# danielSanchezQ/dkg

Measured on AMD Instinct MI355X. Metric: verified shares/sec (whole node) at n=1024,t=511; full-ceremony wall time, higher is better.
Workload: dtype u32 (GF(2^255-19), Z_l); 1 GPU; one DKG ceremony n=1024, t=511 (share gen + round-2/4 checks + finalise); n=1024, t=511, parallelism=single GPU, verify_streams=2, rounds_2_4_fused=True, degree_split=4, recombination=short lattice multipliers, recombination_addends=affine Niels, stepping_additions=dedicated (complete redo where exceptional)

## Files before the change

### dkg_amd/_lib.py

```python
import ctypes
import os
import sys

HERE = os.path.dirname(os.path.abspath(__file__))
LIB_PATH = os.environ.get("DKG_AMD_LIB", os.path.join(HERE, "libdkg_amd.so"))

DKG_OK = 0
DKG_E_ARG = -1
DKG_E_DECODE = -2
DKG_E_DEVICE = -3
DKG_E_NOMEM = -4
REJECT, ACCEPT, SELF, SKIPPED, MISSING = 0, 1, 2, 3, 4
FIN_OK, FIN_R2_ERROR, FIN_R4_ERROR, FIN_PHASE4_ERROR, FIN_INSUFFICIENT, FIN_PANIC = 0, 1, 2, 3, 4, 5
COMPLAINT_IGNORED, COMPLAINT_NO_PHASE3 = 4, 5
COMPLAINT_NOT_OWNED = -2
DKG_PS_OK, DKG_PS_NO_COMMITMENT, DKG_PS_NO_DISCLOSURE = 0, 1, 2

_lib = None


class DkgError(RuntimeError):
    def __init__(self, code, msg=""):
        self.code = code
        names = {DKG_E_ARG: "DKG_E_ARG", DKG_E_DECODE: "DKG_E_DECODE", DKG_E_DEVICE: "DKG_E_DEVICE",
                 DKG_E_NOMEM: "DKG_E_NOMEM"}
        super().__init__(f"{names.get(code, code)}: {msg}")


class CeremonyOut(ctypes.Structure):
    _fields_ = [
        ("E", ctypes.c_void_p), ("A", ctypes.c_void_p),
        ("s", ctypes.c_void_p), ("s_prime", ctypes.c_void_p),
        ("dec2", ctypes.c_void_p), ("dec4", ctypes.c_void_p),
        ("qualified", ctypes.c_void_p), ("r2_error", ctypes.c_void_p), ("r4_error", ctypes.c_void_p),
        ("complaints2", ctypes.c_void_p), ("reconstruct", ctypes.c_void_p),
        ("final_share", ctypes.c_void_p), ("public_share", ctypes.c_void_p),
        ("mpk", ctypes.c_uint8 * 32),
        ("n_qualified", ctypes.c_int32), ("phase4_error", ctypes.c_int32),
        ("ms_round1", ctypes.c_double), ("ms_round2", ctypes.c_double), ("ms_round3", ctypes.c_double),
        ("ms_round4", ctypes.c_double), ("ms_finalise", ctypes.c_double), ("ms_total", ctypes.c_double),
    ]


class ReceiverPlan(ctypes.Structure):
    _fields_ = [("chunk", ctypes.c_uint32), ("stages", ctypes.c_uint32), ("arity", ctypes.c_uint32 * 16),
                ("mult", (ctypes.c_uint8 * 32) * 16)]


class ShardOutcome(ctypes.Structure):
    _fields_ = [
        ("qualified", ctypes.c_void_p), ("complaints2", ctypes.c_void_p), ("r2_error", ctypes.c_void_p),
        ("reconstruct", ctypes.c_void_p), ("r4_error", ctypes.c_void_p),
        ("n_qualified", ctypes.c_int32), ("phase4_error", ctypes.c_int32),
    ]


class BatchOut(ctypes.Structure):
    _fields_ = [
        ("mpk", ctypes.c_void_p), ("n_qualified", ctypes.c_void_p), ("phase4_error", ctypes.c_void_p),
        ("qualified", ctypes.c_void_p),
        ("r2_error", ctypes.c_void_p), ("r4_error", ctypes.c_void_p), ("complaints2", ctypes.c_void_p),
        ("reconstruct", ctypes.c_void_p), ("final_share", ctypes.c_void_p), ("public_share", ctypes.c_void_p),
        ("dec2", ctypes.c_void_p), ("dec4", ctypes.c_void_p),
        ("ms_round1", ctypes.c_double), ("ms_checks", ctypes.c_double), ("ms_round3", ctypes.c_double),
        ("ms_finalise", ctypes.c_double), ("ms_total", ctypes.c_double),
    ]


def lib():
    global _lib
    if _lib is not None:
        return _lib
    if not os.path.exists(LIB_PATH):
        raise RuntimeError(f"{LIB_PATH} is missing: build it with `make -C dkg_amd` or __graft_entry__.build()")
    if "torch" not in sys.modules and not os.environ.get("DKG_NO_TORCH_PREIMPORT"):
        try:
            import torch
        except Exception:
            pass
    L = ctypes.CDLL(LIB_PATH)
    sz, p, u8p = ctypes.c_size_t, ctypes.c_void_p, ctypes.c_char_p
    L.dkg_ctx_create.argtypes = [ctypes.c_int, ctypes.POINTER(p)]
    L.dkg_ctx_destroy.argtypes = [p]
    L.dkg_ctx_destroy.restype = None
    L.dkg_ctx_last_error.argtypes = [p]
    L.dkg_ctx_last_error.restype = ctypes.c_char_p
    L.dkg_device_count.argtypes = []
    L.dkg_ctx_set_streams.argtypes = [p, ctypes.c_int]
    L.dkg_ctx_set_overlap.argtypes = [p, ctypes.c_int]
    L.dkg_ctx_set_verify_mode.argtypes = [p, ctypes.c_int]
    L.dkg_ctx_fallback_rows.argtypes = [p]
    L.dkg_ctx_fallback_rows.restype = sz
    L.dkg_ctx_set_split.argtypes = [p, ctypes.c_int]
    L.dkg_ctx_set_stepping.argtypes = [p, ctypes.c_int]
    L.dkg_ctx_set_field_mode.argtypes = [p, ctypes.c_int]
    L.dkg_ctx_set_binomial.argtypes = [p, ctypes.c_int]
    L.dkg_ctx_set_check.argtypes = [p, ctypes.c_int]
    L.dkg_ctx_last_split.argtypes = [p]
    L.dkg_ctx_last_split_len.argtypes = [p]
    L.dkg_ctx_last_split_len.restype = sz
    L.dkg_split_model_ms.argtypes = [sz, sz, sz, ctypes.c_int]
    L.dkg_split_model_ms.restype = ctypes.c_double
    L.dkg_split_len.argtypes = [sz, sz, sz, ctypes.c_int]
    L.dkg_split_len.restype = sz
    L.dkg_ctx_set_combine.argtypes = [p, ctypes.c_int]
    L.dkg_ctx_last_combine.argtypes = [p]
    L.dkg_ctx_last_binomial.argtypes = [p]
    L.dkg_ctx_set_addends.argtypes = [p, ctypes.c_int]
    L.dkg_ctx_set_stepping_formula.argtypes = [p, ctypes.c_int]
    L.dkg_ctx_stepping_redos.argtypes = [p]
    L.dkg_ctx_stepping_redos.restype = ctypes.c_longlong
    L.dkg_ctx_binomial_reruns.argtypes = [p]
    L.dkg_ctx_binomial_wave_redos.argtypes = [p]
    L.dkg_ctx_binomial_wave_redos.restype = ctypes.c_longlong
    L.dkg_ctx_clock_probe.argtypes = [p, ctypes.c_uint, ctypes.POINTER(ctypes.c_double), ctypes.POINTER(ctypes.c_double)]
    L.dkg_device_pci_bus_id.argtypes = [ctypes.c_int, ctypes.c_char_p, ctypes.c_int]
    L.dkg_split_multipliers.argtypes = [sz, sz, ctypes.c_int, p, p]
    if hasattr(L, "dkg_zero_tests"):
        L.dkg_zero_tests.argtypes = [p, sz, p, p]
    if hasattr(L, "dkg_fe_ops"):
        L.dkg_fe_ops.argtypes = [p, ctypes.c_int, ctypes.c_int, sz, p, p]
    if hasattr(L, "dkg_sc_ops"):
        L.dkg_sc_ops.argtypes = [p, ctypes.c_int, sz, p, p]
    L.dkg_jsf_digits.argtypes = [p, p, p, p, p]
    L.dkg_split_digits.argtypes = [sz, sz, ctypes.c_int, ctypes.c_int, p, p]
    L.dkg_ctx_phase_ms.argtypes = [p, ctypes.c_char_p]
    L.dkg_ctx_phase_ms.restype = ctypes.c_double
    L.dkg_env_check.argtypes = [sz, sz]
    L.dkg_env_init.argtypes = [p, sz, sz, u8p, sz, p]
    L.dkg_msm_batch.argtypes = [p, sz, sz, u8p, u8p, p]
    L.dkg_fixed_base_batch.argtypes = [p, p, sz, u8p, p]
    L.dkg_poly_eval_batch.argtypes = [p, sz, sz, u8p, sz, p, p]
    L.dkg_points_valid_batch.argtypes = [p, sz, u8p, p]
    L.dkg_share_gen.argtypes = [p, sz, sz, sz, u8p, u8p, p, p, p, p]
    L.dkg_verify_pairs.argtypes = [p, sz, sz, ctypes.c_int, sz, sz, u8p, u8p, p, p]
    L.dkg_verify_receiver.argtypes = [p, sz, sz, ctypes.c_int, sz, u8p, u8p, p, p]
    L.dkg_receiver_plan_for.argtypes = [sz, sz, ctypes.c_uint32, ctypes.c_int, ctypes.POINTER(ReceiverPlan)]
    L.dkg_receiver_plan_cost_us.argtypes = [sz, sz, ctypes.c_uint32, ctypes.POINTER(ReceiverPlan)]
    L.dkg_receiver_plan_cost_us.restype = ctypes.c_double
    L.dkg_receiver_plan_constants.argtypes = [ctypes.POINTER(ctypes.c_double)]
    L.dkg_receiver_plan_constants.restype = None
    L.dkg_ctx_set_receiver_chunk.argtypes = [p, ctypes.c_int]
    L.dkg_ctx_last_receiver_chunk.argtypes = [p]
    L.dkg_commitment_eval.argtypes = [p, sz, sz, sz, p, u8p, p, p]
    if hasattr(L, "dkg_pair_eval_shape"):
        L.dkg_pair_eval_shape.argtypes = [sz, ctypes.c_int] + [ctypes.POINTER(ctypes.c_uint32)] * 3
        L.dkg_commitment_eval_pairs.argtypes = [p, sz, sz, sz, p, p, u8p, p, p]
    L.dkg_verify_receivers.argtypes = [p, sz, sz, ctypes.c_int, sz, p, u8p, u8p, p, p, p]
    L.dkg_party_round2.argtypes = [p, sz, sz, sz, u8p, u8p, u8p, u8p, p, p, p, p, p, p, p]
    if hasattr(L, "dkg_seat_pack"):
        L.dkg_seat_pack.argtypes = [sz, sz, p] + [ctypes.POINTER(ctypes.c_uint32)] * 3 + [p, p, ctypes.POINTER(ctypes.c_uint32)]
        L.dkg_commitment_eval_seats.argtypes = [p, sz, sz, sz, sz, p, p, u8p, p, p]
        L.dkg_verify_seats.argtypes = [p, sz, sz, sz, ctypes.c_int, sz, p, p, u8p, u8p, p, p, p]
        L.dkg_party_round2_seats.argtypes = [p, sz, sz, sz, sz, p, p, u8p, u8p, u8p, u8p, p, p, p, p, p, p, p]
    if hasattr(L, "dkg_finalise_seats"):
        L.dkg_complaints_verify_ceremonies.argtypes = [p, sz, sz, sz, sz, p, p, p, u8p, u8p, u8p, u8p, u8p, p, p]
        L.dkg_complaints3_verify_ceremonies.argtypes = [p, sz, sz, sz, sz, p, p, p, u8p, u8p, u8p, u8p, u8p, u8p, p, p]
        L.dkg_party_round3_seats.argtypes = [p, sz, sz, sz, sz, p, p, u8p, u8p, p, p]
        L.dkg_finalise_seats.argtypes = [p, sz, sz, sz, sz, p, p, u8p, u8p, u8p, u8p, u8p, u8p, u8p, sz, p, p, p, u8p,
                                         p, p, p]
        L.dkg_seat_finalise_status.argtypes = [sz, sz, sz, u8p, u8p, u8p, p, ctypes.c_int, ctypes.c_int, p]
    if hasattr(L, "dkg_party_round1_seats"):
        L.dkg_party_round1_seats.argtypes = [p, sz, sz, sz, sz, p, p, u8p, u8p, u8p, u8p, p, p, p, p, p, p, p]
        L.dkg_ctx_set_seat_deal.argtypes = [p, ctypes.c_int]
        L.dkg_ctx_last_seat_deal.argtypes = [p]
        L.dkg_seat_enc_digits.argtypes = [p, p, ctypes.POINTER(ctypes.c_int)]
    if hasattr(L, "dkg_seat_eval_shape"):
        L.dkg_seat_eval_shape.argtypes = [sz, sz, sz, ctypes.c_uint32, ctypes.c_int] + [ctypes.POINTER(ctypes.c_uint32)] * 3 + [
            ctypes.POINTER(ctypes.c_uint64)]
        L.dkg_seat_eval_constants.argtypes = [ctypes.POINTER(ctypes.c_double)]
        L.dkg_seat_eval_constants.restype = None
        L.dkg_ctx_set_seat_eval.argtypes = [p, ctypes.c_int, ctypes.c_int]
        L.dkg_ctx_last_seat_eval.argtypes = [p, ctypes.POINTER(ctypes.c_int)]
    if hasattr(L, "dkg_public_shares"):
        L.dkg_commitment_sum.argtypes = [p, sz, sz, sz, u8p, u8p, p, p]
        L.dkg_public_shares.argtypes = [p, sz, sz, sz, u8p, u8p, u8p, u8p, sz, p, sz, p, p, p, u8p, p, p, p, p]
        L.dkg_public_share_status.argtypes = [sz, u8p, u8p, u8p, ctypes.c_uint32, sz, p, p, p]
        L.dkg_ctx_set_public_share_slab.argtypes = [p, sz]
    L.dkg_ceremony_run.argtypes = [p, sz, sz, u8p, u8p, ctypes.POINTER(CeremonyOut)]
    L.dkg_ceremony_verify.argtypes = [p, sz, sz, u8p, u8p, u8p, u8p, ctypes.POINTER(CeremonyOut)]
    L.dkg_ceremony_verify_fetched.argtypes = [p, sz, sz, u8p, u8p, u8p, u8p, u8p, u8p, ctypes.POINTER(CeremonyOut)]
    L.dkg_ceremony_run_device.argtypes = [p, sz, sz, p, p, ctypes.POINTER(CeremonyOut)]
    L.dkg_ceremony_shard_device.argtypes = [p, sz, sz, sz, sz, p, p, p, p, p, p, ctypes.POINTER(ctypes.c_double)]
    L.dkg_ceremony_shard_verify_device.argtypes = [p, sz, sz, sz, sz, p, p, p, p, p, p, p, p,
                                                    ctypes.POINTER(ctypes.c_double)]
    L.dkg_ceremony_shard_full_device.argtypes = [p, sz, sz, sz, sz, p, p, p, u8p, u8p, p, p, p, p, p, p,
                                                  ctypes.POINTER(ctypes.c_double)]
    L.dkg_ceremony_shard_verify_full_device.argtypes = [p, sz, sz, sz, sz, p, p, p, p, u8p, p, p, p, p,
                                                         ctypes.POINTER(ctypes.c_double)]
    L.dkg_ctx_set_key_comb.argtypes = [p, ctypes.c_int]
    L.dkg_ctx_last_key_comb.argtypes = [p]
    L.dkg_key_comb_choice.argtypes = [sz, sz, ctypes.c_int, ctypes.c_int]
    L.dkg_key_comb_constants.argtypes = [ctypes.POINTER(ctypes.c_double)]
    L.dkg_key_comb_constants.restype = None
    L.dkg_ceremony_batch_device.argtypes = [p, sz, sz, sz, p, p, ctypes.POINTER(BatchOut)]
    L.dkg_ceremony_batch_verify.argtypes = [p, sz, sz, sz, u8p, u8p, u8p, u8p, ctypes.POINTER(BatchOut)]
    L.dkg_dealer_coeffs_device.argtypes = [p, u8p, ctypes.c_uint32, sz, sz, sz, sz, p, p]
    L.dkg_member_keys.argtypes = [p, u8p, ctypes.c_uint32, sz, p, p]
    L.dkg_enc_randomness.argtypes = [u8p, ctypes.c_uint32, sz, sz, sz, sz, p]
    L.dkg_enc_randomness_device.argtypes = [p, u8p, ctypes.c_uint32, sz, sz, sz, sz, sz, p]
    L.dkg_encrypt_shares.argtypes = [p, sz, sz, u8p, u8p, u8p, u8p, p, p]
    L.dkg_decrypt_shares.argtypes = [p, sz, sz, u8p, u8p, u8p, p, p, p]
    L.dkg_ceremony_run_full_device.argtypes = [p, sz, sz, p, p, p, u8p, u8p, ctypes.POINTER(CeremonyOut)]
    L.dkg_ceremony_verify_full.argtypes = [p, sz, sz, u8p, u8p, u8p, u8p, u8p, ctypes.POINTER(CeremonyOut)]
    L.dkg_member_keys_batch.argtypes = [p, u8p, ctypes.c_uint32, sz, sz, p, p]
    L.dkg_encrypt_shares_batch.argtypes = [p, sz, sz, u8p, u8p, u8p, u8p, p, p]
    L.dkg_decrypt_shares_batch.argtypes = [p, sz, sz, u8p, u8p, u8p, p, p, p]
    L.dkg_ceremony_batch_full_device.argtypes = [p, sz, sz, sz, p, p, p, u8p, u8p, ctypes.POINTER(BatchOut)]
    L.dkg_ceremony_batch_verify_full.argtypes = [p, sz, sz, sz, u8p, u8p, u8p, u8p, u8p, ctypes.POINTER(BatchOut),
                                                 p, p]
    L.dkg_ctx_set_batch_full_chunk.argtypes = [p, sz]
    L.dkg_misbehaviour_prove.argtypes = [p, sz, u8p, u8p, u8p, p]
    L.dkg_complaint1_verify.argtypes = [p, sz, sz, p, u8p, u8p, u8p, u8p, p]
    L.dkg_complaint3_verify.argtypes = [p, sz, sz, p, u8p, u8p, u8p, u8p, p]
    L.dkg_complaints_prove.argtypes = [p, sz, u8p, u8p, u8p, p]
    L.dkg_complaints_verify.argtypes = [p, sz, sz, sz, p, p, u8p, u8p, u8p, u8p, u8p, p, p]
    L.dkg_ctx_set_complaint_eval.argtypes = [p, ctypes.c_int]
    L.dkg_ceremony_verify_full_complaints.argtypes = [p, sz, sz, u8p, u8p, u8p, u8p, u8p, u8p, sz, p, p, u8p,
                                                      ctypes.POINTER(CeremonyOut), p, p]
    L.dkg_complaints3_verify.argtypes = [p, sz, sz, sz, p, p, u8p, u8p, u8p, u8p, u8p, u8p, p, p]
    L.dkg_ceremony_verify_fetched_proven.argtypes = [p, sz, sz, u8p, u8p, u8p, u8p, u8p, u8p, sz, p, p, u8p, u8p,
                                                     ctypes.POINTER(CeremonyOut), p, p, p]
    L.dkg_ceremony_verify_full_proven.argtypes = [p, sz, sz, u8p, u8p, u8p, u8p, u8p, u8p, sz, p, p, u8p, u8p, sz, p, p,
                                                  u8p, u8p, ctypes.POINTER(CeremonyOut), p, p, p, p, p]
    L.dkg_ceremony_batch_verify_proven.argtypes = [p, sz, sz, sz, u8p, u8p, u8p, u8p, u8p, u8p, sz, p, p, p, u8p, u8p,
                                                   ctypes.POINTER(BatchOut), p, p, p]
    L.dkg_ceremony_batch_verify_full_proven.argtypes = [p, sz, sz, sz, u8p, u8p, u8p, u8p, u8p, u8p, sz, p, p, p, u8p,
                                                        u8p, sz, p, p, p, u8p, u8p, ctypes.POINTER(BatchOut), p, p, p, p,
                                                        p, p, p]
    L.dkg_ceremony_shard_verify_proven_device.argtypes = [p, sz, sz, sz, sz, p, p, p, p, u8p, u8p, sz, p, p, u8p, u8p,
                                                           p, p, p, p, sz, p, p, ctypes.POINTER(ctypes.c_double)]
    L.dkg_ceremony_shard_verify_full_proven_device.argtypes = [p, sz, sz, sz, sz, p, p, p, p, u8p, u8p, u8p, u8p, sz, p,
                                                                p, u8p, sz, p, p, u8p, u8p, p, p, p, p, sz, p, p, p, p,
                                                                ctypes.POINTER(ctypes.c_double)]
    L.dkg_ctx_last_complaint_eval.argtypes = [p]
    L.dkg_shard_combine_proven_device.argtypes = [p, sz, sz, sz, p, p, p, p, ctypes.c_int, p, p,
                                                  ctypes.POINTER(ShardOutcome), p, p, p]
    L.dkg_multi_ceremony_verify_proven.argtypes = [p, sz, sz, u8p, u8p, u8p, u8p, u8p, u8p, sz, p, p, u8p, u8p,
                                                   ctypes.POINTER(CeremonyOut), p, p, p]
    L.dkg_multi_ceremony_verify_full_proven.argtypes = [p, sz, sz, u8p, u8p, u8p, u8p, u8p, u8p, sz, p, p, u8p, u8p, sz,
                                                        p, p, u8p, u8p, ctypes.POINTER(CeremonyOut), p, p, p, p, p]
    L.dkg_dealer_coeffs.argtypes = [u8p, ctypes.c_uint32, sz, sz, sz, p, p]
    L.dkg_scalar_sum_device.argtypes = [p, sz, sz, p, p, p]
    L.dkg_point_sum_device.argtypes = [p, sz, p, p, p]
    L.dkg_share_gen_device.argtypes = [p, sz, sz, sz, p, p, p, p, p, p]
    L.dkg_ceremony_shard_recon_device.argtypes = [p, sz, sz, sz, sz, u8p, u8p, u8p, u8p, p, p,
                                                  ctypes.POINTER(ctypes.c_int32)]
    L.dkg_finalise_parties.argtypes = [p, sz, sz, u8p, u8p, u8p, u8p, u8p, u8p, u8p, p, p, p]
    L.dkg_shard_range.argtypes = [sz, sz, sz, ctypes.POINTER(sz), ctypes.POINTER(sz)]
    L.dkg_shard_range.restype = None
    L.dkg_shard_rows.argtypes = [sz, sz]
    L.dkg_shard_rows.restype = sz
    L.dkg_shard_combine_device.argtypes = [p, sz, sz, sz, p, p, p, p, ctypes.POINTER(ShardOutcome)]
    L.dkg_shard_combine_packed_device.argtypes = [p, sz, sz, sz, p, p, p, p, ctypes.POINTER(ShardOutcome)]
    L.dkg_fixed_base_windows.argtypes = []
    L.dkg_key_comb_windows.argtypes = []
    if hasattr(L, "dkg_comb_geometry"):
        L.dkg_ctx_set_comb_build.argtypes = [p, ctypes.c_int]
        L.dkg_ctx_last_comb_build.argtypes = [p]
        L.dkg_ctx_last_comb_build_ms.argtypes = [p]
        L.dkg_ctx_last_comb_build_ms.restype = ctypes.c_double
        L.dkg_comb_geometry.argtypes = [ctypes.c_int, ctypes.POINTER(ctypes.c_int), ctypes.POINTER(ctypes.c_int),
                                        ctypes.POINTER(ctypes.c_uint32), ctypes.POINTER(ctypes.c_uint32)]
        L.dkg_comb_entries.argtypes = [p, ctypes.c_int, u8p, ctypes.c_int, ctypes.c_uint32, ctypes.c_uint32, p]
    L.dkg_packed_row_words.argtypes = [sz]
    L.dkg_packed_row_words.restype = sz
    L.dkg_decisions_pack_device.argtypes = [p, sz, sz, sz, sz, p, p]
    L.dkg_shard_finalise_device.argtypes = [p, sz, sz, sz, p, p, u8p, ctypes.c_int, p, p, p]
    L.dkg_multi_create.argtypes = [ctypes.POINTER(ctypes.c_int), ctypes.c_int, ctypes.POINTER(p)]
    L.dkg_multi_destroy.argtypes = [p]
    L.dkg_multi_destroy.restype = None
    L.dkg_multi_size.argtypes = [p]
    L.dkg_multi_ctx.argtypes = [p, ctypes.c_int]
    L.dkg_multi_ctx.restype = p
    L.dkg_multi_last_error.argtypes = [p]
    L.dkg_multi_last_error.restype = ctypes.c_char_p
    L.dkg_multi_phase_ms.argtypes = [p, ctypes.c_char_p]
    L.dkg_multi_phase_ms.restype = ctypes.c_double
    L.dkg_multi_env_init.argtypes = [p, sz, sz, u8p, sz, p]
    L.dkg_multi_ceremony_run.argtypes = [p, sz, sz, u8p, u8p, ctypes.POINTER(CeremonyOut)]
    L.dkg_multi_ceremony_run_device.argtypes = [p, sz, sz, ctypes.POINTER(p), ctypes.POINTER(p),
                                                ctypes.POINTER(CeremonyOut)]
    L.dkg_multi_ceremony_verify.argtypes = [p, sz, sz, u8p, u8p, u8p, u8p, ctypes.POINTER(CeremonyOut)]
    L.dkg_multi_ceremony_run_full.argtypes = [p, sz, sz, u8p, u8p, u8p, u8p, u8p, ctypes.POINTER(CeremonyOut)]
    L.dkg_multi_ceremony_run_full_device.argtypes = [p, sz, sz, ctypes.POINTER(p), ctypes.POINTER(p), ctypes.POINTER(p),
                                                     u8p, u8p, ctypes.POINTER(CeremonyOut)]
    L.dkg_multi_ceremony_verify_full.argtypes = [p, sz, sz, u8p, u8p, u8p, u8p, u8p, ctypes.POINTER(CeremonyOut)]
    _lib = L
    return L


EXPORTED = [
    "dkg_ctx_create", "dkg_ctx_destroy", "dkg_ctx_last_error", "dkg_ctx_phase_ms", "dkg_ctx_set_streams", "dkg_ctx_set_overlap",
    "dkg_device_count", "dkg_env_init",
    "dkg_env_check", "dkg_msm_batch", "dkg_fixed_base_batch", "dkg_poly_eval_batch",
    "dkg_points_valid_batch", "dkg_share_gen", "dkg_verify_pairs", "dkg_verify_receiver",
    "dkg_ctx_set_split", "dkg_ctx_set_stepping", "dkg_ctx_set_field_mode", "dkg_ctx_set_binomial", "dkg_ctx_set_check", "dkg_ctx_last_split", "dkg_ctx_last_split_len", "dkg_ctx_set_verify_mode", "dkg_ctx_fallback_rows", "dkg_split_model_ms", "dkg_split_len",
    "dkg_ctx_set_combine", "dkg_ctx_last_combine", "dkg_ctx_last_binomial", "dkg_ctx_set_addends", "dkg_ctx_set_stepping_formula", "dkg_ctx_stepping_redos", "dkg_zero_tests", "dkg_fe_ops", "dkg_sc_ops", "dkg_stepping_lane_map", "dkg_ctx_binomial_reruns", "dkg_ctx_binomial_wave_redos", "dkg_split_multipliers", "dkg_jsf_digits", "dkg_split_digits",
    "dkg_ctx_clock_probe", "dkg_device_pci_bus_id",
    "dkg_ceremony_run", "dkg_ceremony_verify", "dkg_ceremony_verify_fetched", "dkg_ceremony_run_device", "dkg_ceremony_shard_device",
    "dkg_ceremony_shard_verify_device",
    "dkg_ceremony_batch_device", "dkg_ceremony_batch_verify", "dkg_member_keys", "dkg_enc_randomness",
    "dkg_enc_randomness_device", "dkg_encrypt_shares", "dkg_decrypt_shares", "dkg_ceremony_run_full_device",
    "dkg_ceremony_verify_full", "dkg_misbehaviour_prove", "dkg_complaint1_verify", "dkg_complaint3_verify", "dkg_dealer_coeffs", "dkg_dealer_coeffs_device",
    "dkg_scalar_sum_device", "dkg_point_sum_device", "dkg_ceremony_shard_recon_device", "dkg_finalise_parties",
    "dkg_share_gen_device", "dkg_shard_range", "dkg_shard_rows", "dkg_shard_combine_device",
    "dkg_shard_combine_packed_device", "dkg_packed_row_words", "dkg_fixed_base_windows", "dkg_key_comb_windows", "dkg_decisions_pack_device",
    "dkg_shard_finalise_device", "dkg_multi_create", "dkg_multi_destroy", "dkg_multi_size", "dkg_multi_ctx",
    "dkg_multi_last_error", "dkg_multi_phase_ms", "dkg_multi_env_init", "dkg_multi_ceremony_run",
    "dkg_multi_ceremony_run_device", "dkg_multi_ceremony_verify",
    "dkg_member_keys_batch", "dkg_encrypt_shares_batch", "dkg_decrypt_shares_batch", "dkg_ceremony_batch_full_device",
    "dkg_ceremony_batch_verify_full", "dkg_ctx_set_batch_full_chunk",
    "dkg_complaints_prove", "dkg_complaints_verify", "dkg_ctx_set_complaint_eval", "dkg_ceremony_verify_full_complaints",
    "dkg_complaints3_verify", "dkg_ceremony_verify_fetched_proven", "dkg_ceremony_verify_full_proven",
    "dkg_ceremony_batch_verify_proven", "dkg_ceremony_batch_verify_full_proven",
    "dkg_ceremony_shard_full_device", "dkg_ceremony_shard_verify_full_device", "dkg_ctx_set_key_comb",
    "dkg_ctx_last_key_comb", "dkg_key_comb_choice", "dkg_key_comb_constants", "dkg_multi_ceremony_run_full",
    "dkg_multi_ceremony_run_full_device", "dkg_multi_ceremony_verify_full",
    "dkg_ceremony_shard_verify_proven_device", "dkg_ceremony_shard_verify_full_proven_device",
    "dkg_ctx_last_complaint_eval", "dkg_shard_combine_proven_device",
    "dkg_multi_ceremony_verify_proven", "dkg_multi_ceremony_verify_full_proven",
    "dkg_receiver_plan_for", "dkg_receiver_plan_cost_us", "dkg_receiver_plan_constants", "dkg_ctx_set_receiver_chunk",
    "dkg_ctx_set_comb_build", "dkg_ctx_last_comb_build", "dkg_ctx_last_comb_build_ms", "dkg_comb_geometry", "dkg_comb_entries",
    "dkg_ctx_last_receiver_chunk", "dkg_pair_eval_shape", "dkg_commitment_eval_pairs", "dkg_commitment_eval", "dkg_verify_receivers", "dkg_party_round2",
    "dkg_seat_pack", "dkg_commitment_eval_seats", "dkg_verify_seats", "dkg_party_round2_seats",
    "dkg_complaints_verify_ceremonies", "dkg_complaints3_verify_ceremonies", "dkg_party_round3_seats", "dkg_finalise_seats",
    "dkg_seat_finalise_status",
    "dkg_party_round1_seats", "dkg_ctx_set_seat_deal", "dkg_ctx_last_seat_deal", "dkg_seat_enc_digits",
    "dkg_seat_eval_shape", "dkg_seat_eval_constants", "dkg_ctx_set_seat_eval", "dkg_ctx_last_seat_eval",
    "dkg_commitment_sum", "dkg_public_shares", "dkg_public_share_status", "dkg_ctx_set_public_share_slab",
]
```

### dkg_amd/api.py

```python
import ctypes
from collections.abc import Sequence
from dataclasses import dataclass
from typing import List, Optional

from . import _lib
from ._lib import BatchOut, CeremonyOut, DkgError

CK_DEFAULT = b"Example of a shared string."


def _check(ctx, rc):
    if rc != _lib.DKG_OK:
        msg = _lib.lib().dkg_ctx_last_error(ctx).decode() if ctx else ""
        raise DkgError(rc, msg)


def env_check(threshold: int, nr_members: int) -> None:
    rc = _lib.lib().dkg_env_check(threshold, nr_members)
    if rc != _lib.DKG_OK:
        raise DkgError(rc, f"threshold {threshold} must be < (nr_members + 1) / 2 = {(nr_members + 1) // 2}")


def dealer_coefficients(master: bytes, ceremony: int, d0: int, D: int, t: int):
    N = t + 1
    a = ctypes.create_string_buffer(32 * D * N)
    b = ctypes.create_string_buffer(32 * D * N)
    rc = _lib.lib().dkg_dealer_coeffs(master, ceremony, d0, D, t, a, b)
    if rc != _lib.DKG_OK:
        raise DkgError(rc, "dealer_coeffs")
    return a.raw, b.raw


def enc_randomness(master: bytes, ceremony: int, d0: int, D: int, n: int, t: int) -> bytes:
    r = ctypes.create_string_buffer(max(64 * D * n, 1))
    rc = _lib.lib().dkg_enc_randomness(master, ceremony, d0, D, n, t, r)
    if rc != _lib.DKG_OK:
        raise DkgError(rc, "enc_randomness")
    return r.raw[:64 * D * n]


def split_multipliers(n: int, L: int, pieces: int):
    mag = ctypes.create_string_buffer(32 * n * pieces)
    sign = ctypes.create_string_buffer(n * pieces)
    rc = _lib.lib().dkg_split_multipliers(n, L, pieces, mag, sign)
    if rc != _lib.DKG_OK:
        raise DkgError(rc, "split_multipliers")
    sg = [1 if b < 128 else -1 for b in sign.raw]
    m = mag.raw
    return [[sg[j * pieces + u] * int.from_bytes(m[(j * pieces + u) * 32:(j * pieces + u + 1) * 32], "little")
             for u in range(pieces)] for j in range(n)]


def _carray(ctype, count: int, values=()):
    return (ctype * max(count, 1))(*values)


@dataclass
class CeremonyResult:
    n: int
    t: int
    mpk: bytes
    qualified: List[int]
    r2_error: List[int]
    r4_error: List[int]
    complaints2: List[int]
    reconstruct: List[int]
    n_qualified: int
    phase4_error: int
    ms: dict
    E: Optional[bytes] = None
    A: Optional[bytes] = None
    s: Optional[bytes] = None
    s_prime: Optional[bytes] = None
    dec2: Optional[bytes] = None
    dec4: Optional[bytes] = None
    final_share: Optional[bytes] = None
    public_share: Optional[bytes] = None


@dataclass
class ProvenResult:
    result: CeremonyResult
    verdict4: List[int]
    finalise_status: int
    recovery_index: int
    verdict: Optional[List[int]] = None
    dissent: Optional[List[int]] = None


@dataclass
class PartyFinalise:
    mpk: List[bytes]
    status: List[int]
    recovery_index: List[int]


@dataclass
class PublicShares:
    V: bytes
    status: List[int]
    which: List[int]
    S: Optional[bytes]


class Backend:

    def __init__(self, device: int = 0):
        L = _lib.lib()
        h = ctypes.c_void_p()
        rc = L.dkg_ctx_create(device, ctypes.byref(h))
        if rc != _lib.DKG_OK:
            raise DkgError(rc, f"dkg_ctx_create(device={device}) failed (is a gfx950 GPU visible?)")
        self._ctx = h
        self.device = device
        self.h: Optional[bytes] = None

    def close(self):
        if self._ctx:
            _lib.lib().dkg_ctx_destroy(self._ctx)
            self._ctx = None

    def __del__(self):
        try:
            self.close()
        except Exception:
            pass

    @property
    def ctx(self):
        return self._ctx

    def set_streams(self, nsub: int):
        _check(self._ctx, _lib.lib().dkg_ctx_set_streams(self._ctx, nsub))

    def set_verify_mode(self, mode):
        m = {"group": 0, "interp": 1}.get(mode, mode)
        _check(self._ctx, _lib.lib().dkg_ctx_set_verify_mode(self._ctx, int(m)))

    def fallback_rows(self) -> int:
        return _lib.lib().dkg_ctx_fallback_rows(self._ctx)

    def set_split(self, pieces: int):
        _check(self._ctx, _lib.lib().dkg_ctx_set_split(self._ctx, pieces))

    def set_field_mode(self, mode: int):
        _check(self._ctx, _lib.lib().dkg_ctx_set_field_mode(self._ctx, mode))

    def set_binomial(self, mode: int):
        _check(self._ctx, _lib.lib().dkg_ctx_set_binomial(self._ctx, mode))

    def set_check(self, mode: int):
        _check(self._ctx, _lib.lib().dkg_ctx_set_check(self._ctx, mode))

    def set_stepping(self, mode: int):
        _check(self._ctx, _lib.lib().dkg_ctx_set_stepping(self._ctx, mode))

    def set_combine(self, mode: int):
        _check(self._ctx, _lib.lib().dkg_ctx_set_combine(self._ctx, mode))

    def set_stepping_formula(self, mode: int):
        _check(self._ctx, _lib.lib().dkg_ctx_set_stepping_formula(self._ctx, mode))

    def stepping_redos(self) -> int:
        r = _lib.lib().dkg_ctx_stepping_redos(self._ctx)
        if r < 0:
            raise DkgError(_lib.DKG_E_DEVICE, "dkg_ctx_stepping_redos failed")
        return r

    def zero_tests(self, limbs) -> list:
        count = len(limbs)
        arr = (ctypes.c_uint32 * (10 * max(count, 1)))(*[v for el in limbs for v in el])
        out = ctypes.create_string_buffer(3 * max(count, 1))
        _check(self._ctx, _lib.lib().dkg_zero_tests(self._ctx, count, arr, out))
        return [tuple(out.raw[3 * i:3 * i + 3]) for i in range(count)]

    FE_OPS = {"mul": (0, 20, 10), "sq": (1, 10, 10), "mul2": (2, 40, 20), "sq2": (3, 20, 20),
              "mul_small": (4, 11, 10), "carry": (5, 10, 10), "add": (6, 20, 10), "sub": (7, 20, 10),
              "neg": (8, 10, 10), "dbl": (9, 10, 10), "invert": (10, 10, 10), "pow22523": (11, 10, 10),
              "tobytes": (12, 10, 10), "frombytes": (13, 8, 10), "abs": (14, 10, 10)}
    SC_OPS = {"reduce9": (0, 9, 8), "reduce256": (1, 8, 8), "reduce512": (2, 16, 8), "add": (3, 16, 8),
              "sub": (4, 16, 8), "neg": (5, 8, 8), "mul_small_add": (6, 17, 8), "horner2": (7, 25, 8),
              "lazy": (8, 20, 18), "mont_mul": (9, 16, 8), "mul": (10, 16, 8), "mont_inv": (11, 8, 8),
              "radix16": (12, 8, 16)}

    @staticmethod
    def _word_ops(table, op, tuples):
        code, win, wout = table[op]
        count = len(tuples)
        flat = [w for tup in tuples for w in tup]
        if len(flat) != win * count:
            raise ValueError(f"{op}: every operand tuple takes {win} words")
        arr = (ctypes.c_uint32 * max(len(flat), 1))(*flat)
        out = (ctypes.c_uint32 * max(wout * count, 1))()
        return code, count, wout, arr, out

    def fe_ops(self, flavour: int, op: str, tuples) -> list:
        code, count, wout, arr, out = self._word_ops(self.FE_OPS, op, tuples)
        _check(self._ctx, _lib.lib().dkg_fe_ops(self._ctx, flavour, code, count, arr, out))
        return [list(out[wout * i:wout * (i + 1)]) for i in range(count)]

    def sc_ops(self, op: str, tuples) -> list:
        code, count, wout, arr, out = self._word_ops(self.SC_OPS, op, tuples)
        _check(self._ctx, _lib.lib().dkg_sc_ops(self._ctx, code, count, arr, out))
        return [list(out[wout * i:wout * (i + 1)]) for i in range(count)]

    def binomial_reruns(self) -> int:
        return _lib.lib().dkg_ctx_binomial_reruns(self._ctx)

    def binomial_wave_redos(self) -> int:
        r = _lib.lib().dkg_ctx_binomial_wave_redos(self._ctx)
        if r < 0:
            raise DkgError(_lib.DKG_E_DEVICE, "dkg_ctx_binomial_wave_redos failed")
        return r

    def clock_probe(self, iters: int = 200_000) -> dict:
        mhz, ms = ctypes.c_double(), ctypes.c_double()
        _check(self._ctx, _lib.lib().dkg_ctx_clock_probe(self._ctx, iters, ctypes.byref(mhz), ctypes.byref(ms)))
        return {"sclk_mhz": mhz.value, "busy_ms": ms.value}

    def pci_bus_id(self) -> str:
        return device_pci_bus_id(self.device)

    def set_addends(self, mode: int):
        _check(self._ctx, _lib.lib().dkg_ctx_set_addends(self._ctx, mode))

    def last_combine(self) -> int:
        return _lib.lib().dkg_ctx_last_combine(self._ctx)

    def last_binomial(self) -> int:
        return _lib.lib().dkg_ctx_last_binomial(self._ctx)

    def last_split(self) -> int:
        return _lib.lib().dkg_ctx_last_split(self._ctx)

    def last_split_len(self) -> int:
        return _lib.lib().dkg_ctx_last_split_len(self._ctx)

    def set_overlap(self, on: bool):
        _check(self._ctx, _lib.lib().dkg_ctx_set_overlap(self._ctx, 1 if on else 0))

    def phase_times(self, tag="r24") -> dict:
        L = _lib.lib()
        if isinstance(tag, int):
            tag = f"r{tag}"
        names = (("interpolate", "coef_check", "decide", "fallback") if tag == "interp"
                 else ("decrypt", "decode", "chunks", "fold", "check", "prove") if tag == "recv"
                 else ("decode", "eval") if tag == "pairs"
                 else ("decode", "sum", "eval", "disclosed") if tag == "pubshares"
                 else ("decrypt", "decode", "eval", "fold", "check", "prove", "lagrange", "mpk", "commit", "deal_e1", "deal_mul",
                       "deal_encode", "deal_sym") if tag == "seats"
                 else ("enc_mul", "enc_encode", "enc_sym", "dec_decode", "dec_mul", "dec_encode", "dec_sym")
                 if tag == "full" else ("binomial", "stepping", "combine", "check"))
        return {k: L.dkg_ctx_phase_ms(self._ctx, f"{tag}.{k}".encode()) for k in names}

    def env_init(self, threshold: int, nr_members: int, ck_gen_bytes: bytes = CK_DEFAULT) -> bytes:
        out = ctypes.create_string_buffer(32)
        _check(self._ctx, _lib.lib().dkg_env_init(self._ctx, threshold, nr_members, ck_gen_bytes,
                                                   len(ck_gen_bytes), out))
        self.h = out.raw
        return out.raw

    def msm_batch(self, scalars: bytes, points: bytes, B: int, N: int) -> bytes:
        out = ctypes.create_string_buffer(32 * max(B, 1))
        _check(self._ctx, _lib.lib().dkg_msm_batch(self._ctx, B, N, scalars, points, out))
        return out.raw[: 32 * B]

    def fixed_base_batch(self, scalars: bytes, base: Optional[bytes] = None) -> bytes:
        count = len(scalars) // 32
        out = ctypes.create_string_buffer(32 * max(count, 1))
        _check(self._ctx, _lib.lib().dkg_fixed_base_batch(self._ctx, base, count, scalars, out))
        return out.raw[: 32 * count]

    def poly_eval_batch(self, coeffs: bytes, D: int, N: int, xs: List[int]) -> bytes:
        M = len(xs)
        arr = _carray(ctypes.c_uint32, M, xs)
        out = ctypes.create_string_buffer(32 * max(D * M, 1))
        _check(self._ctx, _lib.lib().dkg_poly_eval_batch(self._ctx, D, N, coeffs, M, arr, out))
        return out.raw[: 32 * D * M]

    def points_valid(self, points: bytes) -> bytes:
        count = len(points) // 32
        out = ctypes.create_string_buffer(max(count, 1))
        _check(self._ctx, _lib.lib().dkg_points_valid_batch(self._ctx, count, points, out))
        return out.raw[:count]

    def share_gen(self, a: bytes, b: bytes, D: int, n: int, t: int):
        N = t + 1
        E, A = ctypes.create_string_buffer(32 * D * N), ctypes.create_string_buffer(32 * D * N)
        s, sp = ctypes.create_string_buffer(32 * D * n), ctypes.create_string_buffer(32 * D * n)
        _check(self._ctx, _lib.lib().dkg_share_gen(self._ctx, D, n, t, a, b, E, A, s, sp))
        return E.raw, A.raw, s.raw, sp.raw

    def share_gen_device(self, D: int, n: int, t: int, d_a: int, d_b: int, d_E: Optional[int], d_A: Optional[int],
                         d_s: int, d_sp: int):
        vp = ctypes.c_void_p
        _check(self._ctx, _lib.lib().dkg_share_gen_device(self._ctx, D, n, t, vp(d_a), vp(d_b), vp(d_E), vp(d_A),
                                                           vp(d_s), vp(d_sp)))

    def verify_pairs(self, n: int, t: int, rnd: int, d0: int, d1: int, C: bytes, s: bytes,
                     s_prime: Optional[bytes] = None) -> bytes:
        dec = ctypes.create_string_buffer(max((d1 - d0) * n, 1))
        _check(self._ctx, _lib.lib().dkg_verify_pairs(self._ctx, n, t, rnd, d0, d1, C, s, s_prime, dec))
        return dec.raw[: (d1 - d0) * n]

    def verify_receiver(self, n: int, t: int, rnd: int, j: int, C: bytes, s_col: bytes,
                        sp_col: Optional[bytes] = None) -> bytes:
        dec = ctypes.create_string_buffer(max(n, 1))
        _check(self._ctx, _lib.lib().dkg_verify_receiver(self._ctx, n, t, rnd, j, C, s_col, sp_col, dec))
        return dec.raw[:n]

    def set_receiver_chunk(self, chunk: int = 0):
        _check(self._ctx, _lib.lib().dkg_ctx_set_receiver_chunk(self._ctx, chunk))

    def last_receiver_chunk(self) -> int:
        return _lib.lib().dkg_ctx_last_receiver_chunk(self._ctx)

    def commitment_eval(self, D: int, t: int, js: Sequence[int], C: bytes):
        M = len(js)
        arr = (ctypes.c_uint32 * max(M, 1))(*js)
        P = ctypes.create_string_buffer(max(32 * M * D, 1))
# ... 1090 lines not shown
```

### dkg_amd/csrc/kernels.hip

```cpp
#ifdef DKG_FE_ILP
#define dkgk dkgk_ilp
#endif
#include "kernels.h"
#include "split.h"

#include <algorithm>
#include <cmath>
#include <type_traits>
#include "points.h"

namespace dkgk {

constexpr int COMB_WORDS = AFF_WORDS * COMB_ENTRIES;

#ifndef DKG_DECODE_WAVES
#define DKG_DECODE_WAVES 2
#endif
__global__ __launch_bounds__(256, DKG_DECODE_WAVES) void k_decode(const uint32_t* __restrict__ comp, size_t count,
                                                uint32_t* __restrict__ ext, size_t stride,
                                                uint8_t* __restrict__ ok, size_t pm_N, size_t pm_npad,
                                                uint32_t nseg, uint32_t seg, size_t pm_L, size_t pm_pstride) {
  size_t e = (size_t)blockIdx.x * blockDim.x + threadIdx.x;
  if (e >= count) return;
  uint32_t w[8];
  ld_words8(w, comp + 8 * e);
  ge_p3 p;
  bool v = ristretto_decode(p, w);
  if (!v) ge_identity(p);
  size_t idx = e, oidx = e;
  if (pm_N) {
    const size_t i = e / pm_N, k = e % pm_N;
    const size_t col = (i / 64) * 64 * nseg + seg * 64 + i % 64;
    idx = (k % pm_L) * pm_npad + (k / pm_L) * pm_pstride + col;
    oidx = col * pm_N + k;
  }
  pt_store(ext, stride, idx, p);
  ok[oidx] = v ? 1 : 0;
}

__global__ __launch_bounds__(256) void k_place_pm(const uint32_t* __restrict__ src, size_t sstride, size_t D,
                                                  size_t N, uint32_t* __restrict__ out, size_t npad, uint32_t nseg,
                                                  uint32_t seg, size_t L, size_t pstride) {
  __shared__ uint32_t tile[64][65];
  const size_t w = blockIdx.z, k0 = (size_t)blockIdx.x * 64, i0 = (size_t)blockIdx.y * 64;
  const int tx = threadIdx.x & 63, ty = threadIdx.x >> 6;
#pragma unroll
  for (int r = 0; r < 16; r++) {
    const size_t i = i0 + ty + 4 * r, k = k0 + tx;
    if (i < D && k < N) tile[ty + 4 * r][tx] = src[w * sstride + i * N + k];
  }
  __syncthreads();
  const size_t i = i0 + tx;
  const size_t col = (i / 64) * 64 * nseg + seg * 64 + i % 64;
  uint32_t* o = out + w * L * npad + col;
#pragma unroll
  for (int r = 0; r < 16; r++) {
    const size_t k = k0 + ty + 4 * r;
    if (i < D && k < N) o[(k % L) * npad + (k / L) * pstride] = tile[tx][ty + 4 * r];
  }
}

void place_position_major(const uint32_t* src, size_t sstride, size_t D, size_t N, size_t npad, uint32_t* out,
                          hipStream_t stream, int nseg, int seg, size_t L, size_t pstride) {
  if (!D || !N) return;
  if (!L) L = N;
  hipLaunchKernelGGL(k_place_pm, dim3((unsigned)((N + 63) / 64), (unsigned)((D + 63) / 64), (unsigned)PT_WORDS),
                     dim3(256), 0, stream, src, sstride, D, N, out, npad, (uint32_t)nseg, (uint32_t)seg, L, pstride);
}

__global__ void k_gather_pts(const uint32_t* __restrict__ src, size_t sstride, size_t step, size_t k0, size_t count,
                             uint32_t* __restrict__ dst, size_t dstride) {
  const size_t i = (size_t)blockIdx.x * blockDim.x + threadIdx.x;
  if (i >= count) return;
#pragma unroll 8
  for (int w = 0; w < PT_WORDS; w++) dst[w * dstride + i] = src[w * sstride + i * step + k0];
}

void gather_points(const uint32_t* src, size_t sstride, size_t step, size_t k0, size_t count, uint32_t* dst,
                   size_t dstride, hipStream_t stream) {
  if (!count) return;
  hipLaunchKernelGGL(k_gather_pts, dim3((unsigned)((count + 255) / 256)), dim3(256), 0, stream, src, sstride, step, k0,
                     count, dst, dstride);
}

#ifndef DKG_ENCODE_WAVES
#define DKG_ENCODE_WAVES 3
#endif
#ifndef DKG_ENCODE_RECOMP
#define DKG_ENCODE_RECOMP 0
#endif
#ifndef DKG_ENCODE_PAIR
#define DKG_ENCODE_PAIR 0
#endif
#if DKG_ENCODE_PAIR
__global__ __launch_bounds__(256, DKG_ENCODE_WAVES) void k_encode(const uint32_t* __restrict__ ext, size_t stride,
                                                size_t count, uint32_t* __restrict__ comp) {
  const size_t half = (count + 1) / 2;
  const size_t e0 = (size_t)blockIdx.x * blockDim.x + threadIdx.x;
  if (e0 >= half) return;
  const size_t e1 = e0 + half;
  const bool two = e1 < count;
  fe t[2], inv[2];
#pragma unroll
  for (int k = 0; k < 2; k++) {
    ge_p3 p;
    fe u1, u2;
    pt_load(p, ext, stride, (k && two) ? e1 : e0);
    ristretto_encode_pre(u1, u2, t[k], p);
  }
  fe_invsqrt_x2(inv, t);
  const uint32_t* ext2 = ext;
  asm volatile("" : "+s"(ext2));
#pragma unroll
  for (int k = 0; k < 2; k++) {
    if (k && !two) break;
    const size_t e = k ? e1 : e0;
    ge_p3 p;
    pt_load(p, ext2, stride, e);
    fe u1, u2;
    ristretto_encode_u(u1, u2, p);
    uint32_t w[8];
    ristretto_encode_post(w, p, u1, u2, inv[k]);
    st_words8(comp + 8 * e, w);
  }
}
#else
__global__ __launch_bounds__(256, DKG_ENCODE_WAVES) void k_encode(const uint32_t* __restrict__ ext, size_t stride,
                                                size_t count, uint32_t* __restrict__ comp) {
  size_t e = (size_t)blockIdx.x * blockDim.x + threadIdx.x;
  if (e >= count) return;
  fe u1, u2, t, inv, one;
  {
    ge_p3 p;
    pt_load(p, ext, stride, e);
    ristretto_encode_pre(u1, u2, t, p);
  }
  fe_one(one);
  fe_sqrt_ratio_m1(inv, one, t);
  const uint32_t* ext2 = ext;
  asm volatile("" : "+s"(ext2));
  ge_p3 p;
  pt_load(p, ext2, stride, e);
  if (DKG_ENCODE_RECOMP) ristretto_encode_u(u1, u2, p);
  uint32_t w[8];
  ristretto_encode_post(w, p, u1, u2, inv);
  st_words8(comp + 8 * e, w);
}
#endif

void decode_points(const uint32_t* comp, size_t count, uint32_t* ext, size_t stride, uint8_t* ok,
                   hipStream_t stream) {
  if (!count) return;
  hipLaunchKernelGGL(k_decode, dim3((unsigned)((count + 255) / 256)), dim3(256), 0, stream, comp, count,
                     ext, stride, ok, (size_t)0, (size_t)0, 1u, 0u, (size_t)1, (size_t)0);
}

void decode_position_major(const uint32_t* comp, size_t D, size_t N, size_t npad, uint32_t* out, uint8_t* ok,
                           hipStream_t stream, int nseg, int seg, size_t L, size_t pstride) {
  const size_t count = D * N;
  if (!count) return;
  if (!L) L = N;
  hipLaunchKernelGGL(k_decode, dim3((unsigned)((count + 255) / 256)), dim3(256), 0, stream, comp, count, out,
                     L * npad, ok, N, npad, (uint32_t)nseg, (uint32_t)seg, L, pstride);
}

void encode_points(const uint32_t* ext, size_t stride, size_t count, uint32_t* comp, hipStream_t stream) {
  if (!count) return;
  const size_t lanes = DKG_ENCODE_PAIR ? (count + 1) / 2 : count;
  hipLaunchKernelGGL(k_encode, dim3((unsigned)((lanes + 255) / 256)), dim3(256), 0, stream, ext, stride,
                     count, comp);
}

__global__ __launch_bounds__(64) void k_build_comb(const uint32_t* __restrict__ ext, size_t stride, size_t e0,
                                                   uint32_t* __restrict__ tab) {
  const int w = threadIdx.x;
  tab += (size_t)blockIdx.x * COMB_WORDS;
  ge_p3 b;
  pt_load(b, ext, stride, e0 + blockIdx.x);
  for (int i = 0; i < 4 * w; i++) ge_dbl<true>(b, b);
  ge_cached bc;
  ge_to_cached(bc, b);
  ge_p3 m = b;
  fe d2;
  fe_ld(d2, ge_const::D2);
  for (int d = 1; d <= 8; d++) {
    if (d > 1) ge_add(m, m, bc);
    fe zi, x, y, t;
    fe_invert(zi, m.Z);
    fe_mul(x, m.X, zi);
    fe_mul(y, m.Y, zi);
    const int e = w * 8 + d - 1;
    fe_add(t, y, x);
    fe_carry(t, t);
#pragma unroll
    for (int i = 0; i < 10; i++) tab[i * COMB_ENTRIES + e] = t.v[i];
    fe_sub(t, y, x);
    fe_carry(t, t);
#pragma unroll
    for (int i = 0; i < 10; i++) tab[(10 + i) * COMB_ENTRIES + e] = t.v[i];
    fe_mul(t, x, y);
    fe_mul(t, t, d2);
#pragma unroll
    for (int i = 0; i < 10; i++) tab[(20 + i) * COMB_ENTRIES + e] = t.v[i];
  }
}

void build_comb(const uint32_t* ext, size_t stride, size_t e0, uint32_t* tab, hipStream_t stream, size_t count) {
  if (!count) return;
  hipLaunchKernelGGL(k_build_comb, dim3((unsigned)count), dim3(64), 0, stream, ext, stride, e0, tab);
}

__device__ __forceinline__ void lds_fill(uint32_t* lds, const uint32_t* __restrict__ g, int words) {
  const uint4* src = reinterpret_cast<const uint4*>(g);
  uint4* dst = reinterpret_cast<uint4*>(lds);
  for (int i = threadIdx.x; i < words / 4; i += blockDim.x) dst[i] = src[i];
}


__global__ __launch_bounds__(256, DKG_COMB_WAVES) void k_commit(size_t count, const uint32_t* __restrict__ a,
                                                const uint32_t* __restrict__ b,
                                                const uint32_t* __restrict__ tab_g,
                                                const uint32_t* __restrict__ tab_h,
                                                uint32_t* __restrict__ A_ext, uint32_t* __restrict__ E_ext,
                                                size_t stride) {
  const size_t e = (size_t)blockIdx.x * blockDim.x + threadIdx.x;
  if (e >= count) return;
  sc x;
  sc_load(x, a + 8 * e);
  ge_p3 acc;
  ge_identity(acc);
  combw_mul_add(acc, x, tab_g);
  pt_store(A_ext, stride, e, acc);
  sc_load(x, b + 8 * e);
  combw_mul_add(acc, x, tab_h);
  pt_store(E_ext, stride, e, acc);
}

void commit(size_t count, const uint32_t* a, const uint32_t* b, const uint32_t* tab_g, const uint32_t* tab_h,
            uint32_t* A_ext, uint32_t* E_ext, hipStream_t stream, size_t stride) {
  if (!count) return;
  hipLaunchKernelGGL(k_commit, dim3((unsigned)((count + 255) / 256)), dim3(256), 0, stream, count, a, b, tab_g, tab_h,
                     A_ext, E_ext, stride ? stride : count);
}

__global__ __launch_bounds__(64, 3) void k_commit_pm(size_t D, size_t N, const uint32_t* __restrict__ a,
                                                   const uint32_t* __restrict__ b,
                                                   const uint32_t* __restrict__ tab_g,
                                                   const uint32_t* __restrict__ tab_h, uint32_t* __restrict__ out,
                                                   size_t W, size_t L, size_t pstride,
                                                   uint32_t* __restrict__ A0, size_t A0stride) {
  const size_t g = blockIdx.x, i = g * 64 + threadIdx.x;
  const uint32_t k = blockIdx.y, Lu = (uint32_t)L;
  if (i >= D) return;
  sc x;
  sc_load(x, a + 8 * (i * N + k));
  ge_p3 acc;
  ge_identity(acc);
  combw_mul_add(acc, x, tab_g);
  uint32_t* o = out + (size_t)(k % Lu) * W + (size_t)(k / Lu) * pstride + g * 128;
  asm volatile("" : "+s"(o));
  pt_store(o + 64, L * W, threadIdx.x, acc);
  if (k == 0) pt_store(A0, A0stride, i, acc);
  sc_load(x, b + 8 * (i * N + k));
  combw_mul_add(acc, x, tab_h);
  asm volatile("" : "+s"(o));
  pt_store(o, L * W, threadIdx.x, acc);
}

void commit_position_major(size_t D, size_t N, const uint32_t* a, const uint32_t* b, const uint32_t* tab_g,
                           const uint32_t* tab_h, uint32_t* out, size_t W, size_t L, size_t pstride, uint32_t* A0,
                           size_t A0stride, hipStream_t stream) {
  if (!D || !N) return;
  hipLaunchKernelGGL(k_commit_pm, dim3((unsigned)((D + 63) / 64), (unsigned)N), dim3(64), 0, stream, D, N, a, b, tab_g,
                     tab_h, out, W, L, pstride, A0, A0stride);
}

__global__ __launch_bounds__(256) void k_share_eval(size_t D, size_t n, size_t N, const uint32_t* __restrict__ a,
                                                    const uint32_t* __restrict__ b, uint32_t* __restrict__ s,
                                                    uint32_t* __restrict__ sp) {
  const size_t e = (size_t)blockIdx.x * blockDim.x + threadIdx.x;
  if (e >= D * n) return;
  size_t i = e / n;
  const size_t j = e % n;
  if (n % 64 == 0) i = (size_t)(uint32_t)__builtin_amdgcn_readfirstlane((uint32_t)i);
  const uint32_t x = (uint32_t)(j + 1);
  const uint32_t* ai = a + 8 * i * N;
  const uint32_t* bi = b + 8 * i * N;
  sc fa, fb, c;
  sc_load(fa, ai + 8 * (N - 1));
  sc_load(fb, bi + 8 * (N - 1));
  size_t k = N - 1;
  if (x < 8192) {
    uint32_t va[10], vb[10];
#pragma unroll
    for (int i = 0; i < 10; i++) {
      va[i] = i < 8 ? fa.v[i] : 0u;
      vb[i] = i < 8 ? fb.v[i] : 0u;
    }
    while (k > 0) {
      const int steps = k < (size_t)SC_LAZY_STEPS ? (int)k : SC_LAZY_STEPS;
#pragma unroll 1
      for (int u = 0; u < steps; u++) {
        k--;
        sc_load(c, ai + 8 * k);
        sc_lazy_step(va, x, c);
        sc_load(c, bi + 8 * k);
        sc_lazy_step(vb, x, c);
      }
      sc_lazy_fold(va);
      sc_lazy_fold(vb);
    }
    sc_lazy_final(fa, va);
    sc_lazy_final(fb, vb);
  }
  while (k-- > 0) {
    sc_load(c, ai + 8 * k);
    sc_mul_small_add(fa, fa, x, c);
    sc_load(c, bi + 8 * k);
    sc_mul_small_add(fb, fb, x, c);
  }
  st_words8(s + 8 * e, fa.v);
  st_words8(sp + 8 * e, fb.v);
}
// ... 1697 lines not shown
  if (!width || !jn || (pieces != 2 && pieces != 4)) return;
  const dim3 grid((unsigned)((width + 63) / 64), (unsigned)jn);
  if (pieces == 2)
    hipLaunchKernelGGL((k_combine_jsf<2, 1>), grid, dim3(64), 0, stream, width, pstride, nrecv, digits, top, ev, A, R, j0);
  else
    hipLaunchKernelGGL((k_combine_jsf<4, 2>), grid, dim3(64), 0, stream, width, pstride, nrecv, digits, top, ev, A, R, j0);
}

void combine(size_t width, size_t pstride, size_t pieces, size_t nrecv, const int8_t* digits, const int16_t* top,
             uint32_t* R, hipStream_t stream) {
  if (!width || !nrecv || pieces < 2) return;
  const dim3 grid((unsigned)((width + 63) / 64), (unsigned)nrecv);
  if (pieces == 2)
    hipLaunchKernelGGL(k_combine<1>, grid, dim3(64), 0, stream, width, pstride, (int)pieces, nrecv, digits, top, R);
  else
    hipLaunchKernelGGL(k_combine<2>, grid, dim3(64), 0, stream, width, pstride, (int)pieces, nrecv, digits, top, R);
}

__global__ __launch_bounds__(256, DKG_COMB_WAVES) void k_check(size_t ndealers, size_t nrecv, size_t dealer_base, size_t recv_base,
                                               uint32_t nmod, int round,
                                               const uint32_t* __restrict__ s, const uint32_t* __restrict__ sp,
                                               const uint32_t* __restrict__ R,
                                               const uint32_t* __restrict__ tab_g,
                                               const uint32_t* __restrict__ tab_h,
                                               const uint8_t* __restrict__ dok, uint8_t* __restrict__ dec,
                                               const uint32_t* __restrict__ scale) {
  const size_t p = (size_t)blockIdx.x * blockDim.x + threadIdx.x;
  if (p >= ndealers * nrecv) return;
  const size_t i = p / nrecv, j = p % nrecv;
  ge_p3 acc, r;
  ge_identity(acc);
  sc x, f;
  if (scale) sc_load(f, scale + 8 * j);
  sc_load(x, s + 8 * p);
  if (scale) sc_mont_mul(x, x, f);
  combw_mul_add(acc, x, tab_g);
  if (round == 2) {
    sc_load(x, sp + 8 * p);
    if (scale) sc_mont_mul(x, x, f);
    combw_mul_add(acc, x, tab_h);
  }
  pt_load_aos(r, R, p);
  const bool eq = ristretto_eq(acc, r);
  uint8_t v = dok[i] ? (eq ? 1 : 0) : (round == 2 ? 4 : 0);
  if ((uint32_t)((i + dealer_base) % nmod) == (uint32_t)(j + recv_base)) v = 2;
  dec[p] = v;
}

void check(size_t ndealers, size_t nrecv, size_t dealer_base, size_t recv_base, size_t nmod, int round,
           const uint32_t* s, const uint32_t* sp, const uint32_t* R, const uint32_t* tab_g,
           const uint32_t* tab_h, const uint8_t* dok, uint8_t* dec, hipStream_t stream, const uint32_t* scale) {
  const size_t total = ndealers * nrecv;
  if (!total) return;
  hipLaunchKernelGGL(k_check, dim3((unsigned)((total + 255) / 256)), dim3(256), 0, stream, ndealers, nrecv,
                     dealer_base, recv_base, (uint32_t)nmod, round, s, sp, R, tab_g, tab_h, dok, dec, scale);
}

template <int PASS>
__global__ __launch_bounds__(256, DKG_COMB_WAVES) void k_check_both(size_t ndealers, size_t nrecv, size_t dealer0, size_t dealer_base,
                                                    uint32_t nmod, const uint32_t* __restrict__ s,
                                                    const uint32_t* __restrict__ sp, const uint32_t* __restrict__ R,
                                                    const uint32_t* __restrict__ tab_g,
                                                    const uint32_t* __restrict__ tab_h,
                                                    const uint8_t* __restrict__ dok, uint8_t* __restrict__ dec2,
                                                    uint8_t* __restrict__ dec4, const uint32_t* __restrict__ scale,
                                                    size_t j0, size_t jn, uint32_t* __restrict__ accb) {
  const size_t p = (size_t)blockIdx.x * blockDim.x + threadIdx.x;
  if (p >= ndealers * jn) return;
  const size_t i = dealer0 + p / jn, j = j0 + p % jn;
  const size_t cE = (i / 64) * 128 + i % 64, cA = cE + 64;
  const size_t q = i * nrecv + j;
  const bool self = (uint32_t)((i + dealer_base) % nmod) == (uint32_t)j;
  ge_p3 acc, r;
  sc x, f;
  if (scale) sc_load(f, scale + 8 * j);
  if constexpr (PASS != 2) {
    ge_identity(acc);
    sc_load(x, s + 8 * q);
    if (scale) sc_mont_mul(x, x, f);
    combw_mul_add<DKG_CHECK_IL != 0>(acc, x, tab_g);
    pt_load_aos(r, R, cA * nrecv + j);
    const bool eq = ristretto_eq(acc, r);
    dec4[q] = self ? 2 : ((dok[cA] && eq) ? 1 : 0);
    if constexpr (PASS == 1) {
      pt_store_aos(accb, p, acc);
      return;
    }
  } else {
    pt_load_aos(acc, accb, p);
  }
  sc_load(x, sp + 8 * q);
  if (scale) sc_mont_mul(x, x, f);
  combw_mul_add<DKG_CHECK_IL != 0>(acc, x, tab_h);
  pt_load_aos(r, R, cE * nrecv + j);
  const bool eq = ristretto_eq(acc, r);
  dec2[q] = self ? 2 : (dok[cE] ? (eq ? 1 : 0) : 4);
}

void check_both(size_t ndealers, size_t nrecv, size_t dealer0, size_t dealer_base, size_t nmod, const uint32_t* s,
                const uint32_t* sp, const uint32_t* R, const uint32_t* tab_g, const uint32_t* tab_h,
                const uint8_t* dok, uint8_t* dec2, uint8_t* dec4, hipStream_t stream, const uint32_t* scale, size_t j0,
                size_t jn, uint32_t* acc) {
  if (!jn) jn = nrecv - j0;
  const size_t total = ndealers * jn;
  if (!total) return;
  const dim3 grid((unsigned)((total + 255) / 256));
  if (!acc) {
    hipLaunchKernelGGL(k_check_both<0>, grid, dim3(256), 0, stream, ndealers, nrecv, dealer0, dealer_base,
                       (uint32_t)nmod, s, sp, R, tab_g, tab_h, dok, dec2, dec4, scale, j0, jn, acc);
    return;
  }
  hipLaunchKernelGGL(k_check_both<1>, grid, dim3(256), 0, stream, ndealers, nrecv, dealer0, dealer_base,
                     (uint32_t)nmod, s, sp, R, tab_g, tab_h, dok, dec2, dec4, scale, j0, jn, acc);
  hipLaunchKernelGGL(k_check_both<2>, grid, dim3(256), 0, stream, ndealers, nrecv, dealer0, dealer_base,
                     (uint32_t)nmod, s, sp, R, tab_g, tab_h, dok, dec2, dec4, scale, j0, jn, acc);
}

__global__ void k_fill_all_identity(size_t S, uint32_t* __restrict__ out) {
  const size_t e = (size_t)blockIdx.x * blockDim.x + threadIdx.x;
  if (e >= S) return;
  ge_p3 id;
  ge_identity(id);
  pt_store(out, S, e, id);
}

void fill_identity(size_t S, uint32_t* out, hipStream_t stream) {
  if (!S) return;
  hipLaunchKernelGGL(k_fill_all_identity, dim3((unsigned)((S + 255) / 256)), dim3(256), 0, stream, S, out);
}

__global__ void k_dealer_ok(size_t ndealers, size_t N, const uint8_t* __restrict__ pok, uint8_t* __restrict__ ok) {
  const size_t i = (size_t)blockIdx.x * blockDim.x + threadIdx.x;
  if (i >= ndealers) return;
  uint8_t v = 1;
  for (size_t k = 0; k < N; k++) v &= pok[i * N + k];
  ok[i] = v;
}

__global__ void k_and_dealer_mask(size_t D, uint32_t nseg, uint32_t seg, const uint8_t* __restrict__ extra,
                                  uint8_t* __restrict__ dok) {
  const size_t i = (size_t)blockIdx.x * blockDim.x + threadIdx.x;
  if (i >= D) return;
  const size_t col = (i / 64) * 64 * nseg + seg * 64 + i % 64;
  dok[col] &= extra[i];
}

void and_dealer_mask(size_t D, int nseg, int seg, const uint8_t* extra, uint8_t* dok, hipStream_t stream) {
  if (!D) return;
  hipLaunchKernelGGL(k_and_dealer_mask, dim3((unsigned)((D + 255) / 256)), dim3(256), 0, stream, D, (uint32_t)nseg,
                     (uint32_t)seg, extra, dok);
}

__global__ __launch_bounds__(256) void k_mask_not_and(size_t V, const uint8_t* __restrict__ a,
                                                      const uint8_t* __restrict__ b, uint8_t* __restrict__ out) {
  const size_t i = (size_t)blockIdx.x * 256 + threadIdx.x;
  if (i < V) out[i] = !a[i] && (!b || b[i]);
}

void mask_not_and(size_t V, const uint8_t* a, const uint8_t* b, uint8_t* out, hipStream_t stream) {
  if (!V) return;
  hipLaunchKernelGGL(k_mask_not_and, dim3((unsigned)((V + 255) / 256)), dim3(256), 0, stream, V, a, b, out);
}

void dealer_ok(size_t ndealers, size_t N, const uint8_t* point_ok, uint8_t* ok, hipStream_t stream) {
  if (!ndealers) return;
  hipLaunchKernelGGL(k_dealer_ok, dim3((unsigned)((ndealers + 255) / 256)), dim3(256), 0, stream, ndealers, N,
                     point_ok, ok);
}

__global__ __launch_bounds__(64, 3) void k_horner(size_t ndealers, size_t npad, size_t N, const uint32_t* __restrict__ C,
                                                uint32_t x0, size_t nrecv, uint32_t* __restrict__ R) {
  const size_t d = (size_t)blockIdx.x * blockDim.x + threadIdx.x;
  const uint32_t x = x0 + blockIdx.y;
  if (d >= npad) return;
  const size_t S = N * npad;
  ge_p3 acc, c;
  pt_load(acc, C, S, (N - 1) * npad + d);
  for (size_t k = N - 1; k-- > 0;) {
    mul_small_uniform(acc, acc, x);
    pt_load(c, C, S, k * npad + d);
    ge_cached cc;
    ge_to_cached(cc, c);
    ge_add(acc, acc, cc);
  }
  if (d < ndealers) pt_store_aos(R, d * nrecv + blockIdx.y, acc);
}

void horner(size_t ndealers, size_t npad, size_t N, const uint32_t* C, uint32_t x0, size_t nrecv, uint32_t* R,
            hipStream_t stream) {
  if (!ndealers || !nrecv) return;
  hipLaunchKernelGGL(k_horner, dim3((unsigned)(npad / 64), (unsigned)nrecv), dim3(64), 0, stream, ndealers, npad, N,
                     C, x0, nrecv, R);
}

__global__ __launch_bounds__(256) void k_sum_points(size_t count, const uint32_t* __restrict__ pts, size_t stride,
                                                    const uint8_t* __restrict__ mask, uint32_t* __restrict__ out,
                                                    size_t ostride, size_t col) {
  __shared__ uint32_t red[256][PT_WORDS];
  ge_p3 acc;
  ge_identity(acc);
  const size_t g = blockIdx.x;
  for (size_t e = g * count + threadIdx.x; e < (g + 1) * count; e += blockDim.x) {
    if (mask && !mask[e]) continue;
    ge_p3 p;
    pt_load(p, pts, stride, e);
    ge_cached pc;
    ge_to_cached(pc, p);
    ge_add(acc, acc, pc);
  }
  uint32_t* aw = reinterpret_cast<uint32_t*>(&acc);
  for (int w = 0; w < PT_WORDS; w++) red[threadIdx.x][w] = aw[w];
  __syncthreads();
  for (int h = 128; h > 0; h >>= 1) {
    if ((int)threadIdx.x < h) {
      ge_p3 x, y;
      uint32_t* xw = reinterpret_cast<uint32_t*>(&x);
      uint32_t* yw = reinterpret_cast<uint32_t*>(&y);
      for (int w = 0; w < PT_WORDS; w++) {
        xw[w] = red[threadIdx.x][w];
        yw[w] = red[threadIdx.x + h][w];
      }
      ge_cached yc;
      ge_to_cached(yc, y);
      ge_add(x, x, yc);
      for (int w = 0; w < PT_WORDS; w++) red[threadIdx.x][w] = xw[w];
    }
    __syncthreads();
  }
  if (threadIdx.x == 0)
    for (int w = 0; w < PT_WORDS; w++) out[w * ostride + col + g] = red[0][w];
}

void sum_points(size_t count, const uint32_t* pts, size_t stride, const uint8_t* mask, uint32_t* out,
                size_t ostride, size_t col, hipStream_t stream, size_t groups) {
  if (!groups) return;
  hipLaunchKernelGGL(k_sum_points, dim3((unsigned)groups), dim3(256), 0, stream, count, pts, stride, mask, out,
                     ostride, col);
}

__global__ __launch_bounds__(256) void k_add_points(size_t count, const uint32_t* __restrict__ a,
                                                    const uint32_t* __restrict__ b, size_t stride,
                                                    uint32_t* __restrict__ out) {
  const size_t e = (size_t)blockIdx.x * blockDim.x + threadIdx.x;
  if (e >= count) return;
  ge_p3 x, y;
  pt_load(x, a, stride, e);
  pt_load(y, b, stride, e);
  ge_cached yc;
  ge_to_cached(yc, y);
  ge_add(x, x, yc);
  pt_store(out, stride, e, x);
}

void add_points(size_t count, const uint32_t* a, const uint32_t* b, size_t stride, uint32_t* out,
                hipStream_t stream) {
  if (!count) return;
  hipLaunchKernelGGL(k_add_points, dim3((unsigned)((count + 255) / 256)), dim3(256), 0, stream, count, a, b, stride,
                     out);
}

__global__ void k_from_uniform(const uint32_t* __restrict__ in16, uint32_t* __restrict__ out) {
  uint32_t a[8], b[8];
  for (int i = 0; i < 8; i++) {
    a[i] = in16[i];
    b[i] = in16[8 + i];
  }
  ge_p3 p, q;
  ristretto_elligator(p, a);
  ristretto_elligator(q, b);
  ge_cached qc;
  ge_to_cached(qc, q);
  ge_add(p, p, qc);
  pt_store(out, 1, 0, p);
}

void from_uniform(const uint32_t* in16, uint32_t* out, hipStream_t stream) {
  hipLaunchKernelGGL(k_from_uniform, dim3(1), dim3(1), 0, stream, in16, out);
}

__global__ __launch_bounds__(256) void k_msm_tables(size_t count, const uint32_t* __restrict__ pts, size_t stride,
                                                  uint32_t* __restrict__ tab) {
  const size_t e = (size_t)blockIdx.x * blockDim.x + threadIdx.x;
  if (e >= count) return;
  ge_p3 p, acc;
  pt_load(p, pts, stride, e);
  ge_cached pc;
  ge_to_cached(pc, p);
  acc = p;
  uint4* out = reinterpret_cast<uint4*>(tab + e * 15 * PT_WORDS);
#pragma unroll 1
  for (int d = 1; d <= 15; d++) {
    if (d > 1) ge_add(acc, acc, pc);
    ge_cached c;
    ge_to_cached(c, acc);
    const uint4* c4 = reinterpret_cast<const uint4*>(&c);
#pragma unroll
    for (int w = 0; w < PT_WORDS / 4; w++) out[(d - 1) * (PT_WORDS / 4) + w] = c4[w];
  }
}

__global__ __launch_bounds__(256) void k_msm(size_t N, const uint32_t* __restrict__ scalars,
                                             const uint32_t* __restrict__ tab, uint32_t* __restrict__ out,
                                             size_t ostride) {
  __shared__ uint32_t red[256][PT_WORDS];
  const size_t b = blockIdx.x;
  const int T = blockDim.x, q = threadIdx.x;
  ge_p3 acc;
  ge_identity(acc);
  if ((size_t)q < N) {
#pragma unroll 1
    for (int w = 63; w >= 0; w--) {
      if (w != 63) {
#pragma unroll 1
        for (int i = 0; i < 4; i++) ge_dbl_lean(acc, acc, i == 3);
      }
#pragma unroll 1
      for (size_t k = q; k < N; k += T) {
        const uint32_t word = scalars[8 * (b * N + k) + (w >> 3)];
        const uint32_t nib = (word >> (4 * (w & 7))) & 15u;
        if (nib) {
          ge_cached c;
          const uint4* src = reinterpret_cast<const uint4*>(tab + ((b * N + k) * 15 + nib - 1) * PT_WORDS);
          uint4* c4 = reinterpret_cast<uint4*>(&c);
#pragma unroll
          for (int x = 0; x < PT_WORDS / 4; x++) c4[x] = src[x];
          ge_add(acc, acc, c);
        }
      }
    }
  }
  uint32_t* aw = reinterpret_cast<uint32_t*>(&acc);
  for (int w = 0; w < PT_WORDS; w++) red[q][w] = aw[w];
  __syncthreads();
  for (int h = T / 2; h > 0; h >>= 1) {
    if (q < h) {
      ge_p3 x, y;
      uint32_t* xw = reinterpret_cast<uint32_t*>(&x);
      uint32_t* yw = reinterpret_cast<uint32_t*>(&y);
      for (int w = 0; w < PT_WORDS; w++) {
        xw[w] = red[q][w];
        yw[w] = red[q + h][w];
      }
      ge_cached yc;
      ge_to_cached(yc, y);
      ge_add(x, x, yc);
      for (int w = 0; w < PT_WORDS; w++) red[q][w] = xw[w];
    }
    __syncthreads();
  }
  if (q == 0) {
    ge_p3 r;
    uint32_t* rw = reinterpret_cast<uint32_t*>(&r);
    for (int w = 0; w < PT_WORDS; w++) rw[w] = red[0][w];
    pt_store(out, ostride, b, r);
  }
}

void msm_batch(size_t B, size_t N, const uint32_t* scalars, const uint32_t* pts, size_t stride, uint32_t* tab,
               uint32_t* out_ext, hipStream_t stream) {
  if (!B) return;
  const size_t count = B * N;
  if (count)
    hipLaunchKernelGGL(k_msm_tables, dim3((unsigned)((count + 255) / 256)), dim3(256), 0, stream, count, pts, stride,
                       tab);
  size_t T = 64;
  while (T < N && T < 256) T <<= 1;
  hipLaunchKernelGGL(k_msm, dim3((unsigned)B), dim3((unsigned)T), 0, stream, N, scalars, tab, out_ext, B);
}

__global__ __launch_bounds__(256, 4) void k_fixed_base(size_t count, const uint32_t* __restrict__ scalars,
                                                    const uint32_t* __restrict__ tab, uint32_t* __restrict__ out) {
  const size_t e = (size_t)blockIdx.x * blockDim.x + threadIdx.x;
  if (e >= count) return;
  sc x;
  sc_load(x, scalars + 8 * e);
  ge_p3 acc;
  ge_identity(acc);
  combw_mul_add(acc, x, tab);
  pt_store(out, count, e, acc);
}

void fixed_base(size_t count, const uint32_t* scalars, const uint32_t* tab, uint32_t* out_ext, hipStream_t stream) {
  if (!count) return;
  hipLaunchKernelGGL(k_fixed_base, dim3((unsigned)((count + 255) / 256)), dim3(256), 0, stream, count, scalars, tab,
                     out_ext);
}

__global__ void k_to_pos_major(size_t D, size_t N, size_t npad, const uint32_t* __restrict__ in,
                               uint32_t* __restrict__ out) {
  const size_t e = (size_t)blockIdx.x * blockDim.x + threadIdx.x;
  if (e >= N * npad) return;
  const size_t k = e / npad, i = e % npad;
  const size_t S = N * npad, Sin = D * N;
  for (int w = 0; w < PT_WORDS; w++) {
    uint32_t v;
    if (i < D) v = in[w * Sin + i * N + k];
    else v = (w == 10 || w == 20) ? 1u : 0u;
    out[w * S + e] = v;
  }
}

void to_position_major(size_t D, size_t N, size_t npad, const uint32_t* in, uint32_t* out, hipStream_t stream) {
  const size_t tot = N * npad;
  if (!tot) return;
  hipLaunchKernelGGL(k_to_pos_major, dim3((unsigned)((tot + 255) / 256)), dim3(256), 0, stream, D, N, npad, in, out);
}

__global__ void k_reduce_scalars(size_t count, const uint32_t* __restrict__ in, uint32_t* __restrict__ out) {
  const size_t e = (size_t)blockIdx.x * blockDim.x + threadIdx.x;
  if (e >= count) return;
  uint32_t w[8];
  ld_words8(w, in + 8 * e);
  w[7] &= 0x7fffffffu;
  sc r;
  sc_reduce256(r, w);
  st_words8(out + 8 * e, r.v);
}

void reduce_scalars(size_t count, const uint32_t* in, uint32_t* out, hipStream_t stream) {
  if (!count) return;
  hipLaunchKernelGGL(k_reduce_scalars, dim3((unsigned)((count + 255) / 256)), dim3(256), 0, stream, count, in, out);
}

template <int SLICES>
__global__ __launch_bounds__(64 * SLICES) void k_sum_shares(size_t D, size_t n, const uint32_t* __restrict__ s,
                                                          const uint8_t* __restrict__ mask,
                                                          uint32_t* __restrict__ out) {
  __shared__ uint32_t part[SLICES > 1 ? SLICES * 8 * 64 : 1];
  const int lane = threadIdx.x & 63, slice = threadIdx.x >> 6;
  const size_t j = (size_t)blockIdx.x * 64 + lane;
  const size_t g = blockIdx.y;
  s += g * D * n * 8;
  mask += g * D;
  out += g * n * 8;
  sc acc, x;
  sc_zero(acc);
  if (j < n)
    for (size_t i = slice; i < D; i += SLICES) {
      if (!mask[i]) continue;
      sc_load(x, s + 8 * (i * n + j));
      sc_add(acc, acc, x);
    }
  if (SLICES > 1) {
#pragma unroll
    for (int w = 0; w < 8; w++) part[(slice * 8 + w) * 64 + lane] = acc.v[w];
    __syncthreads();
    if (slice != 0) return;
    for (int q = 1; q < SLICES; q++) {
#pragma unroll
      for (int w = 0; w < 8; w++) x.v[w] = part[(q * 8 + w) * 64 + lane];
      sc_add(acc, acc, x);
    }
  }
  if (j < n) st_words8(out + 8 * j, acc.v);
}

void sum_shares(size_t D, size_t n, const uint32_t* s, const uint8_t* mask, uint32_t* out, hipStream_t stream,
                size_t groups) {
  if (!n) return;
  for (size_t g0 = 0; g0 < groups; g0 += 65535) {
    const size_t gc = groups - g0 < 65535 ? groups - g0 : 65535;
    const dim3 grid((unsigned)((n + 63) / 64), (unsigned)gc);
    if (gc * ((n + 63) / 64) >= 1024)
      hipLaunchKernelGGL(k_sum_shares<1>, grid, dim3(64), 0, stream, D, n, s + g0 * D * n * 8, mask + g0 * D,
                         out + g0 * n * 8);
    else
      hipLaunchKernelGGL(k_sum_shares<16>, grid, dim3(1024), 0, stream, D, n, s + g0 * D * n * 8, mask + g0 * D,
                         out + g0 * n * 8);
  }
}

__global__ __launch_bounds__(256) void k_row_reject(size_t rows, size_t n, const uint8_t* __restrict__ dec,
                                                    uint8_t* __restrict__ out) {
  const size_t i = (size_t)blockIdx.x * 4 + (threadIdx.x >> 6);
  if (i >= rows) return;
  bool r = false;
  for (size_t j = threadIdx.x & 63; j < n; j += 64) r |= dec[i * n + j] == 0 || dec[i * n + j] == 4;
  const bool any = __ballot(r) != 0;
  if ((threadIdx.x & 63) == 0) out[i] = any;
}

constexpr int COL_SLICES = 16;
template <typename Pred>
__device__ __forceinline__ int32_t column_count(size_t groups, size_t n, const uint8_t* __restrict__ dec, Pred pred,
                                                size_t& e_out) {
  __shared__ int32_t part[COL_SLICES][64];
  const int lane = threadIdx.x & 63, slice = threadIdx.x >> 6;
  const size_t e = (size_t)blockIdx.x * 64 + lane;
  const bool live = e < groups * n;
  const size_t g = live ? e / n : 0, j = live ? e % n : 0;
  int32_t c = 0;
  if (live)
    for (size_t i = slice; i < n; i += COL_SLICES) c += pred(g * n + i, dec[(g * n + i) * n + j]);
  part[slice][lane] = c;
  __syncthreads();
  int32_t s = 0;
  if (slice == 0)
    for (int k = 0; k < COL_SLICES; k++) s += part[k][lane];
  e_out = live && slice == 0 ? e : SIZE_MAX;
  return s;
}

__global__ __launch_bounds__(64 * COL_SLICES) void k_col_complaints(size_t groups, size_t n,
                                                                   const uint8_t* __restrict__ dec,
                                                                   int32_t* __restrict__ out) {
  size_t e;
  const int32_t c = column_count(groups, n, dec, [](size_t, uint8_t d) { return (int32_t)(d == 0); }, e);
  if (e != SIZE_MAX) out[e] = c;
}

__global__ __launch_bounds__(64 * COL_SLICES) void k_r4_error(size_t groups, size_t n, size_t t,
                                                             const uint8_t* __restrict__ dec,
                                                             const uint8_t* __restrict__ qmask,
                                                             uint8_t* __restrict__ out) {
  size_t e;
  const int32_t c = column_count(
      groups, n, dec, [qmask](size_t row, uint8_t d) { return (int32_t)(qmask[row] && d == 1); }, e);
  if (e != SIZE_MAX) out[e] = (size_t)(1 + c) < t + 1;
}

void r4_error(size_t groups, size_t n, size_t t, const uint8_t* dec, const uint8_t* qmask, uint8_t* out,
              hipStream_t stream) {
  const size_t rows = groups * n;
  if (!rows) return;
  hipLaunchKernelGGL(k_r4_error, dim3((unsigned)((rows + 63) / 64)), dim3(64 * COL_SLICES), 0, stream, groups, n, t,
                     dec, qmask, out);
}

__global__ __launch_bounds__(256) void k_apply_skipped(size_t rows, size_t n, uint8_t* __restrict__ dec,
                                                       const uint8_t* __restrict__ qmask) {
  const size_t i = (size_t)blockIdx.x * 4 + (threadIdx.x >> 6);
  if (i >= rows || qmask[i]) return;
  const size_t self = i % n;
  for (size_t j = threadIdx.x & 63; j < n; j += 64)
    if (j != self) dec[i * n + j] = 3;
}

void apply_skipped(size_t groups, size_t n, uint8_t* dec, const uint8_t* qmask, hipStream_t stream) {
  const size_t rows = groups * n;
  if (!rows) return;
  hipLaunchKernelGGL(k_apply_skipped, dim3((unsigned)((rows + 3) / 4)), dim3(256), 0, stream, rows, n, dec, qmask);
}

template <typename T>
__global__ __launch_bounds__(256) void k_compact_ranks(size_t n, size_t ws, size_t R, size_t q,
                                                       const T* __restrict__ in, T* __restrict__ out) {
  const size_t e = (size_t)blockIdx.x * 256 + threadIdx.x;
  if (e >= n * q) return;
  const size_t i = e / q, w = e % q;
  size_t r = (i * ws) / n;
  while (r + 1 < ws && ((r + 1) * n) / ws <= i) r++;
  while (r > 0 && (r * n) / ws > i) r--;
  out[e] = in[(r * R + (i - (r * n) / ws)) * q + w];
}

void compact_ranks(size_t n, size_t ws, size_t R, size_t width, const void* in, void* out, hipStream_t stream) {
  if (!n || !width) return;
  const uintptr_t al = (uintptr_t)in | (uintptr_t)out | width;
  if (al % 16 == 0) {
    const size_t q = width / 16, total = n * q;
    hipLaunchKernelGGL(k_compact_ranks<uint4>, dim3((unsigned)((total + 255) / 256)), dim3(256), 0, stream, n, ws, R,
                       q, (const uint4*)in, (uint4*)out);
  } else if (al % 4 == 0) {
    const size_t q = width / 4, total = n * q;
    hipLaunchKernelGGL(k_compact_ranks<uint32_t>, dim3((unsigned)((total + 255) / 256)), dim3(256), 0, stream, n, ws,
                       R, q, (const uint32_t*)in, (uint32_t*)out);
  } else {
    const size_t total = n * width;
    hipLaunchKernelGGL(k_compact_ranks<uint8_t>, dim3((unsigned)((total + 255) / 256)), dim3(256), 0, stream, n, ws,
                       R, width, (const uint8_t*)in, (uint8_t*)out);
  }
}

__global__ __launch_bounds__(64) void k_pack_rows(size_t nvalid, size_t n, size_t d0, const uint8_t* __restrict__ dec,
                                                  uint32_t* __restrict__ out, uint32_t* __restrict__ err) {
  const size_t r = blockIdx.y, W = (n + 31) / 32, w = (size_t)blockIdx.x * 64 + threadIdx.x;
  if (w > W) return;
  uint32_t* o = out + r * (W + 1);
  if (r >= nvalid) {
    o[w] = 0;
    return;
  }
  const uint8_t* row = dec + r * n;
  const size_t self = d0 + r;
  const uint8_t ref = n > 1 ? row[self == 0 ? 1 : 0] : 1;
  const uint32_t kind = ref == 4 ? 1u : ref == 3 ? 2u : 0u;
  if (w == W) {
    o[w] = kind;
    return;
  }
  uint32_t bits = 0, bad = 0;
  for (int b = 0; b < 32; b++) {
    const size_t j = w * 32 + b;
    if (j >= n) break;
    const uint32_t v = row[j];
    if (j == self) bad |= v != 2;
    else if (kind == 0) {
      bad |= v > 1;
      bits |= (v & 1u) << b;
    } else {
      bad |= v != (kind == 1 ? 4u : 3u);
    }
  }
  o[w] = bits;
  if (bad) err[0] = 1u;
}

void pack_rows(size_t rows, size_t nvalid, size_t n, size_t d0, const uint8_t* dec, uint32_t* out, uint32_t* err,
               hipStream_t stream) {
  if (!rows || !n) return;
  const size_t W1 = (n + 31) / 32 + 1;
  hipLaunchKernelGGL(k_pack_rows, dim3((unsigned)((W1 + 63) / 64), (unsigned)rows), dim3(64), 0, stream, nvalid, n,
                     d0, dec, out, err);
}

__global__ __launch_bounds__(256) void k_unpack_ranks(size_t n, size_t ws, size_t R, const uint32_t* __restrict__ in,
                                                      uint8_t* __restrict__ out) {
  const size_t W = (n + 31) / 32, e = (size_t)blockIdx.x * 256 + threadIdx.x;
  if (e >= n * W) return;
  const size_t i = e / W, w = e % W;
  size_t r = (i * ws) / n;
// ... 47 lines not shown
```

### dkg_amd/csrc/kernels_decl.inc

```
namespace dkgk {

void decode_points(const uint32_t* comp, size_t count, uint32_t* ext, size_t stride, uint8_t* ok,
                   hipStream_t stream);
void place_position_major(const uint32_t* src, size_t sstride, size_t D, size_t N, size_t npad, uint32_t* out,
                          hipStream_t stream, int nseg = 1, int seg = 0, size_t L = 0, size_t pstride = 0);
void gather_points(const uint32_t* src, size_t sstride, size_t step, size_t k0, size_t count, uint32_t* dst,
                   size_t dstride, hipStream_t stream);
void decode_position_major(const uint32_t* comp, size_t D, size_t N, size_t npad, uint32_t* out, uint8_t* ok,
                           hipStream_t stream, int nseg = 1, int seg = 0, size_t L = 0, size_t pstride = 0);
void fill_identity(size_t S, uint32_t* out, hipStream_t stream);
void check_both(size_t ndealers, size_t nrecv, size_t dealer0, size_t dealer_base, size_t nmod, const uint32_t* s,
                const uint32_t* sp, const uint32_t* R, const uint32_t* tab_g, const uint32_t* tab_h,
                const uint8_t* dok, uint8_t* dec2, uint8_t* dec4, hipStream_t stream, const uint32_t* scale = nullptr,
                size_t j0 = 0, size_t jn = 0, uint32_t* acc = nullptr);
void encode_points(const uint32_t* ext, size_t stride, size_t count, uint32_t* comp, hipStream_t stream);
void build_comb(const uint32_t* ext, size_t stride, size_t e0, uint32_t* tab, hipStream_t stream, size_t count = 1);
void build_combw(const uint32_t* ext, size_t stride, size_t e0, uint32_t* tab, hipStream_t stream, size_t count = 1);

void commit_position_major(size_t D, size_t N, const uint32_t* a, const uint32_t* b, const uint32_t* tab_g,
                           const uint32_t* tab_h, uint32_t* out, size_t W, size_t L, size_t pstride, uint32_t* A0,
                           size_t A0stride, hipStream_t stream);
void commit(size_t count, const uint32_t* a, const uint32_t* b, const uint32_t* tab_g,
            const uint32_t* tab_h, uint32_t* A_ext, uint32_t* E_ext, hipStream_t stream, size_t stride = 0);
void share_eval(size_t D, size_t n, size_t N, const uint32_t* a, const uint32_t* b, uint32_t* s,
                uint32_t* sp, hipStream_t stream);
void poly_eval(size_t D, size_t N, const uint32_t* coeffs, size_t M, const uint32_t* xs, uint32_t* out,
               hipStream_t stream);

uint32_t* binomial(size_t width, size_t npad, size_t N, const uint32_t* C, uint32_t* e0, uint32_t* e1,
                   hipStream_t stream, size_t pieces = 1, size_t pstride = 0, size_t last_len = 0);
void binom_init(size_t width, size_t npad, size_t N, const uint32_t* C, uint32_t* e0, hipStream_t stream,
                size_t pieces = 1, size_t pstride = 0);
void binom_step(size_t r, size_t width, size_t npad, size_t N, const uint32_t* C, const uint32_t* in, uint32_t* out,
                hipStream_t stream, size_t pieces = 1, size_t pstride = 0, size_t last_len = 0,
                uint32_t* flags = nullptr, size_t col_base = 0, size_t dreal = 0, unsigned gw = 64,
                bool flag_any = false,
                bool nt = false,
                bool il = false);
void binomial_wave_redo(size_t width, size_t npad, size_t N, const uint32_t* C, uint32_t* e, hipStream_t stream,
                        size_t pieces, size_t pstride, size_t last_len, uint32_t* flags, size_t col_base,
                        size_t dreal, unsigned gw);
uint32_t* binomial_wave(size_t width, size_t npad, size_t N, const uint32_t* C, uint32_t* e, hipStream_t stream,
                        size_t pieces = 1, size_t pstride = 0, size_t last_len = 0, uint32_t* eT = nullptr,
                        bool prefetch = false, uint32_t* flags = nullptr, size_t col_base = 0, size_t dreal = 0,
                        unsigned gw = 64);
void binom_step_pair(size_t r, size_t width, size_t npad, size_t N, const uint32_t* C, const uint32_t* in,
                     uint32_t* out, hipStream_t stream, size_t pieces = 1, size_t pstride = 0, size_t last_len = 0);
void to_column_major(size_t width, size_t npad, size_t N, const uint32_t* e, uint32_t* eT, size_t pieces,
                     size_t pstride, hipStream_t stream);
struct StepShape {
  size_t nblk, P, per, bs, maxbs;
};
StepShape stepping_shape(size_t N);
double step_occupancy(size_t bs, size_t maxbs);
bool stepping_whole_columns(size_t L, size_t pieces, size_t last_len);
double stepping_cycles(size_t cols, size_t N, size_t pieces, size_t last_len, bool whole, size_t nrecv = 0);
double stepping_waves_per_simd(size_t cols, size_t N, size_t pieces, size_t last_len, bool whole);
size_t stepping_flag_words(size_t ndealers, size_t pieces);
void zero_tests(size_t count, const uint32_t* limbs, uint8_t* out, hipStream_t stream);
enum {
  FE_OP_MUL, FE_OP_SQ, FE_OP_MUL2, FE_OP_SQ2, FE_OP_MUL_SMALL, FE_OP_CARRY, FE_OP_ADD, FE_OP_SUB, FE_OP_NEG,
  FE_OP_DBL, FE_OP_INVERT, FE_OP_POW22523, FE_OP_TOBYTES, FE_OP_FROMBYTES, FE_OP_ABS, FE_OP_COUNT
};
bool fe_ops_shape(int op, size_t* win, size_t* wout);
void fe_ops(int op, size_t count, const uint32_t* in, uint32_t* out, hipStream_t stream);
enum {
  SC_OP_REDUCE9, SC_OP_REDUCE256, SC_OP_REDUCE512, SC_OP_ADD, SC_OP_SUB, SC_OP_NEG, SC_OP_MUL_SMALL_ADD,
  SC_OP_HORNER2, SC_OP_LAZY, SC_OP_MONT_MUL, SC_OP_MUL, SC_OP_MONT_INV, SC_OP_RADIX16, SC_OP_COUNT
};
bool sc_ops_shape(int op, size_t* win, size_t* wout);
uint32_t sc_ops_lazy_steps();
void sc_ops(int op, size_t count, const uint32_t* in, uint32_t* out, hipStream_t stream);
bool stepping(size_t ndealers, size_t npad, size_t N, const uint32_t* e, size_t nrecv, uint32_t* R,
              uint32_t* stream_a, uint32_t* stream_b, hipStream_t stream, size_t pieces = 1, size_t pstride = 0,
              size_t last_len = 0, bool whole = true, uint32_t* flags = nullptr, size_t col0 = 0,
              size_t dreal = (size_t)-1, unsigned gw = 64, uint32_t* Rz = nullptr, uint32_t* tail_a = nullptr,
              uint32_t* tail_b = nullptr, bool r_scaled = false);
int stepping_tail_phases(size_t N, size_t nrecv, size_t pieces);
size_t stepping_tail_words(size_t ndealers, size_t N);
void combine(size_t width, size_t pstride, size_t pieces, size_t nrecv, const int8_t* digits, const int16_t* top,
             uint32_t* R, hipStream_t stream);
void combine_short(size_t width, size_t pstride, size_t pieces, size_t nrecv, const uint32_t* digits,
                   const int16_t* top, uint32_t* R, hipStream_t stream);
void affine_pieces(size_t width, size_t pstride, size_t pieces, size_t nrecv, const uint32_t* R, uint32_t* A,
                   hipStream_t stream, const uint32_t* Rz = nullptr, size_t j0 = 0, size_t jn = 0,
                   bool scaled = false);
void combine_short_aff(size_t width, size_t pstride, size_t pieces, size_t nrecv, const uint32_t* digits,
                       const int16_t* top, const uint32_t* A, uint32_t* R, hipStream_t stream, size_t j0 = 0,
                       size_t jn = 0);
void affine_pairs(size_t width, size_t pstride, size_t pieces, size_t nrecv, const uint32_t* R, uint32_t* A,
                  hipStream_t stream, size_t j0 = 0, size_t jn = 0, bool scaled = false);
constexpr uint32_t JSF_EV_NONE = 0xffu;
constexpr size_t JSF_EV_WORDS = 384;
void combine_short_jsf(size_t width, size_t pstride, size_t pieces, size_t nrecv, const uint32_t* digits,
                       const int16_t* top, const uint32_t* ev, const uint32_t* A, uint32_t* R, hipStream_t stream,
                       size_t j0 = 0, size_t jn = 0);
void check(size_t ndealers, size_t nrecv, size_t dealer_base, size_t recv_base, size_t nmod, int round,
           const uint32_t* s, const uint32_t* sp, const uint32_t* R, const uint32_t* tab_g,
           const uint32_t* tab_h, const uint8_t* dealer_ok, uint8_t* decision, hipStream_t stream,
           const uint32_t* scale = nullptr);
void and_dealer_mask(size_t D, int nseg, int seg, const uint8_t* extra, uint8_t* dok, hipStream_t stream);
void dealer_ok(size_t ndealers, size_t N, const uint8_t* point_ok, uint8_t* ok, hipStream_t stream);
void horner(size_t ndealers, size_t npad, size_t N, const uint32_t* C, uint32_t x0, size_t nrecv, uint32_t* R,
            hipStream_t stream);
void sum_points(size_t count, const uint32_t* pts, size_t stride, const uint8_t* mask, uint32_t* out, size_t ostride,
                size_t col, hipStream_t stream, size_t groups = 1);
void add_points(size_t count, const uint32_t* a, const uint32_t* b, size_t stride, uint32_t* out, hipStream_t stream);
void r4_error(size_t groups, size_t n, size_t t, const uint8_t* dec, const uint8_t* qmask, uint8_t* out,
              hipStream_t stream);
void decision_summary(size_t groups, size_t n, const uint8_t* dec, uint8_t* row_reject, int32_t* complaints,
                      hipStream_t stream);
void apply_skipped(size_t groups, size_t n, uint8_t* dec, const uint8_t* qmask, hipStream_t stream);
void compact_ranks(size_t n, size_t ws, size_t R, size_t width, const void* in, void* out, hipStream_t stream);
void mask_not_and(size_t V, const uint8_t* a, const uint8_t* b, uint8_t* out, hipStream_t stream);
void row_reject(size_t rows, size_t n, const uint8_t* dec, uint8_t* out, hipStream_t stream);
size_t key_comb_words();
int key_comb_windows();
void build_key_combs(const uint32_t* ext, size_t stride, size_t e0, uint32_t* tab, hipStream_t stream,
                     size_t count);
int fixed_base_windows();
void pack_rows(size_t rows, size_t nvalid, size_t n, size_t d0, const uint8_t* dec, uint32_t* out, uint32_t* err,
               hipStream_t stream);
void unpack_ranks(size_t n, size_t ws, size_t R, const uint32_t* in, uint8_t* out, hipStream_t stream);
void from_uniform(const uint32_t* in16, uint32_t* out, hipStream_t stream);

void msm_batch(size_t B, size_t N, const uint32_t* scalars, const uint32_t* pts, size_t stride, uint32_t* tab,
               uint32_t* out_ext, hipStream_t stream);
void fixed_base(size_t count, const uint32_t* scalars, const uint32_t* tab, uint32_t* out_ext,
                hipStream_t stream);
void to_position_major(size_t D, size_t N, size_t npad, const uint32_t* in, uint32_t* out,
                       hipStream_t stream);
void reduce_scalars(size_t count, const uint32_t* in, uint32_t* out, hipStream_t stream);
void sum_shares(size_t D, size_t n, const uint32_t* s, const uint8_t* mask, uint32_t* out, hipStream_t stream,
                size_t groups = 1);
void dealer_coeffs(size_t rows, size_t D, size_t d0, uint32_t c0, const uint32_t* master, size_t N, uint32_t* seeds,
                   uint32_t* a, uint32_t* b, hipStream_t stream);

void enc_mul(size_t D, size_t n, const uint32_t* r, const uint32_t* tab_gw, const uint32_t* tabs_pk, uint32_t* R_ext,
             uint32_t* K_ext, hipStream_t stream);
void dec_mul(size_t D, size_t n, const uint32_t* sk, const uint32_t* R_ext, uint32_t* K_ext, hipStream_t stream,
             uint32_t* table = nullptr);
size_t dec_mul_table_words(size_t D, size_t n);
void sym_xor(size_t D, size_t n, const uint32_t* Kc, bool decrypt, uint32_t* ct, uint32_t* s, uint32_t* sp,
             hipStream_t stream);
void dealer_seeds(size_t rows, size_t D, size_t d0, uint32_t c0, const uint32_t* master, uint32_t* seeds,
                  hipStream_t stream);
void enc_randomness(size_t rows, size_t n, size_t N, const uint32_t* seeds, uint32_t* r, hipStream_t stream);

size_t benc_tab_words();
void benc_tab(size_t keys, const uint32_t* pk_ext, size_t stride, uint32_t* tab, hipStream_t stream);
void benc_mul(size_t keys, size_t n, size_t rows, const uint32_t* r, const uint32_t* tab, uint32_t* K_ext,
              size_t count, hipStream_t stream);
size_t bdec_mul_table_words(size_t keys, size_t n);
size_t bdec_launch_waves();
void bdec_mul(size_t keys, size_t n, const uint32_t* sk, const uint32_t* R_ext, uint32_t* K_ext, size_t count,
              uint32_t* table, hipStream_t stream);
void seat_dec_mul(size_t seats, size_t n, const uint32_t* sk, const uint32_t* R_ext, uint32_t* K_ext, size_t count,
                  uint32_t* table, hipStream_t stream);

size_t cmp_ladder_table_words(size_t cnt);
void cmp_ladder(size_t cnt, bool joint, const uint32_t* bp, const uint32_t* bq, const uint32_t* sa, const uint32_t* sb,
                const uint32_t* Pext, size_t pstride, uint32_t* T, uint32_t* out, hipStream_t stream);
void cmp_horner(size_t cnt, const uint32_t* list, const uint32_t* xs, const uint32_t* crow, const uint32_t* Eext,
                size_t stride, size_t N, int nb, uint32_t* R, hipStream_t stream);
void cv_prep(size_t C, const uint32_t* party, const uint32_t* pk, const uint32_t* enc, const uint32_t* proofs,
             uint32_t* Pc, uint32_t* rs, uint32_t* nc, uint32_t* p12, uint32_t* bp1, uint32_t* bp2, uint32_t* bq2,
             hipStream_t stream);
void cv_check(size_t C, const uint32_t* accuser, const uint32_t* p12, const uint32_t* ridx, const uint32_t* Rh,
              const uint32_t* Rt, const uint32_t* scale, const uint32_t* tab_g, const uint32_t* tab_h, uint8_t* eq,
              hipStream_t stream);
void cv_final(size_t C, const uint32_t* party, const uint32_t* crow, const uint32_t* pk, const uint32_t* enc,
              const uint32_t* proofs, const uint32_t* a1c, const uint32_t* a2c, const uint8_t* pok, const uint8_t* rowok,
              const uint8_t* fetched, const uint8_t* eq, int32_t* verdict, hipStream_t stream);
void cp_prep(size_t C, const uint32_t* sk, const uint32_t* enc, const uint32_t* w, uint32_t* Pc, uint32_t* ls,
             uint32_t* lb, uint32_t* gs, hipStream_t stream);
void cp_finish(size_t C, const uint32_t* enc, const uint32_t* lc, const uint32_t* gc, const uint32_t* gs,
               uint32_t* proofs, hipStream_t stream);
void qualified_complaints(size_t rows, size_t n, const uint8_t* dec, const uint8_t* cmask, uint8_t* rej, uint8_t* qmask,
                          hipStream_t stream);
void c3_prep(size_t C, size_t arows, const uint32_t* accuser, const uint32_t* crow, const uint32_t* share,
             const uint32_t* randomness, uint32_t* sr, uint32_t* acc2, uint32_t* acd2, hipStream_t stream);
void c3_check(size_t C, const uint32_t* accuser, const uint32_t* sr, const uint32_t* ridx, const uint32_t* Rh,
              const uint32_t* Rt, const uint32_t* scale, const uint32_t* tab_g, const uint32_t* tab_h, uint8_t* eq,
              hipStream_t stream);
void c3_final(size_t C, size_t arows, const uint32_t* crow, const uint32_t* drow, const uint8_t* rowok,
              const uint8_t* qualified, const uint8_t* fetched3, const uint8_t* eq, int32_t* verdict,
              hipStream_t stream);
void gather_rows(size_t R, size_t N, const uint32_t* rows, const uint32_t* srcE, const uint32_t* srcA, uint32_t* out,
                 hipStream_t stream);
void gather_enc(size_t C, size_t n, const uint32_t* drow, const uint32_t* accuser, const uint32_t* e1,
                const uint32_t* ct, uint32_t* enc, hipStream_t stream);
void proven_masks(size_t C2, size_t n, const uint32_t* drow2, const uint32_t* accuser2, const int32_t* verdict2,
                  size_t C4, const uint32_t* drow4, const int32_t* verdict4, uint8_t* cmask, uint8_t* pair,
                  uint8_t* proven4, hipStream_t stream);
void dissent_rows(size_t V, size_t n, const uint8_t* dec2, const uint8_t* pair, int32_t* dissent, hipStream_t stream);
void segment_mask(size_t D, int nseg, int seg, const uint8_t* dok, uint8_t* out, hipStream_t stream);
void shard_ridx(size_t C, int items, size_t D, size_t n, const uint32_t* lrow, const uint32_t* accuser,
                const uint8_t* rowok, uint32_t* ridx, hipStream_t stream);
void shard_flags(size_t D, size_t rows, const uint8_t* cmask, const uint8_t* proven4, const uint8_t* a_dec,
                 const uint8_t* fetched3, uint32_t* flags, hipStream_t stream);
void shard_dissent(size_t D, size_t n, const uint8_t* dec2, const uint8_t* pair, int32_t* dissent, hipStream_t stream);
void flag_masks(size_t n, const uint32_t* flags, uint8_t* cmask, uint8_t* proven4, uint8_t* a_ok, hipStream_t stream);
void sum_partials_i32(size_t ws, size_t n, const int32_t* in, int32_t* out, hipStream_t stream);

void interp(size_t D, size_t N, size_t nrecv, const uint32_t* WT, const uint32_t* s, const uint32_t* sp, uint32_t* F,
            uint32_t* Fp, hipStream_t stream);
void coef_check(size_t D, size_t N, const uint32_t* F, const uint32_t* Fp, const uint32_t* Eext, const uint32_t* Aext,
                size_t cstride, const uint32_t* tab_g, const uint32_t* tab_h, uint8_t* okE, uint8_t* okA,
                hipStream_t stream);
void interp_decide(size_t D, size_t nrecv, size_t N, size_t dealer_base, size_t nmod, const uint32_t* s,
                   const uint32_t* sp, const uint32_t* F, const uint32_t* Fp, const uint8_t* dokE, const uint8_t* dokA,
                   const uint8_t* cE, const uint8_t* cA, const uint32_t* tab_g, const uint32_t* tab_h, uint8_t* dec2,
                   uint8_t* dec4, hipStream_t stream);
void and_mask(size_t D, const uint8_t* extra, uint8_t* ok, hipStream_t stream);

void recv_chunks(size_t ndealers, size_t npad, size_t N, size_t L, const uint32_t* C, const uint32_t* xs, size_t m0,
                 size_t Ms, uint32_t* Q, uint32_t* R, hipStream_t stream);
void recv_fold(size_t ndealers, size_t npad, size_t Gin, size_t r, const uint32_t* in, const uint32_t* digits,
               size_t dstride, size_t m0, size_t Ms, uint32_t* out, uint32_t* R, hipStream_t stream);
void recv_decide(size_t M, size_t n, int round, const uint32_t* xs, const uint8_t* dok, const uint8_t* qualified,
                 uint8_t* dec, hipStream_t stream);
void recv_encode(size_t M, size_t D, const uint32_t* R, const uint8_t* dok, uint32_t* P, hipStream_t stream);
void pair_eval(size_t cnt, const uint32_t* list, const uint32_t* xs, const uint32_t* crow, const uint32_t* slot,
               const uint32_t* Eext, size_t stride, size_t N, uint32_t L, uint32_t G, uint32_t S,
               const uint32_t* digits, uint32_t* R, hipStream_t stream);
void seat_horner(size_t waves, size_t n, size_t N, size_t cols, uint32_t width, const uint32_t* wdesc,
                 const uint32_t* wseat, const uint32_t* scol, const uint32_t* C, uint32_t* R, hipStream_t stream);
void seat_chunks(size_t waves, size_t n, size_t N, size_t cols, uint32_t width, size_t L, const uint32_t* wdesc,
                 const uint32_t* wseat, const uint32_t* scol, const uint32_t* C, uint32_t* Q, hipStream_t stream);
void seat_fold(size_t waves, size_t n, uint32_t width, size_t Gin, const uint32_t* wdesc, const uint32_t* wseat,
               const uint32_t* xslot, const uint32_t* digits, size_t dstride, const uint32_t* in, uint32_t* out,
               uint32_t* R, hipStream_t stream);
void seat_ok(size_t S, size_t n, const uint32_t* scol, const uint8_t* dok, const uint8_t* extra, uint8_t* sok,
             hipStream_t stream);
void seat_decide(size_t S, size_t n, int round, const uint32_t* sx, const uint32_t* scer, const uint8_t* sok,
                 const uint8_t* qualified, uint8_t* dec, hipStream_t stream);
void pair_ok(size_t cnt, const uint32_t* crow, const uint8_t* rowok, uint8_t* ok, hipStream_t stream);

void commit_colsum(size_t n, size_t N, size_t r0, size_t rows, size_t spad, const uint32_t* C, const uint8_t* rowok,
                   const uint8_t* use, size_t bpad, uint32_t* Sacc, uint8_t* ok, hipStream_t stream);
void pubshare_out(size_t B, size_t M, const uint32_t* R, const uint32_t* G, uint32_t* V, hipStream_t stream);

}
```

### dkg_amd/csrc/runtime.hip

```cpp
#include <hip/hip_runtime.h>

#include <cstdio>
#include <cstdlib>
#include <cstring>
#include <algorithm>
#include <array>
#include <iterator>
#include <map>
#include <memory>
#include <optional>
#include <string>
#include <thread>
#include <unordered_map>
#include <unordered_set>
#include <vector>

#include "../../include/dkg_amd.h"
#include "host_crypto.h"
#include "kernels.h"
#include "kernels_ilp.h"
#include "comb_build.h"
#include "seat_finalise.h"
#include "seat_deal.h"

struct dkg_ctx {
  int device = 0;
  hipStream_t stream = nullptr;
  std::string err;
  std::map<std::string, std::pair<void*, size_t>> bufs;
  std::map<std::string, std::pair<void*, size_t>> hbufs;
  uint32_t* tab_g = nullptr;
  uint32_t* tab_h = nullptr;
  uint32_t* tab_gw = nullptr;
  uint32_t* tab_hw = nullptr;
  uint8_t h[32] = {0};
  bool have_h = false;
  size_t threshold = 0, nr_members = 0;
  hipEvent_t ev[8] = {};
  struct PhaseMark {
    const char* tag;
    int phase;
  };
  std::vector<hipEvent_t> phase_pool;
  std::vector<PhaseMark> phase_marks;
  int receiver_chunk = 0;
  int last_receiver_chunk = 0;
  size_t ps_slab = 0;
  std::map<std::array<size_t, 4>, dkg_receiver_plan> recv_plans;
  std::map<std::array<size_t, 3>, std::vector<uint32_t>> pair_digits;
  static constexpr int MAX_SUB = 8;
  int nsub = 2;
  hipStream_t sub[MAX_SUB] = {};
  hipEvent_t fork = nullptr, join[MAX_SUB] = {};
  hipStream_t side = nullptr;
  hipEvent_t side_fork = nullptr, shares_done = nullptr, pub_done = nullptr;
  hipEvent_t terms_done = nullptr;
  bool shares_pending = false;
  bool overlap = true;
  int split = 0;
  std::vector<uint8_t> key_tabs_pk;
  std::vector<uint8_t> key_tabs16_pk;
  int key_comb = 0;
  int last_key_comb = 0;
  int seat_deal = 0;
  int last_seat_deal = 0;
  int seat_eval = 0, seat_eval_chunk = 0;
  int last_seat_eval = 0, last_seat_eval_chunk = 0;
  uint8_t fb_base[32] = {0};
  bool fb_valid = false;
  int comb_build = 0;
  int last_comb_build = 0;
  hipEvent_t cb_ev[2] = {};
  int binom_mode = 0;
  int step_mode = 0;
  int check_mode = 0;
  int fe_mode = 0;
  int verify_mode = 0;
  size_t vinv_N = 0;
  size_t fallback_rows = 0;
  int last_split = 1;
  size_t last_split_len = 0;
  size_t ydig_n = 0, ydig_L = 0;
  int combine_mode = 0;
  int last_combine = 0;
  int last_binomial = 0;
  int step_formula = 0;
  uint32_t* last_step_flags = nullptr;
  size_t last_step_flag_words = 0;
  uint32_t* last_bflags = nullptr;
  size_t last_bflag_words = 0;
  bool binom_step_ded = false;
  uint32_t* binom_any = nullptr;
  const uint32_t* binom_any_host = nullptr;
  int last_binom_rerun = 0;
  int addend_mode = 0;
  size_t sdig_n = 0, sdig_L = 0, sdig_K = 0;
  int sdig_jsf = -1;
  const uint32_t* last_R = nullptr;
  const uint32_t* last_scale = nullptr;
  const uint8_t* last_dok = nullptr;
  int last_dok_nseg = 1;
  const uint8_t* last_pok = nullptr;
  size_t last_npad = 0;
  int complaint_eval = 0;
  int last_complaint_eval = 0;
  const uint32_t* ext_E = nullptr;
  const uint32_t* ext_A = nullptr;
  const uint32_t* r1_a = nullptr;
  const uint32_t* r1_b = nullptr;
  size_t r1_D = 0;
  uint32_t* r1_A0 = nullptr;
  size_t ext_stride = 0;
  const uint32_t* shard_s = nullptr;
  size_t shard_n = 0, shard_d0 = 0, shard_D = 0;
  size_t bfull_chunk = 0;
  std::map<std::string, double> phase_ms;
};

namespace {

constexpr size_t PTB = 160;
constexpr size_t PT_WORDS_H = 40;
constexpr size_t AFFP_WORDS_H = 32;
constexpr size_t COMB_BYTES = 30 * 512 * 4;
#ifndef DKG_COMBW_BITS
#define DKG_COMBW_BITS 19
#endif
constexpr size_t COMBW_BYTES =
    (size_t)(256 / DKG_COMBW_BITS + 1) * (1u << (DKG_COMBW_BITS - 1)) * 32 * 4;
const uint8_t BASEPOINT[32] = {0xe2, 0xf2, 0xae, 0x0a, 0x6a, 0xbc, 0x4e, 0x71, 0xa8, 0x84, 0xa9,
                               0x61, 0xc5, 0x00, 0x51, 0x5f, 0x58, 0xe3, 0x0b, 0x6a, 0xa5, 0x82,
                               0xdd, 0x8d, 0xb6, 0xa6, 0x59, 0x45, 0xe0, 0x8d, 0x2d, 0x76};

struct Fail {
  int code;
};

#define HCK(call)                                                                      \
  do {                                                                                 \
    hipError_t e_ = (call);                                                            \
    if (e_ != hipSuccess) {                                                            \
      ctx->err = std::string(#call) + ": " + hipGetErrorString(e_);                    \
      throw Fail{DKG_E_DEVICE};                                                        \
    }                                                                                  \
  } while (0)

template <typename T = void>
T* buf(dkg_ctx* ctx, const char* name, size_t bytes) {
  if (bytes == 0) bytes = 16;
  auto it = ctx->bufs.find(name);
  if (it != ctx->bufs.end() && it->second.second >= bytes) return reinterpret_cast<T*>(it->second.first);
  if (it != ctx->bufs.end()) {
    HCK(hipDeviceSynchronize());
    HCK(hipFree(it->second.first));
    ctx->bufs.erase(it);
  }
  void* p = nullptr;
  hipError_t e = hipMalloc(&p, bytes);
  if (e != hipSuccess) {
    ctx->err = std::string("hipMalloc(") + name + ", " + std::to_string(bytes) + "): " + hipGetErrorString(e);
    throw Fail{DKG_E_NOMEM};
  }
  ctx->bufs[name] = {p, bytes};
  return reinterpret_cast<T*>(p);
}

template <typename T = void>
T* hbuf(dkg_ctx* ctx, const char* name, size_t bytes) {
  if (bytes == 0) bytes = 16;
  auto it = ctx->hbufs.find(name);
  if (it != ctx->hbufs.end() && it->second.second >= bytes) return reinterpret_cast<T*>(it->second.first);
  if (it != ctx->hbufs.end()) {
    HCK(hipDeviceSynchronize());
    HCK(hipHostFree(it->second.first));
    ctx->hbufs.erase(it);
  }
  void* p = nullptr;
  hipError_t e = hipHostMalloc(&p, bytes, hipHostMallocDefault);
  if (e != hipSuccess) {
    ctx->err = std::string("hipHostMalloc(") + name + ", " + std::to_string(bytes) + "): " + hipGetErrorString(e);
    throw Fail{DKG_E_NOMEM};
  }
  ctx->hbufs[name] = {p, bytes};
  return reinterpret_cast<T*>(p);
}

void h2d(dkg_ctx* ctx, void* d, const void* h, size_t n) {
  if (n) HCK(hipMemcpyAsync(d, h, n, hipMemcpyHostToDevice, ctx->stream));
}
void d2h(dkg_ctx* ctx, void* h, const void* d, size_t n) {
  if (n) HCK(hipMemcpyAsync(h, d, n, hipMemcpyDeviceToHost, ctx->stream));
}
void sync(dkg_ctx* ctx) {
  HCK(hipStreamSynchronize(ctx->stream));
}
void check_launch(dkg_ctx* ctx) { HCK(hipGetLastError()); }

size_t pad64(size_t x) { return (x + 63) / 64 * 64; }

template <typename F>
int guarded(dkg_ctx* ctx, F&& f) {
  if (!ctx) return DKG_E_ARG;
  try {
    HCK(hipSetDevice(ctx->device));
    ctx->phase_marks.clear();
    int rc = f();
    return rc;
  } catch (const Fail& x) {
// ... 681 lines not shown
    Zl den = zero;
    for (size_t k = N; k-- > 0;) den = dkgh::zl_add(dkgh::zl_mul(den, xj), q[k]);
    const Zl scale = dkgh::zl_mul(dkgh::zl_inv(den), R);
    for (size_t k = 0; k < N; k++) {
      uint8_t b[33] = {0};
      dkgh::zl_to_bytes(b, dkgh::zl_mul(q[k], scale));
      for (size_t a = 0; a < 11; a++) {
        const size_t by = 3 * a;
        host[(j * 11 + a) * N + k] = (uint32_t)b[by] | (uint32_t)b[by + 1] << 8 | (uint32_t)b[by + 2] << 16;
      }
    }
  }
  h2d(ctx, dev, host.data(), 4 * host.size());
  ctx->vinv_N = N;
  return dev;
}

enum { IP_INTERPOLATE, IP_COEF_CHECK, IP_DECIDE, IP_FALLBACK };
const PhaseRow INTERP_PHASES[] = {{"interpolate", 1u << IP_INTERPOLATE}, {"coef_check", 1u << IP_COEF_CHECK},
                                  {"decide", 1u << IP_DECIDE}, {"fallback", 1u << IP_FALLBACK}};

template <typename F>
void verify_rounds_interp(dkg_ctx* ctx, size_t n, size_t t, size_t D, size_t dealer_base, const uint32_t* Ecomp,
                          const uint32_t* Acomp, const uint32_t* s, const uint32_t* sp, uint8_t* dec2, uint8_t* dec4,
                          hipEvent_t after2, F&& between, const uint8_t* e_ok, const uint8_t* a_ok) {
  const size_t N = t + 1;
  hipStream_t st = ctx->stream;
  if (D) {
    phase_mark(ctx, st, "interp", -1);
    const uint32_t *Ee, *Ae;
    size_t cs;
    uint8_t* dokE = buf<uint8_t>(ctx, "i.dokE", D);
    uint8_t* dokA = buf<uint8_t>(ctx, "i.dokA", D);
    if (ctx->ext_E) {
      Ee = ctx->ext_E;
      Ae = ctx->ext_A;
      cs = ctx->ext_stride;
      HCK(hipMemsetAsync(dokE, 1, D, st));
      HCK(hipMemsetAsync(dokA, 1, D, st));
    } else {
      uint32_t* ee = buf<uint32_t>(ctx, "i.Eext", PTB * D * N);
      uint32_t* ae = buf<uint32_t>(ctx, "i.Aext", PTB * D * N);
      uint8_t* pok = buf<uint8_t>(ctx, "i.pok", D * N);
      dkgk::decode_points(Ecomp, D * N, ee, D * N, pok, st);
      dkgk::dealer_ok(D, N, pok, dokE, st);
      dkgk::decode_points(Acomp, D * N, ae, D * N, pok, st);
      dkgk::dealer_ok(D, N, pok, dokA, st);
      Ee = ee;
      Ae = ae;
      cs = D * N;
    }
    dkgk::and_mask(D, e_ok, dokE, st);
    dkgk::and_mask(D, a_ok, dokA, st);
    const uint32_t* WT = vinv_table(ctx, N);
    uint32_t* Fa = buf<uint32_t>(ctx, "i.F", 32 * D * N);
    uint32_t* Fb = buf<uint32_t>(ctx, "i.Fp", 32 * D * N);
    dkgk::interp(D, N, n, WT, s, sp, Fa, Fb, st);
    phase_mark(ctx, st, "interp", IP_INTERPOLATE);
    uint8_t* okE = buf<uint8_t>(ctx, "i.okE", D * N);
    uint8_t* okA = buf<uint8_t>(ctx, "i.okA", D * N);
    dkgk::coef_check(D, N, Fa, Fb, Ee, Ae, cs, ctx->tab_gw, ctx->tab_hw, okE, okA, st);
    uint8_t* cE = buf<uint8_t>(ctx, "i.cE", D);
    uint8_t* cA = buf<uint8_t>(ctx, "i.cA", D);
    dkgk::dealer_ok(D, N, okE, cE, st);
    dkgk::dealer_ok(D, N, okA, cA, st);
    phase_mark(ctx, st, "interp", IP_COEF_CHECK);
    dkgk::interp_decide(D, n, N, dealer_base, n, s, sp, Fa, Fb, dokE, dokA, cE, cA, ctx->tab_gw, ctx->tab_hw, dec2,
                        dec4, st);
    phase_mark(ctx, st, "interp", IP_DECIDE);
    check_launch(ctx);
    std::vector<uint8_t> h_dE(D), h_dA(D), h_cE(D), h_cA(D);
    d2h(ctx, h_dE.data(), dokE, D);
    d2h(ctx, h_dA.data(), dokA, D);
    d2h(ctx, h_cE.data(), cE, D);
    d2h(ctx, h_cA.data(), cA, D);
    sync(ctx);
    std::vector<size_t> rows;
    for (size_t d = 0; d < D; d++)
      if ((h_dE[d] && !h_cE[d]) || (h_dA[d] && !h_cA[d])) rows.push_back(d);
    if (!rows.empty()) {
      const size_t R = rows.size();
      uint32_t* rs = buf<uint32_t>(ctx, "i.rs", 32 * R * n);
      uint32_t* rsp = buf<uint32_t>(ctx, "i.rsp", 32 * R * n);
      uint8_t* r2 = buf<uint8_t>(ctx, "i.r2", R * n);
      uint8_t* r4 = buf<uint8_t>(ctx, "i.r4", R * n);
      uint32_t *rE = nullptr, *rA = nullptr, *rEx = nullptr, *rAx = nullptr;
      if (ctx->ext_E) {
        rEx = buf<uint32_t>(ctx, "i.rEx", PTB * R * N);
        rAx = buf<uint32_t>(ctx, "i.rAx", PTB * R * N);
      } else {
        rE = buf<uint32_t>(ctx, "i.rE", 32 * R * N);
        rA = buf<uint32_t>(ctx, "i.rA", 32 * R * N);
      }
      for (size_t r = 0; r < R; r++) {
        const size_t d = rows[r];
        HCK(hipMemcpyAsync(rs + 8 * r * n, s + 8 * d * n, 32 * n, hipMemcpyDeviceToDevice, st));
        HCK(hipMemcpyAsync(rsp + 8 * r * n, sp + 8 * d * n, 32 * n, hipMemcpyDeviceToDevice, st));
        if (rEx) {
          HCK(hipMemcpy2DAsync(rEx + r * N, 4 * R * N, ctx->ext_E + d * N, 4 * ctx->ext_stride, 4 * N, PT_WORDS_H,
                               hipMemcpyDeviceToDevice, st));
          HCK(hipMemcpy2DAsync(rAx + r * N, 4 * R * N, ctx->ext_A + d * N, 4 * ctx->ext_stride, 4 * N, PT_WORDS_H,
                               hipMemcpyDeviceToDevice, st));
        } else {
          HCK(hipMemcpyAsync(rE + 8 * r * N, Ecomp + 8 * d * N, 32 * N, hipMemcpyDeviceToDevice, st));
          HCK(hipMemcpyAsync(rA + 8 * r * N, Acomp + 8 * d * N, 32 * N, hipMemcpyDeviceToDevice, st));
        }
      }
      const uint32_t *sE = ctx->ext_E, *sA = ctx->ext_A;
      const size_t sstr = ctx->ext_stride;
      if (rEx) {
        ctx->ext_E = rEx;
        ctx->ext_A = rAx;
        ctx->ext_stride = R * N;
      }
      VerifySeg g[2] = {{2, R, n, rE, rs, rsp, r2, nullptr, 2 * n + R}, {4, R, n, rA, rs, nullptr, r4, nullptr, 2 * n + R}};
      const bool ov = ctx->overlap;
      ctx->overlap = true;
      verify_device(ctx, n, t, g, 2, false, "");
      ctx->overlap = ov;
      ctx->ext_E = sE;
      ctx->ext_A = sA;
      ctx->ext_stride = sstr;
      for (size_t r = 0; r < R; r++) {
        const size_t d = rows[r], jself = (d + dealer_base) % n;
        if (h_dE[d] && !h_cE[d]) {
          HCK(hipMemcpyAsync(dec2 + d * n, r2 + r * n, n, hipMemcpyDeviceToDevice, st));
          HCK(hipMemsetAsync(dec2 + d * n + jself, DKG_SELF, 1, st));
        }
        if (h_dA[d] && !h_cA[d]) {
          HCK(hipMemcpyAsync(dec4 + d * n, r4 + r * n, n, hipMemcpyDeviceToDevice, st));
          HCK(hipMemsetAsync(dec4 + d * n + jself, DKG_SELF, 1, st));
        }
      }
      check_launch(ctx);
    }
    phase_mark(ctx, st, "interp", IP_FALLBACK);
    ctx->fallback_rows = rows.size();
  }
  if (after2) HCK(hipEventRecord(after2, st));
  sync(ctx);
  if (D) phase_collect(ctx, "interp", INTERP_PHASES, std::size(INTERP_PHASES));
  between();
}

template <typename F>
void verify_rounds(dkg_ctx* ctx, size_t n, size_t t, size_t D, size_t dealer_base, const uint32_t* Ecomp,
                   const uint32_t* Acomp, const uint32_t* s, const uint32_t* sp, uint8_t* dec2, uint8_t* dec4,
                   hipEvent_t after2, F&& between, const uint8_t* e_ok = nullptr, const uint8_t* a_ok = nullptr,
                   bool host_between = true) {
  ctx->last_step_flags = nullptr;
  ctx->last_step_flag_words = 0;
  ctx->last_bflags = nullptr;
  ctx->last_bflag_words = 0;
  ctx->binom_any = nullptr;
  ctx->binom_any_host = nullptr;
  if (ctx->binom_step_ded && DKG_BINOM_STEP_DED == 1) {
    ctx->binom_any = buf<uint32_t>(ctx, "v.bany", 4);
    HCK(hipMemsetAsync(ctx->binom_any, 0, 4, ctx->stream));
  }
  if (ctx->verify_mode == 1)
    verify_rounds_interp(ctx, n, t, D, dealer_base, Ecomp, Acomp, s, sp, dec2, dec4, after2, between, e_ok, a_ok);
  else
    verify_rounds_group(ctx, n, t, D, dealer_base, Ecomp, Acomp, s, sp, dec2, dec4, after2, between, e_ok, a_ok,
                        host_between);
}

void binom_mark_copy(dkg_ctx* ctx) {
  if (!ctx->binom_any) return;
  uint32_t* h = hbuf<uint32_t>(ctx, "bany.h", 4);
  d2h(ctx, h, ctx->binom_any, 4);
  ctx->binom_any_host = h;
}

bool binom_marked(dkg_ctx* ctx) {
  if (!ctx->binom_any) return false;
  uint32_t v = 0;
  if (ctx->binom_any_host)
    v = *ctx->binom_any_host;
  else
    HCK(hipMemcpy(&v, ctx->binom_any, 4, hipMemcpyDeviceToHost));
  return v != 0;
}

template <typename F>
void with_binom_ded(dkg_ctx* ctx, F&& f) {
  struct Off {
    dkg_ctx* c;
    ~Off() { c->binom_step_ded = false; }
  } off{ctx};
  ctx->binom_step_ded = true;
  ctx->last_binom_rerun = 0;
  f();
  ctx->binom_step_ded = false;
  if (binom_marked(ctx)) {
    ctx->last_binom_rerun = 1;
    f();
  }
}

double ev_ms(dkg_ctx* ctx, int a, int b) {
  float ms = 0;
  HCK(hipEventElapsedTime(&ms, ctx->ev[a], ctx->ev[b]));
  return ms;
}

std::vector<dkgh::Zl> lagrange_zero_coeffs(size_t n, const uint8_t* in_set) {
  using namespace dkgh;
  const Zl zero = zl_from_u64(0), one = zl_from_u64(1);
  std::vector<Zl> fact(n + 1), ifact(n + 1), lam(n, zero);
  fact[0] = one;
  for (size_t k = 1; k <= n; k++) fact[k] = zl_mul(fact[k - 1], zl_from_u64(k));
  ifact[n] = zl_inv(fact[n]);
  for (size_t k = n; k > 0; k--) ifact[k - 1] = zl_mul(ifact[k], zl_from_u64(k));
  Zl P = one;
  std::vector<size_t> outside;
  for (size_t j = 0; j < n; j++) {
    if (in_set[j]) P = zl_mul(P, zl_from_u64(j + 1));
    else outside.push_back(j);
  }
  for (size_t j = 0; j < n; j++) {
    if (!in_set[j]) continue;
    Zl v = zl_mul(P, zl_mul(ifact[j + 1], ifact[n - 1 - j]));
    for (size_t e : outside) v = zl_mul(v, zl_sub(zl_from_u64(e + 1), zl_from_u64(j + 1)));
    lam[j] = (j & 1) ? zl_sub(zero, v) : v;
  }
  return lam;
}

dkgh::Zl lagrange_dot(const std::vector<dkgh::Zl>& lam, const uint8_t* ys, size_t n) {
  dkgh::Zl acc = dkgh::zl_from_u64(0);
  for (size_t j = 0; j < n; j++)
    if (!dkgh::zl_is_zero(lam[j])) acc = dkgh::zl_add(acc, dkgh::zl_mul(lam[j], dkgh::zl_from_bits(ys + 32 * j)));
  return acc;
}

std::vector<uint8_t> final_parties(size_t n, const uint8_t* qualified, const uint8_t* recon) {
  std::vector<uint8_t> f(n);
  for (size_t j = 0; j < n; j++) f[j] = qualified[j] && !recon[j];
  return f;
}

std::vector<uint8_t> disclosing_parties(size_t n, const uint8_t* qualified, const uint8_t* recon, const uint8_t* r2err,
                                        const uint8_t* r4err) {
  std::vector<uint8_t> f = final_parties(n, qualified, recon);
  for (size_t j = 0; j < n; j++) f[j] = f[j] && !(r2err && r2err[j]) && !(r4err && r4err[j]);
  return f;
}

bool recovery_fails(const std::vector<uint8_t>& S, size_t t) {
  size_t c = 0;
  for (auto v : S) c += v != 0;
  return c < t;
}

std::vector<uint8_t> recon_secrets(size_t n, const std::vector<uint8_t>& fin, const uint8_t* hs,
                                   const std::vector<size_t>& rows) {
  const std::vector<dkgh::Zl> lam = lagrange_zero_coeffs(n, fin.data());
  std::vector<uint8_t> secrets(32 * rows.size());
  for (size_t r = 0; r < rows.size(); r++) dkgh::zl_to_bytes(&secrets[32 * r], lagrange_dot(lam, hs + 32 * n * rows[r], n));
  return secrets;
}

void round2_device(dkg_ctx* ctx, size_t groups, size_t n, const uint8_t* dec2, uint8_t* qmask, uint8_t* rej,
                   int32_t* cnt, const uint8_t* cmask = nullptr) {
  dkgk::decision_summary(groups, n, dec2, rej, cnt, ctx->stream);
  if (cmask) dkgk::qualified_complaints(groups * n, n, dec2, cmask, rej, qmask, ctx->stream);
  else dkgk::mask_not_and(groups * n, rej, nullptr, qmask, ctx->stream);
}
void round2_host(size_t V, size_t t, uint8_t* qualified, const int32_t* complaints, uint8_t* r2err) {
  for (size_t i = 0; i < V; i++) {
    qualified[i] = !qualified[i];
    r2err[i] = complaints[i] > (int32_t)t;
  }
}
void round4_device(dkg_ctx* ctx, size_t groups, size_t n, size_t t, uint8_t* dec4, const uint8_t* qmask,
                   uint8_t* rej, uint8_t* r4d) {
  dkgk::decision_summary(groups, n, dec4, rej, nullptr, ctx->stream);
  if (r4d) dkgk::r4_error(groups, n, t, dec4, qmask, r4d, ctx->stream);
  dkgk::apply_skipped(groups, n, dec4, qmask, ctx->stream);
}
void round4_host(size_t V, const uint8_t* qualified, uint8_t* recon) {
  for (size_t i = 0; i < V; i++) recon[i] = qualified[i] && recon[i];
}

struct RoundMasks {
  const uint8_t *e_ok = nullptr, *a_ok = nullptr, *cmask = nullptr, *proven4 = nullptr;
};
struct RoundsResult {
  std::vector<uint8_t> qualified, reconstruct, r2_error, r4_error;
  int32_t n_qualified = 0;
  bool phase4_error = false;
};
RoundsResult receivers_rounds_once(dkg_ctx* ctx, size_t n, size_t t, const uint32_t* Ecomp, const uint32_t* Acomp,
                                   const uint32_t* s, const uint32_t* sp, dkg_ceremony_out* out, bool copy_big,
                                   const RoundMasks& m) {
  const size_t N = t + 1;
  uint8_t* dec2 = buf<uint8_t>(ctx, "dec2", n * n);
  uint8_t* dec4 = buf<uint8_t>(ctx, "dec4", n * n);
  uint32_t* fs = buf<uint32_t>(ctx, "final_share", 32 * n);
  uint32_t* pubc = buf<uint32_t>(ctx, "pub_comp", 32 * n);
  uint8_t* qmask = buf<uint8_t>(ctx, "qmask", n);
  uint8_t* rej2 = buf<uint8_t>(ctx, "o.rej2", n);
  int32_t* cnt = buf<int32_t>(ctx, "o.cnt", 4 * n);
  auto round3 = [&] {
    wait_shares(ctx, ctx->stream);
    round2_device(ctx, 1, n, dec2, qmask, rej2, cnt, m.cmask);
    dkgk::sum_shares(n, n, s, qmask, fs, ctx->stream);
    uint32_t* pub = buf<uint32_t>(ctx, "pub_ext", PTB * n);
    HCK(hipEventRecord(ctx->side_fork, ctx->stream));
    HCK(hipStreamWaitEvent(ctx->side, ctx->side_fork, 0));
    dkgk::fixed_base(n, fs, ctx->tab_gw, pub, ctx->side);
    dkgk::encode_points(pub, n, n, pubc, ctx->side);
    HCK(hipEventRecord(ctx->pub_done, ctx->side));
    HCK(hipEventRecord(ctx->ev[3], ctx->stream));
  };
  verify_rounds(ctx, n, t, n, 0, Ecomp, Acomp, s, sp, dec2, dec4, ctx->ev[2], round3, m.e_ok, m.a_ok, false);
  wait_shares(ctx, ctx->stream);
  ctx->shares_pending = false;
  uint8_t* rej4 = buf<uint8_t>(ctx, "o.rej4", n);
  uint8_t* r4d = buf<uint8_t>(ctx, "o.r4err", n);
  round4_device(ctx, 1, n, t, dec4, qmask, rej4, r4d);
  const uint8_t* acc4 = m.proven4 ? m.proven4 : rej4;
  HCK(hipEventRecord(ctx->ev[4], ctx->stream));
  uint32_t* A0 = buf<uint32_t>(ctx, "A0ext", PTB * n);
  if (ctx->ext_A) {
    dkgk::gather_points(ctx->ext_A, ctx->ext_stride, N, 0, n, A0, n, ctx->stream);
  } else {
    uint32_t* A0c = buf<uint32_t>(ctx, "A0c", 32 * n);
    HCK(hipMemcpy2DAsync(A0c, 32, Acomp, 32 * N, 32, n, hipMemcpyDeviceToDevice, ctx->stream));
    uint8_t* a0ok = buf<uint8_t>(ctx, "A0ok", n);
    dkgk::decode_points(A0c, n, A0, n, a0ok, ctx->stream);
  }
  uint8_t* hmask = buf<uint8_t>(ctx, "hmask", n);
  dkgk::mask_not_and(n, acc4, qmask, hmask, ctx->stream);
  uint32_t* mpk_ext = buf<uint32_t>(ctx, "mpk_ext", PTB);
  dkgk::sum_points(n, A0, n, hmask, mpk_ext, 1, 0, ctx->stream);
  uint32_t* mpk_c = buf<uint32_t>(ctx, "mpk_comp", 32);
  dkgk::encode_points(mpk_ext, 1, 1, mpk_c, ctx->stream);
  check_launch(ctx);
  uint8_t* h = hbuf<uint8_t>(ctx, "rr.out", 8 * n + 32);
  d2h(ctx, h, rej2, n);
  d2h(ctx, h + n, acc4, n);
  d2h(ctx, h + 2 * n, r4d, n);
  d2h(ctx, h + 3 * n, cnt, 4 * n);
  d2h(ctx, h + 7 * n, mpk_c, 32);
  HCK(hipEventRecord(ctx->ev[5], ctx->stream));
  HCK(hipStreamWaitEvent(ctx->stream, ctx->pub_done, 0));
  if (copy_big) {
    if (out->dec2) d2h(ctx, out->dec2, dec2, n * n);
    if (out->dec4) d2h(ctx, out->dec4, dec4, n * n);
    if (out->final_share) d2h(ctx, out->final_share, fs, 32 * n);
    if (out->public_share) d2h(ctx, out->public_share, pubc, 32 * n);
  }
  binom_mark_copy(ctx);
  sync(ctx);
  collect_verify_phases(ctx);
  std::vector<uint8_t> qualified(h, h + n), r2err(n), recon(h + n, h + 2 * n), r4e(h + 2 * n, h + 3 * n);
  std::vector<int32_t> complaints(n);
  memcpy(complaints.data(), h + 3 * n, 4 * n);
  round2_host(n, t, qualified.data(), complaints.data(), r2err.data());
  round4_host(n, qualified.data(), recon.data());
  const std::vector<uint8_t> disc = disclosing_parties(n, qualified.data(), recon.data(), r2err.data(), r4e.data());
  size_t nrecon = 0;
  int32_t nq = 0;
  for (size_t i = 0; i < n; i++) {
    nrecon += recon[i];
    nq += qualified[i];
  }
  const bool phase4_error = nq - (int32_t)nrecon <= (int32_t)t;
  memset(out->mpk, 0, 32);
  if (!phase4_error && !(nrecon && recovery_fails(disc, t))) {
    if (nrecon) {
      std::vector<size_t> rows;
      std::vector<uint8_t> hs(32 * n * nrecon);
      for (size_t i = 0; i < n; i++)
        if (recon[i]) {
          d2h(ctx, &hs[32 * n * rows.size()], s + 8 * n * i, 32 * n);
          rows.push_back(rows.size());
        }
      sync(ctx);
      std::vector<uint8_t> secrets = recon_secrets(n, disc, hs.data(), rows);
      uint32_t* sec = buf<uint32_t>(ctx, "recon_sec", 32 * nrecon);
      h2d(ctx, sec, secrets.data(), secrets.size());
      uint32_t* gsec = buf<uint32_t>(ctx, "recon_ext", PTB * nrecon);
      uint32_t* extra = buf<uint32_t>(ctx, "recon_sum", PTB);
      dkgk::fixed_base(nrecon, sec, ctx->tab_gw, gsec, ctx->stream);
      dkgk::sum_points(nrecon, gsec, nrecon, nullptr, extra, 1, 0, ctx->stream);
      dkgk::add_points(1, mpk_ext, extra, 1, mpk_ext, ctx->stream);
      dkgk::encode_points(mpk_ext, 1, 1, mpk_c, ctx->stream);
      check_launch(ctx);
      d2h(ctx, h + 7 * n, mpk_c, 32);
      sync(ctx);
    }
    memcpy(out->mpk, h + 7 * n, 32);
  }
  if (out->qualified) memcpy(out->qualified, qualified.data(), n);
  if (out->r2_error) memcpy(out->r2_error, r2err.data(), n);
  if (out->r4_error) memcpy(out->r4_error, r4e.data(), n);
  if (out->complaints2) memcpy(out->complaints2, complaints.data(), 4 * n);
  if (out->reconstruct) memcpy(out->reconstruct, recon.data(), n);
  out->n_qualified = nq;
  out->phase4_error = phase4_error;
  return {std::move(qualified), std::move(recon), std::move(r2err), std::move(r4e), nq, phase4_error};
}

RoundsResult receivers_rounds(dkg_ctx* ctx, size_t n, size_t t, const uint32_t* Ecomp, const uint32_t* Acomp,
                              const uint32_t* s, const uint32_t* sp, dkg_ceremony_out* out, bool copy_big,
                              const RoundMasks& m = {}) {
  RoundsResult r;
  with_binom_ded(ctx, [&] { r = receivers_rounds_once(ctx, n, t, Ecomp, Acomp, s, sp, out, copy_big, m); });
  return r;
}

struct Commitments {
  uint32_t *E, *A;
};
Commitments commitment_rows(dkg_ctx* ctx, size_t n, size_t N) {
  uint32_t* EA = buf<uint32_t>(ctx, "cer_EA", 32 * 2 * n * N);
  return {EA, EA + 8 * n * N};
}
Commitments upload_commitments(dkg_ctx* ctx, size_t n, size_t N, const uint8_t* E, const uint8_t* A) {
  const Commitments c = commitment_rows(ctx, n, N);
  h2d(ctx, c.E, E, 32 * n * N);
  h2d(ctx, c.A, A, 32 * n * N);
  return c;
}

void ceremony_times(dkg_ctx* ctx, dkg_ceremony_out* out, bool round1) {
  out->ms_round1 = round1 ? ev_ms(ctx, 0, 1) : 0.0;
  out->ms_round2 = ev_ms(ctx, 1, 2);
  out->ms_round3 = ev_ms(ctx, 2, 3);
  out->ms_round4 = ev_ms(ctx, 3, 4);
  out->ms_finalise = ev_ms(ctx, 4, 5);
  out->ms_total = ev_ms(ctx, 0, 5);
}

void round1_device(dkg_ctx* ctx, size_t D, size_t n, size_t t, const uint32_t* a, const uint32_t* b,
                   uint32_t* Ecomp, uint32_t* Acomp, uint32_t* s, uint32_t* sp, bool encode = true,
                   bool overlap_shares = false) {
  const size_t N = t + 1;
  uint32_t* Aext = buf<uint32_t>(ctx, "Aext", PTB * D * N);
  uint32_t* Eext = buf<uint32_t>(ctx, "Eext", PTB * D * N);
  if (overlap_shares) {
    HCK(hipEventRecord(ctx->side_fork, ctx->stream));
    HCK(hipStreamWaitEvent(ctx->side, ctx->side_fork, 0));
  }
  dkgk::commit(D * N, a, b, ctx->tab_gw, ctx->tab_hw, Aext, Eext, ctx->stream);
  if (encode) {
    dkgk::encode_points(Eext, D * N, D * N, Ecomp, ctx->stream);
    dkgk::encode_points(Aext, D * N, D * N, Acomp, ctx->stream);
  }
  if (overlap_shares) {
    dkgk::share_eval(D, n, N, a, b, s, sp, ctx->side);
    HCK(hipEventRecord(ctx->shares_done, ctx->side));
    ctx->shares_pending = true;
  } else {
    dkgk::share_eval(D, n, N, a, b, s, sp, ctx->stream);
  }
  check_launch(ctx);
}


struct SharesScope {
  dkg_ctx* ctx;
  explicit SharesScope(dkg_ctx* c) : ctx(c) {}
  ~SharesScope() {
    if (ctx->shares_pending) (void)hipStreamWaitEvent(ctx->stream, ctx->shares_done, 0);
    ctx->shares_pending = false;
  }
};

struct ExtScope {
  dkg_ctx* ctx;
  ExtScope(dkg_ctx* c, size_t D, size_t N) : ctx(c) {
    ctx->ext_E = buf<uint32_t>(ctx, "Eext", PTB * D * N);
    ctx->ext_A = buf<uint32_t>(ctx, "Aext", PTB * D * N);
    ctx->ext_stride = D * N;
  }
  ~ExtScope() {
    ctx->ext_E = ctx->ext_A = nullptr;
    ctx->ext_stride = 0;
  }
};

struct BatchRound1 {
  dkg_ctx* ctx;
  BatchRound1(dkg_ctx* c, size_t D, size_t n, size_t t, const uint32_t* a, const uint32_t* b, uint32_t* s,
              uint32_t* sp)
      : ctx(c) {
    const size_t N = t + 1;
    if (deferred()) {
// ... 1013 lines not shown
      HCK(hipEventRecord(ctx->side_fork, ctx->stream));
      HCK(hipStreamWaitEvent(ctx->side, ctx->side_fork, 0));
    }
    decrypt_device(ctx, n, n, dsk, de1, dct, rs, rsp, iok, eok, side ? ctx->side : ctx->stream);
    if (side) {
      HCK(hipEventRecord(ctx->shares_done, ctx->side));
      ctx->shares_pending = true;
    }
    ds = rs, dsp = rsp;
    m.e_ok = eok;
  }
  const RoundsResult r = receivers_rounds(ctx, n, t, cm.E, cm.A, ds, dsp, out, true, m);
  if (full) {
    phase_collect(ctx, "full", FULL_PHASES, std::size(FULL_PHASES));
    if (out->s) d2h(ctx, out->s, ds, 32 * n * n);
    if (out->s_prime) d2h(ctx, out->s_prime, dsp, 32 * n * n);
    sync(ctx);
  }
  ceremony_times(ctx, out, false);
  if (in.c4) proven_outcome(n, t, *in.c4, a_ok.data(), r, out->mpk);
  if (in.c2 && in.c2->dissent)
    complaint_dissent(ctx, n, in.c2->C, in.c2->accuser, in.c2->accused, in.c2->verdict, in.c2->dissent);
  return DKG_OK;
}

struct BatchInput {
  const uint8_t *E = nullptr, *A = nullptr;
  const uint8_t *s = nullptr, *s_prime = nullptr;
  const uint8_t *e1 = nullptr, *ct = nullptr, *sk = nullptr;
  const uint8_t *fetched1 = nullptr, *fetched3 = nullptr;
  const BatchComplaints2* c2 = nullptr;
  const BatchComplaints4* c4 = nullptr;
  uint8_t *s_out = nullptr, *s_prime_out = nullptr;
};

int verify_batch(dkg_ctx* ctx, size_t B, size_t n, size_t t, const BatchInput& in, dkg_batch_out* out) {
  const size_t N = t + 1, V = B * n, items = 2 * V * n;
  const bool full = in.e1 != nullptr;
  BatchDevice d;
  uint32_t* Ec = buf<uint32_t>(ctx, "bat_E", 32 * V * N);
  uint32_t* Ac = buf<uint32_t>(ctx, "bat_A", 32 * V * N);
  h2d(ctx, Ec, in.E, 32 * V * N);
  h2d(ctx, Ac, in.A, 32 * V * N);
  d.E = Ec, d.A = Ac;
  if (full) {
    d.sk = upload_scalars(ctx, "bfm_sk", in.sk, V);
    uint32_t* de1 = buf<uint32_t>(ctx, "bfm_e1", 32 * items);
    uint32_t* dct = buf<uint32_t>(ctx, "bfm_ct", 32 * items);
    h2d(ctx, de1, in.e1, 32 * items);
    h2d(ctx, dct, in.ct, 32 * items);
    d.e1 = de1, d.ct = dct;
  } else {
    d.s = upload_scalars(ctx, "bat_s", in.s, V * n);
    d.s_prime = upload_scalars(ctx, "bat_sp", in.s_prime, V * n);
  }
  d.fetched1 = upload_mask(ctx, "bp.f1", in.fetched1, V);
  d.fetched3 = upload_mask(ctx, "bp.f3", in.fetched3, V);
  BatchProven bp;
  if (in.c4) batch_complaints(ctx, B, n, t, d, full ? in.c2 : nullptr, *in.c4, bp);
  HCK(hipEventRecord(ctx->ev[0], ctx->stream));
  HCK(hipEventRecord(ctx->ev[1], ctx->stream));
  const uint8_t* e_ok = d.fetched1;
  if (full) {
    uint32_t* rs = buf<uint32_t>(ctx, "bfm_s", 32 * V * n);
    uint32_t* rsp = buf<uint32_t>(ctx, "bfm_sp", 32 * V * n);
    uint8_t* iok = buf<uint8_t>(ctx, "bfm_iok", items);
    uint8_t* eok = buf<uint8_t>(ctx, "bfm_eok", V);
    decrypt_batch_device(ctx, B, n, d.sk, d.e1, d.ct, rs, rsp, iok, eok);
    d.s = rs, d.s_prime = rsp;
    e_ok = eok;
  }
  batch_receivers(ctx, B, n, t, d.E, d.A, d.s, d.s_prime, out, e_ok, in.c4 ? &bp : nullptr);
  if (full) phase_collect(ctx, "bfull", BF_ROWS, BF_PHASES);
  if (in.c4) batch_proven_outcome(ctx, B, n, t, *in.c4, bp, out);
  if (full) {
    if (in.s_out) d2h(ctx, in.s_out, d.s, 32 * V * n);
    if (in.s_prime_out) d2h(ctx, in.s_prime_out, d.s_prime, 32 * V * n);
    sync(ctx);
  }
  batch_times(ctx, out, false);
  return DKG_OK;
}

int batch_keys_status(dkg_ctx* ctx, const uint8_t* ok, size_t V) {
  for (size_t k = 0; k < V; k++)
    if (!ok[k]) {
      ctx->err = "encrypt_shares_batch: a recipient public key does not decode";
      return DKG_E_DECODE;
    }
  return DKG_OK;
}

}

__global__ __launch_bounds__(256) void k_clock_probe(unsigned iters, unsigned long long* out) {
  uint32_t x = threadIdx.x * 2654435761u + blockIdx.x;
  const unsigned long long c0 = clock64(), r0 = wall_clock64();
  for (unsigned i = 0; i < iters; i++) x = x * 1664525u + 1013904223u;
  asm volatile("" : "+v"(x));
  const unsigned long long c1 = clock64(), r1 = wall_clock64();
  const size_t w = (size_t)blockIdx.x * (blockDim.x / 64) + threadIdx.x / 64;
  if ((threadIdx.x & 63) == 0) {
    out[2 * w] = (c1 - c0) + (x == 0xffffffffu ? 1 : 0);
    out[2 * w + 1] = r1 - r0;
  }
}

extern "C" {

int dkg_device_count(void) {
  int n = 0;
  if (hipGetDeviceCount(&n) != hipSuccess) return 0;
  return n;
}

int dkg_device_pci_bus_id(int device, char* buf, int len) {
  if (!buf || len < 13) return DKG_E_ARG;
  return hipDeviceGetPCIBusId(buf, len, device) == hipSuccess ? DKG_OK : DKG_E_DEVICE;
}

int dkg_ctx_clock_probe(dkg_ctx* ctx, unsigned iters, double* sclk_mhz, double* busy_ms) {
  return guarded(ctx, [&] {
    if (!sclk_mhz || !busy_ms || !iters) return DKG_E_ARG;
    int cus = 0, wall_khz = 0;
    HCK(hipDeviceGetAttribute(&cus, hipDeviceAttributeMultiprocessorCount, ctx->device));
    HCK(hipDeviceGetAttribute(&wall_khz, hipDeviceAttributeWallClockRate, ctx->device));
    if (cus <= 0 || wall_khz <= 0) return DKG_E_DEVICE;
    const size_t waves = (size_t)cus * 16;
    unsigned long long* d = buf<unsigned long long>(ctx, "clock_probe", 2 * 8 * waves);
    hipLaunchKernelGGL(k_clock_probe, dim3((unsigned)(waves / 4)), dim3(256), 0, ctx->stream, iters, d);
    check_launch(ctx);
    std::vector<unsigned long long> h(2 * waves);
    d2h(ctx, h.data(), d, 2 * 8 * waves);
    sync(ctx);
    std::vector<double> mhz(waves), ms(waves);
    for (size_t w = 0; w < waves; w++) {
      const double real_us = (double)h[2 * w + 1] / wall_khz * 1e3;
      mhz[w] = real_us > 0 ? (double)h[2 * w] / real_us : 0.0;
      ms[w] = real_us / 1e3;
    }
    std::nth_element(mhz.begin(), mhz.begin() + waves / 2, mhz.end());
    std::nth_element(ms.begin(), ms.begin() + waves / 2, ms.end());
    *sclk_mhz = mhz[waves / 2];
    *busy_ms = ms[waves / 2];
    return DKG_OK;
  });
}

int dkg_ctx_create(int device, dkg_ctx** out) {
  if (!out) return DKG_E_ARG;
  *out = nullptr;
  dkg_ctx* ctx = new dkg_ctx();
  ctx->device = device;
  int rc = guarded(ctx, [&] {
    int least = 0, greatest = 0;
    HCK(hipDeviceGetStreamPriorityRange(&least, &greatest));
    HCK(hipStreamCreateWithPriority(&ctx->stream, hipStreamNonBlocking, greatest));
    for (auto& e : ctx->ev) HCK(hipEventCreate(&e));
    ctx->phase_pool.resize(PHASE_POOL_MIN);
    for (auto& e : ctx->phase_pool) HCK(hipEventCreate(&e));
    for (auto& e : ctx->cb_ev) HCK(hipEventCreate(&e));
    for (auto& st : ctx->sub) HCK(hipStreamCreateWithPriority(&st, hipStreamNonBlocking, greatest));
    HCK(hipStreamCreateWithPriority(&ctx->side, hipStreamNonBlocking, least));
    HCK(hipEventCreateWithFlags(&ctx->side_fork, hipEventDisableTiming));
    HCK(hipEventCreateWithFlags(&ctx->shares_done, hipEventDisableTiming));
    HCK(hipEventCreateWithFlags(&ctx->pub_done, hipEventDisableTiming));
    HCK(hipEventCreateWithFlags(&ctx->terms_done, hipEventDisableTiming));
    HCK(hipEventCreateWithFlags(&ctx->fork, hipEventDisableTiming));
    for (auto& e : ctx->join) HCK(hipEventCreateWithFlags(&e, hipEventDisableTiming));
    HCK(hipMalloc(&ctx->tab_g, COMB_BYTES));
    HCK(hipMalloc(&ctx->tab_h, COMB_BYTES));
    HCK(hipMalloc(&ctx->tab_gw, COMBW_BYTES));
    HCK(hipMalloc(&ctx->tab_hw, COMBW_BYTES));
    bool ok = false;
    comb_for_point(ctx, BASEPOINT, ctx->tab_g, &ok, ctx->tab_gw);
    if (!ok) {
      ctx->err = "basepoint failed to decode on device";
      return DKG_E_DEVICE;
    }
    return DKG_OK;
  });
  if (rc != DKG_OK) {
    fprintf(stderr, "dkg_ctx_create: %s\n", ctx->err.c_str());
    dkg_ctx_destroy(ctx);
    return rc;
  }
  *out = ctx;
  return DKG_OK;
}

void dkg_ctx_destroy(dkg_ctx* ctx) {
  if (!ctx) return;
  (void)hipSetDevice(ctx->device);
  if (ctx->stream) (void)hipDeviceSynchronize();
  for (auto& kv : ctx->bufs) (void)hipFree(kv.second.first);
  for (auto& kv : ctx->hbufs) (void)hipHostFree(kv.second.first);
  if (ctx->tab_g) (void)hipFree(ctx->tab_g);
  if (ctx->tab_h) (void)hipFree(ctx->tab_h);
  if (ctx->tab_gw) (void)hipFree(ctx->tab_gw);
  if (ctx->tab_hw) (void)hipFree(ctx->tab_hw);
  for (auto& e : ctx->ev)
    if (e) (void)hipEventDestroy(e);
  for (auto& e : ctx->phase_pool)
    if (e) (void)hipEventDestroy(e);
  for (auto& e : ctx->cb_ev)
    if (e) (void)hipEventDestroy(e);
  for (auto& e : ctx->join)
    if (e) (void)hipEventDestroy(e);
  if (ctx->fork) (void)hipEventDestroy(ctx->fork);
  for (auto& st : ctx->sub)
    if (st) (void)hipStreamDestroy(st);
  if (ctx->stream) (void)hipStreamDestroy(ctx->stream);
  if (ctx->side) (void)hipStreamDestroy(ctx->side);
  if (ctx->side_fork) (void)hipEventDestroy(ctx->side_fork);
  if (ctx->shares_done) (void)hipEventDestroy(ctx->shares_done);
  if (ctx->pub_done) (void)hipEventDestroy(ctx->pub_done);
  if (ctx->terms_done) (void)hipEventDestroy(ctx->terms_done);
  delete ctx;
}

const char* dkg_ctx_last_error(const dkg_ctx* ctx) { return ctx ? ctx->err.c_str() : "null context"; }

double dkg_ctx_phase_ms(const dkg_ctx* ctx, const char* name) {
  if (!ctx || !name) return -1.0;
  auto it = ctx->phase_ms.find(name);
  return it == ctx->phase_ms.end() ? -1.0 : it->second;
}

int dkg_ctx_set_streams(dkg_ctx* ctx, int nsub) {
  if (!ctx || nsub < 1 || nsub > dkg_ctx::MAX_SUB) return DKG_E_ARG;
  ctx->nsub = nsub;
  return DKG_OK;
}

int dkg_ctx_set_verify_mode(dkg_ctx* ctx, int mode) {
  if (!ctx || mode < 0 || mode > 1) return DKG_E_ARG;
  ctx->verify_mode = mode;
  return DKG_OK;
}

size_t dkg_ctx_fallback_rows(const dkg_ctx* ctx) { return ctx ? ctx->fallback_rows : 0; }

int dkg_ctx_set_split(dkg_ctx* ctx, int pieces) {
  if (!ctx || pieces < 0 || pieces > 16) return DKG_E_ARG;
  ctx->split = pieces;
  return DKG_OK;
}

int dkg_ctx_set_binomial(dkg_ctx* ctx, int mode) {
  if (!ctx || mode < 0 || mode > 5) return DKG_E_ARG;
  ctx->binom_mode = mode;
  return DKG_OK;
}

int dkg_ctx_set_check(dkg_ctx* ctx, int mode) {
  if (!ctx || mode < 0 || mode > 1) return DKG_E_ARG;
  ctx->check_mode = mode;
  return DKG_OK;
}

int dkg_ctx_set_field_mode(dkg_ctx* ctx, int mode) {
  if (!ctx || mode < 0 || mode > 2) return DKG_E_ARG;
  ctx->fe_mode = mode;
  return DKG_OK;
}

int dkg_ctx_set_stepping(dkg_ctx* ctx, int mode) {
  if (!ctx || mode < 0 || mode > 3) return DKG_E_ARG;
  ctx->step_mode = mode;
  return DKG_OK;
}

int dkg_ctx_last_split(const dkg_ctx* ctx) { return ctx ? ctx->last_split : 0; }
size_t dkg_ctx_last_split_len(const dkg_ctx* ctx) { return ctx ? ctx->last_split_len : 0; }
int dkg_ctx_set_combine(dkg_ctx* ctx, int mode) {
  if (!ctx || mode < 0 || mode > 3) return DKG_E_ARG;
  ctx->combine_mode = mode;
  return DKG_OK;
}
int dkg_ctx_last_combine(const dkg_ctx* ctx) { return ctx ? ctx->last_combine : 0; }
int dkg_ctx_last_binomial(const dkg_ctx* ctx) { return ctx ? ctx->last_binomial : 0; }
int dkg_ctx_set_stepping_formula(dkg_ctx* ctx, int mode) {
  if (!ctx || mode < 0 || mode > 1) return DKG_E_ARG;
  ctx->step_formula = mode;
  return DKG_OK;
}
long long dkg_ctx_stepping_redos(dkg_ctx* ctx) {
  if (!ctx) return -1;
  if (!ctx->last_step_flags) return 0;
  try {
    std::vector<uint32_t> h(ctx->last_step_flag_words);
    sync(ctx);
    HCK(hipMemcpy(h.data(), ctx->last_step_flags, 4 * h.size(), hipMemcpyDeviceToHost));
    long long c = 0;
    for (uint32_t x : h) c += x != 0;
    return c;
  } catch (const Fail& f) {
    return -1;
  }
}
int dkg_ctx_binomial_reruns(dkg_ctx* ctx) { return ctx ? ctx->last_binom_rerun : -1; }
long long dkg_ctx_binomial_wave_redos(dkg_ctx* ctx) {
  if (!ctx) return -1;
  if (!ctx->last_bflags) return 0;
  try {
    std::vector<uint32_t> h(ctx->last_bflag_words);
    sync(ctx);
    HCK(hipMemcpy(h.data(), ctx->last_bflags, 4 * h.size(), hipMemcpyDeviceToHost));
    long long c = 0;
    for (uint32_t x : h) c += x != 0;
    return c;
  } catch (const Fail& f) {
    return -1;
  }
}
int dkg_ctx_set_addends(dkg_ctx* ctx, int mode) {
  if (!ctx || mode < 0 || mode > 1) return DKG_E_ARG;
  ctx->addend_mode = mode;
  return DKG_OK;
}
int dkg_split_multipliers(size_t n, size_t L, int pieces, uint8_t* mag, int8_t* sign) {
  if (!n || !L || pieces < 2 || pieces > (int)SHORT_MAX || !mag || !sign) return DKG_E_ARG;
  try {
    std::vector<uint8_t> m;
    std::vector<int8_t> sg;
    short_vectors(n, L, (size_t)pieces, m, sg, jsf_built((size_t)pieces));
    memcpy(mag, m.data(), m.size());
    memcpy(sign, sg.data(), sg.size());
  } catch (const std::exception&) {
    return DKG_E_NOMEM;
  }
  return DKG_OK;
}
int dkg_jsf_digits(const uint8_t a[32], const uint8_t b[32], int8_t da[256], int8_t db[256], int16_t* top) {
  if (!a || !b || !da || !db || !top) return DKG_E_ARG;
  return dkgh::jsf_digits(a, b, da, db, top) ? DKG_OK : DKG_E_ARG;
}
int dkg_seat_enc_digits(const uint8_t k[32], int8_t digits[128], int* windows) {
  if (!k || !digits || !windows || (k[31] & 0x80)) return DKG_E_ARG;
  uint32_t w[8];
  for (int i = 0; i < 8; i++)
    w[i] = (uint32_t)k[4 * i] | (uint32_t)k[4 * i + 1] << 8 | (uint32_t)k[4 * i + 2] << 16 | (uint32_t)k[4 * i + 3] << 24;
  int carry = 0;
  for (int win = 0; win < dkgk::SEAT_ENC_WINDOWS; win++)
    digits[win] = (int8_t)dkgk::seat_enc_digit(dkgk::seat_enc_bits(w[win >> 4], win), win, carry);
  *windows = dkgk::SEAT_ENC_WINDOWS;
  return DKG_OK;
}
int dkg_split_digits(size_t n, size_t L, int pieces, int mode, int8_t* digits, int16_t* top) {
  if (!n || !L || pieces < 2 || pieces > (int)SHORT_MAX || mode < 0 || mode > 3 || mode == 1 || !digits || !top)
    return DKG_E_ARG;
  try {
    const size_t K = (size_t)pieces;
    const bool jsf = mode != 3 && jsf_built(K);
    std::vector<uint8_t> m;
    std::vector<int8_t> sg;
    short_vectors(n, L, K, m, sg, jsf);
    std::vector<uint32_t> hd;
    std::vector<int16_t> ht;
    if (!short_digit_words(n, K, jsf, m, sg, hd, ht, nullptr)) return DKG_E_ARG;
    for (size_t j = 0; j < n; j++) {
      top[j] = ht[j];
      for (size_t u = 0; u < K; u++)
        for (size_t b = 0; b < 256; b++)
          digits[(j * K + u) * 256 + b] = (int8_t)(hd[(u / 4) * 256 * n + 256 * j + b] >> (8 * (u % 4)));
    }
  } catch (const std::exception&) {
    return DKG_E_NOMEM;
  }
  return DKG_OK;
}

double dkg_split_model_ms(size_t columns, size_t n, size_t t, int pieces) {
  if (pieces < 1 || t + 1 < (size_t)pieces) return -1;
  return split_model_ms(columns, n, t + 1, (size_t)pieces);
}

int dkg_stepping_lane_map(int lanes, int seg_len, int nseg, int last_len, int lane, int out[3]) {
  if (lanes <= 0 || lanes % 64 || lanes > 512 || lane < 0 || lane >= lanes || !out) return -1;
  const int B = step_band(lanes, seg_len, nseg, last_len);
  if (!B) return 0;
  const StepLane m = step_band_lane(lane, B, lanes);
  out[0] = m.seg, out[1] = m.q, out[2] = m.next;
  return B;
}

size_t dkg_split_len(size_t columns, size_t n, size_t t, int pieces) {
  if (pieces < 1 || t + 1 < (size_t)pieces) return 0;
  return split_len(columns, n, t + 1, (size_t)pieces);
}

int dkg_ctx_set_overlap(dkg_ctx* ctx, int on) {
  if (!ctx) return DKG_E_ARG;
  ctx->overlap = on != 0;
  return DKG_OK;
}

int dkg_env_check(size_t threshold, size_t nr_members) {
  if (nr_members == 0 || !(threshold < (nr_members + 1) / 2)) return DKG_E_ARG;
  return DKG_OK;
}

int dkg_env_init(dkg_ctx* ctx, size_t threshold, size_t nr_members, const uint8_t* ck, size_t ck_len,
                 uint8_t h_out[32]) {
  int rc = dkg_env_check(threshold, nr_members);
  if (rc != DKG_OK) {
    if (ctx) ctx->err = "threshold must be < (nr_members + 1) / 2 (committee.rs:73)";
    return rc;
  }
  return guarded(ctx, [&] {
    uint8_t hash[64];
    dkgh::blake2b(hash, 64, ck, ck_len);
    uint32_t* in = buf<uint32_t>(ctx, "h_in", 64);
    uint32_t* ext = buf<uint32_t>(ctx, "h_ext", PTB);
    uint32_t* comp = buf<uint32_t>(ctx, "h_comp", 32);
    h2d(ctx, in, hash, 64);
    dkgk::from_uniform(in, ext, ctx->stream);
    dkgk::encode_points(ext, 1, 1, comp, ctx->stream);
    check_launch(ctx);
    d2h(ctx, ctx->h, comp, 32);
    sync(ctx);
    bool ok = false;
    comb_for_point(ctx, ctx->h, ctx->tab_h, &ok, ctx->tab_hw);
    if (!ok) return DKG_E_DEVICE;
    ctx->have_h = true;
    ctx->threshold = threshold;
    ctx->nr_members = nr_members;
    if (h_out) memcpy(h_out, ctx->h, 32);
    return DKG_OK;
  });
}

int dkg_msm_batch(dkg_ctx* ctx, size_t B, size_t N, const uint8_t* scalars, const uint8_t* points, uint8_t* out) {
  return guarded(ctx, [&] {
    if (B == 0) return DKG_OK;
    uint32_t* sc = upload_scalars(ctx, "msm_sc", scalars, B * N);
    uint32_t* pc = buf<uint32_t>(ctx, "msm_pc", 32 * B * N);
    uint32_t* pe = buf<uint32_t>(ctx, "msm_pe", PTB * B * N);
    uint8_t* ok = buf<uint8_t>(ctx, "msm_ok", B * N);
    h2d(ctx, pc, points, 32 * B * N);
    dkgk::decode_points(pc, B * N, pe, B * N, ok, ctx->stream);
    uint32_t* oe = buf<uint32_t>(ctx, "msm_oe", PTB * B);
    uint32_t* oc = buf<uint32_t>(ctx, "msm_oc", 32 * B);
    uint32_t* mt = buf<uint32_t>(ctx, "msm_tab", 4 * 15 * PT_WORDS_H * B * N);
  dkgk::msm_batch(B, N, sc, pe, B * N, mt, oe, ctx->stream);
    dkgk::encode_points(oe, B, B, oc, ctx->stream);
    check_launch(ctx);
    std::vector<uint8_t> okh(B * N);
    d2h(ctx, okh.data(), ok, B * N);
// ... 3258 lines not shown
```

### include/dkg_amd.h

```cpp
#ifndef DKG_AMD_H
#define DKG_AMD_H
#include <stddef.h>
#include <stdint.h>

#ifdef __cplusplus
extern "C" {
#endif

#define DKG_OK 0
#define DKG_E_ARG (-1)
#define DKG_E_DECODE (-2)
#define DKG_E_DEVICE (-3)
#define DKG_E_NOMEM (-4)

#define DKG_REJECT 0
#define DKG_ACCEPT 1
#define DKG_SELF 2
#define DKG_SKIPPED 3
#define DKG_MISSING 4

typedef struct dkg_ctx dkg_ctx;

int dkg_ctx_create(int device, dkg_ctx **out);
void dkg_ctx_destroy(dkg_ctx *ctx);
const char *dkg_ctx_last_error(const dkg_ctx *ctx);
double dkg_ctx_phase_ms(const dkg_ctx *ctx, const char *name);
int dkg_ctx_set_streams(dkg_ctx *ctx, int nsub);
int dkg_ctx_set_overlap(dkg_ctx *ctx, int on);
int dkg_ctx_set_split(dkg_ctx *ctx, int pieces);
int dkg_ctx_set_stepping(dkg_ctx *ctx, int mode);
int dkg_ctx_set_field_mode(dkg_ctx *ctx, int mode);
int dkg_ctx_set_binomial(dkg_ctx *ctx, int mode);
int dkg_ctx_set_check(dkg_ctx *ctx, int mode);
int dkg_ctx_set_verify_mode(dkg_ctx *ctx, int mode);
size_t dkg_ctx_fallback_rows(const dkg_ctx *ctx);
int dkg_ctx_last_split(const dkg_ctx *ctx);
size_t dkg_ctx_last_split_len(const dkg_ctx *ctx);
double dkg_split_model_ms(size_t columns, size_t n, size_t t, int pieces);
size_t dkg_split_len(size_t columns, size_t n, size_t t, int pieces);
int dkg_ctx_set_combine(dkg_ctx *ctx, int mode);
int dkg_ctx_last_combine(const dkg_ctx *ctx);
int dkg_ctx_last_binomial(const dkg_ctx *ctx);
int dkg_ctx_set_addends(dkg_ctx *ctx, int mode);
int dkg_ctx_set_stepping_formula(dkg_ctx *ctx, int mode);
long long dkg_ctx_stepping_redos(dkg_ctx *ctx);
int dkg_zero_tests(dkg_ctx *ctx, size_t count, const uint32_t *limbs, uint8_t *out);
int dkg_fe_ops(dkg_ctx *ctx, int flavour, int op, size_t count, const uint32_t *in, uint32_t *out);
int dkg_sc_ops(dkg_ctx *ctx, int op, size_t count, const uint32_t *in, uint32_t *out);
int dkg_stepping_lane_map(int lanes, int seg_len, int nseg, int last_len, int lane, int out[3]);
int dkg_ctx_binomial_reruns(dkg_ctx *ctx);
long long dkg_ctx_binomial_wave_redos(dkg_ctx *ctx);
int dkg_split_multipliers(size_t n, size_t L, int pieces, uint8_t *mag, int8_t *sign);
int dkg_jsf_digits(const uint8_t a[32], const uint8_t b[32], int8_t da[256], int8_t db[256], int16_t *top);
int dkg_split_digits(size_t n, size_t L, int pieces, int mode, int8_t *digits, int16_t *top);
int dkg_device_count(void);
int dkg_ctx_clock_probe(dkg_ctx *ctx, unsigned iters, double *sclk_mhz, double *busy_ms);
int dkg_device_pci_bus_id(int device, char *buf, int len);

int dkg_env_init(dkg_ctx *ctx, size_t threshold, size_t nr_members, const uint8_t *ck_bytes, size_t ck_len,
                 uint8_t h_out[32]);
int dkg_env_check(size_t threshold, size_t nr_members);

int dkg_msm_batch(dkg_ctx *ctx, size_t B, size_t N, const uint8_t *scalars, const uint8_t *points, uint8_t *out);
int dkg_fixed_base_batch(dkg_ctx *ctx, const uint8_t base[32], size_t count, const uint8_t *scalars, uint8_t *out);
int dkg_poly_eval_batch(dkg_ctx *ctx, size_t D, size_t N, const uint8_t *coeffs, size_t M, const uint32_t *xs,
                        uint8_t *out);
int dkg_points_valid_batch(dkg_ctx *ctx, size_t count, const uint8_t *points, uint8_t *ok);

int dkg_share_gen(dkg_ctx *ctx, size_t D, size_t n, size_t t, const uint8_t *a, const uint8_t *b, uint8_t *E,
                  uint8_t *A, uint8_t *s, uint8_t *s_prime);
int dkg_share_gen_device(dkg_ctx *ctx, size_t D, size_t n, size_t t, const void *d_a, const void *d_b, void *d_E,
                         void *d_A, void *d_s, void *d_s_prime);

int dkg_verify_pairs(dkg_ctx *ctx, size_t n, size_t t, int round, size_t d0, size_t d1, const uint8_t *C,
                     const uint8_t *s, const uint8_t *s_prime, uint8_t *decision);
int dkg_verify_receiver(dkg_ctx *ctx, size_t n, size_t t, int round, size_t j, const uint8_t *C, const uint8_t *s,
                        const uint8_t *s_prime, uint8_t *decision);

typedef struct {
  uint32_t chunk;
  uint32_t stages;
  uint32_t arity[16];
  uint8_t mult[16][32];
} dkg_receiver_plan;
int dkg_receiver_plan_for(size_t n, size_t t, uint32_t x, int chunk, dkg_receiver_plan *out);
double dkg_receiver_plan_cost_us(size_t n, size_t t, uint32_t x, const dkg_receiver_plan *p);
void dkg_receiver_plan_constants(double c[5]);
int dkg_ctx_set_receiver_chunk(dkg_ctx *ctx, int chunk);
int dkg_ctx_last_receiver_chunk(const dkg_ctx *ctx);
int dkg_commitment_eval(dkg_ctx *ctx, size_t D, size_t t, size_t M, const uint32_t *js, const uint8_t *C,
                        uint8_t *P, uint8_t *ok);
int dkg_pair_eval_shape(size_t t, int chunk, uint32_t *L, uint32_t *lanes, uint32_t *stages);
int dkg_commitment_eval_pairs(dkg_ctx *ctx, size_t D, size_t t, size_t count, const uint32_t *rows,
                              const uint32_t *js, const uint8_t *C, uint8_t *P, uint8_t *ok);
int dkg_verify_receivers(dkg_ctx *ctx, size_t n, size_t t, int round, size_t M, const uint32_t *js, const uint8_t *C,
                         const uint8_t *s, const uint8_t *s_prime, const uint8_t *qualified, uint8_t *decision);
int dkg_party_round2(dkg_ctx *ctx, size_t n, size_t t, size_t j, const uint8_t *E, const uint8_t *e1, const uint8_t *ct,
                     const uint8_t sk[32], const uint8_t *w, uint8_t *s_out, uint8_t *sp_out, uint8_t *dec,
                     int32_t *complaints, uint8_t *r2_error, uint8_t *proofs);

int dkg_seat_pack(size_t n, size_t S, const uint32_t *js, uint32_t *width, uint32_t *per_wave, uint32_t *tiles,
                  uint32_t *wave_of, uint32_t *slot_of, uint32_t *waves);
int dkg_commitment_eval_seats(dkg_ctx *ctx, size_t B, size_t n, size_t t, size_t S, const uint32_t *cer,
                              const uint32_t *js, const uint8_t *C, uint8_t *P, uint8_t *ok);
int dkg_verify_seats(dkg_ctx *ctx, size_t B, size_t n, size_t t, int round, size_t S, const uint32_t *cer,
                     const uint32_t *js, const uint8_t *C, const uint8_t *s, const uint8_t *s_prime,
                     const uint8_t *qualified, uint8_t *decision);
int dkg_party_round2_seats(dkg_ctx *ctx, size_t B, size_t n, size_t t, size_t S, const uint32_t *cer,
                           const uint32_t *js, const uint8_t *E, const uint8_t *e1, const uint8_t *ct,
                           const uint8_t *sk, const uint8_t *w, uint8_t *s_out, uint8_t *sp_out, uint8_t *dec,
                           int32_t *complaints, uint8_t *r2_error, uint8_t *proofs);
int dkg_seat_eval_shape(size_t n, size_t t, size_t waves, uint32_t x_max, int chunk, uint32_t *L, uint32_t *G,
                        uint32_t *stages, uint64_t *scratch_bytes);
void dkg_seat_eval_constants(double c[6]);
int dkg_ctx_set_seat_eval(dkg_ctx *ctx, int mode, int chunk);
int dkg_ctx_last_seat_eval(const dkg_ctx *ctx, int *chunk);

int dkg_party_round1_seats(dkg_ctx *ctx, size_t B, size_t n, size_t t, size_t S, const uint32_t *cer,
                           const uint32_t *js, const uint8_t *a, const uint8_t *b, const uint8_t *r,
                           const uint8_t *pk, uint8_t *E, uint8_t *A, uint8_t *e1, uint8_t *ct, uint8_t *s_out,
                           uint8_t *sp_out, uint8_t *own);
int dkg_ctx_set_seat_deal(dkg_ctx *ctx, int mode);
int dkg_ctx_last_seat_deal(const dkg_ctx *ctx);
int dkg_seat_enc_digits(const uint8_t k[32], int8_t digits[128], int *windows);

int dkg_complaints_verify_ceremonies(dkg_ctx *ctx, size_t B, size_t n, size_t t, size_t C, const uint32_t *ceremony,
                                     const uint32_t *accuser, const uint32_t *accused, const uint8_t *pk,
                                     const uint8_t *E, const uint8_t *fetched1, const uint8_t *enc,
                                     const uint8_t *proofs, int32_t *verdict, uint8_t *qualified);
int dkg_complaints3_verify_ceremonies(dkg_ctx *ctx, size_t B, size_t n, size_t t, size_t C, const uint32_t *ceremony,
                                      const uint32_t *accuser, const uint32_t *accused, const uint8_t *share,
                                      const uint8_t *randomness, const uint8_t *E, const uint8_t *A,
                                      const uint8_t *qualified, const uint8_t *fetched3, int32_t *verdict,
                                      uint8_t *reconstruct);
int dkg_party_round3_seats(dkg_ctx *ctx, size_t B, size_t n, size_t t, size_t S, const uint32_t *cer,
                           const uint32_t *js, const uint8_t *qualified, const uint8_t *s, uint8_t *final_share,
                           uint8_t *public_share);
int dkg_finalise_seats(dkg_ctx *ctx, size_t B, size_t n, size_t t, size_t S, const uint32_t *cer, const uint32_t *js,
                       const uint8_t *qualified, const uint8_t *reconstruct, const uint8_t *fetched3,
                       const uint8_t *r2_error, const uint8_t *r4_error, const uint8_t *A0, const uint8_t *s,
                       size_t D5, const uint32_t *d_ceremony, const uint32_t *d_sender, const uint32_t *d_dealer,
                       const uint8_t *d_share, uint8_t *mpk, int32_t *status, int32_t *recovery_index);
int dkg_seat_finalise_status(size_t n, size_t t, size_t p, const uint8_t *qualified, const uint8_t *reconstruct,
                             const uint8_t *a_present, const uint32_t *points, int r2_error, int r4_error,
                             int32_t *recovery_index);

#define DKG_PS_OK 0
#define DKG_PS_NO_COMMITMENT 1
#define DKG_PS_NO_DISCLOSURE 2
int dkg_commitment_sum(dkg_ctx *ctx, size_t B, size_t n, size_t t, const uint8_t *A, const uint8_t *mask, uint8_t *S,
                       uint8_t *ok);
int dkg_public_shares(dkg_ctx *ctx, size_t B, size_t n, size_t t, const uint8_t *A, const uint8_t *qualified,
                      const uint8_t *reconstruct, const uint8_t *fetched3, size_t M, const uint32_t *js, size_t D5,
                      const uint32_t *d_ceremony, const uint32_t *d_sender, const uint32_t *d_dealer,
                      const uint8_t *d_share, uint8_t *V, int32_t *status, int32_t *which, uint8_t *S);
int dkg_public_share_status(size_t n, const uint8_t *qualified, const uint8_t *reconstruct, const uint8_t *a_present,
                            uint32_t j, size_t D5, const uint32_t *d_sender, const uint32_t *d_dealer,
                            int32_t *which);
int dkg_ctx_set_public_share_slab(dkg_ctx *ctx, size_t rows);

typedef struct {
  uint8_t *E, *A;
  uint8_t *s, *s_prime;
  uint8_t *dec2, *dec4;
  uint8_t *qualified;
  uint8_t *r2_error;
  uint8_t *r4_error;
  int32_t *complaints2;
  uint8_t *reconstruct;
  uint8_t *final_share;
  uint8_t *public_share;
  uint8_t mpk[32];
  int32_t n_qualified;
  int32_t phase4_error;
  double ms_round1, ms_round2, ms_round3, ms_round4, ms_finalise, ms_total;
} dkg_ceremony_out;

int dkg_ceremony_run(dkg_ctx *ctx, size_t n, size_t t, const uint8_t *a, const uint8_t *b, dkg_ceremony_out *out);
int dkg_ceremony_verify(dkg_ctx *ctx, size_t n, size_t t, const uint8_t *E, const uint8_t *A, const uint8_t *s,
                        const uint8_t *s_prime, dkg_ceremony_out *out);
int dkg_ceremony_verify_fetched(dkg_ctx *ctx, size_t n, size_t t, const uint8_t *E, const uint8_t *A,
                                const uint8_t *s, const uint8_t *s_prime, const uint8_t *fetched1,
                                const uint8_t *fetched3, dkg_ceremony_out *out);
int dkg_ceremony_run_device(dkg_ctx *ctx, size_t n, size_t t, const void *d_a, const void *d_b,
                            dkg_ceremony_out *out);
int dkg_ceremony_shard_device(dkg_ctx *ctx, size_t n, size_t t, size_t d0, size_t d1, const void *d_a,
                              const void *d_b, void *d_dec2, void *d_dec4, void *d_A0, void *d_partial,
                              double *ms_total);
int dkg_ceremony_shard_verify_device(dkg_ctx *ctx, size_t n, size_t t, size_t d0, size_t d1, const void *d_E,
                                     const void *d_A, const void *d_s, const void *d_s_prime, void *d_dec2,
                                     void *d_dec4, void *d_A0, void *d_partial, double *ms_total);
int dkg_ceremony_shard_full_device(dkg_ctx *ctx, size_t n, size_t t, size_t d0, size_t d1, const void *d_a,
                                   const void *d_b, const void *d_r, const uint8_t *sk, const uint8_t *pk, void *d_e1,
                                   void *d_ct, void *d_dec2, void *d_dec4, void *d_A0, void *d_partial,
                                   double *ms_total);
int dkg_ceremony_shard_verify_full_device(dkg_ctx *ctx, size_t n, size_t t, size_t d0, size_t d1, const void *d_E,
                                          const void *d_A, const void *d_e1, const void *d_ct, const uint8_t *sk,
                                          void *d_dec2, void *d_dec4, void *d_A0, void *d_partial, double *ms_total);
// ... 226 lines not shown
```

Baseline: 13.57 million verified shares/s.

## Speculate all-honest finalise tail on side stream, skip recompute when confirmed

Starts the finalise tail (share sums, public-key fixed-base, encoding, A0 gather, master public key sum) on the side stream before round-2/4 results are known, assuming every dealer is qualified. Device-side all_equal checks confirm the assumption, and the masked recompute kernels read a skip flag and exit early when it holds. This takes tail work off the critical path by overlapping it with the round checks. The cost is extra launches and duplicated work whenever a dealer is misbehaving, plus more cross-stream event ordering.

```diff
diff --git a/dkg_amd/_lib.py b/dkg_amd/_lib.py
--- a/dkg_amd/_lib.py
+++ b/dkg_amd/_lib.py
@@ -110,6 +110,9 @@
     L.dkg_ctx_set_stepping_formula.argtypes = [p, ctypes.c_int]
     L.dkg_ctx_stepping_redos.argtypes = [p]
     L.dkg_ctx_stepping_redos.restype = ctypes.c_longlong
+    if hasattr(L, "dkg_ctx_last_tail_speculated"):
+        L.dkg_ctx_last_tail_speculated.argtypes = [p]
+        L.dkg_ctx_set_tail_spec.argtypes = [p, ctypes.c_int]
     L.dkg_ctx_binomial_reruns.argtypes = [p]
     L.dkg_ctx_binomial_wave_redos.argtypes = [p]
     L.dkg_ctx_binomial_wave_redos.restype = ctypes.c_longlong
@@ -296,7 +299,7 @@
     "dkg_env_check", "dkg_msm_batch", "dkg_fixed_base_batch", "dkg_poly_eval_batch",
     "dkg_points_valid_batch", "dkg_share_gen", "dkg_verify_pairs", "dkg_verify_receiver",
     "dkg_ctx_set_split", "dkg_ctx_set_stepping", "dkg_ctx_set_field_mode", "dkg_ctx_set_binomial", "dkg_ctx_set_check", "dkg_ctx_last_split", "dkg_ctx_last_split_len", "dkg_ctx_set_verify_mode", "dkg_ctx_fallback_rows", "dkg_split_model_ms", "dkg_split_len",
-    "dkg_ctx_set_combine", "dkg_ctx_last_combine", "dkg_ctx_last_binomial", "dkg_ctx_set_addends", "dkg_ctx_set_stepping_formula", "dkg_ctx_stepping_redos", "dkg_zero_tests", "dkg_fe_ops", "dkg_sc_ops", "dkg_stepping_lane_map", "dkg_ctx_binomial_reruns", "dkg_ctx_binomial_wave_redos", "dkg_split_multipliers", "dkg_jsf_digits", "dkg_split_digits",
+    "dkg_ctx_set_combine", "dkg_ctx_last_combine", "dkg_ctx_last_binomial", "dkg_ctx_set_addends", "dkg_ctx_set_stepping_formula", "dkg_ctx_stepping_redos", "dkg_ctx_last_tail_speculated", "dkg_ctx_set_tail_spec", "dkg_zero_tests", "dkg_fe_ops", "dkg_sc_ops", "dkg_stepping_lane_map", "dkg_ctx_binomial_reruns", "dkg_ctx_binomial_wave_redos", "dkg_split_multipliers", "dkg_jsf_digits", "dkg_split_digits",
     "dkg_ctx_clock_probe", "dkg_device_pci_bus_id",
     "dkg_ceremony_run", "dkg_ceremony_verify", "dkg_ceremony_verify_fetched", "dkg_ceremony_run_device", "dkg_ceremony_shard_device",
     "dkg_ceremony_shard_verify_device",
diff --git a/dkg_amd/api.py b/dkg_amd/api.py
--- a/dkg_amd/api.py
+++ b/dkg_amd/api.py
@@ -166,6 +166,15 @@
         if r < 0:
             raise DkgError(_lib.DKG_E_DEVICE, "dkg_ctx_stepping_redos failed")
         return r
+
+    def last_tail_speculated(self) -> int:
+        r = _lib.lib().dkg_ctx_last_tail_speculated(self._ctx)
+        if r < 0:
+            raise DkgError(_lib.DKG_E_DEVICE, "dkg_ctx_last_tail_speculated failed")
+        return r
+
+    def set_tail_spec(self, on: bool):
+        _check(self._ctx, _lib.lib().dkg_ctx_set_tail_spec(self._ctx, 1 if on else 0))
 
     def zero_tests(self, limbs) -> list:
         count = len(limbs)
diff --git a/dkg_amd/csrc/kernels.hip b/dkg_amd/csrc/kernels.hip
--- a/dkg_amd/csrc/kernels.hip
+++ b/dkg_amd/csrc/kernels.hip
@@ -94,7 +94,9 @@
 #endif
 #if DKG_ENCODE_PAIR
 __global__ __launch_bounds__(256, DKG_ENCODE_WAVES) void k_encode(const uint32_t* __restrict__ ext, size_t stride,
-                                                size_t count, uint32_t* __restrict__ comp) {
+                                                size_t count, uint32_t* __restrict__ comp,
+                                                const uint32_t* __restrict__ skip) {
+  if (skip && *skip) return;
   const size_t half = (count + 1) / 2;
   const size_t e0 = (size_t)blockIdx.x * blockDim.x + threadIdx.x;
   if (e0 >= half) return;
@@ -126,7 +128,9 @@
 }
 #else
 __global__ __launch_bounds__(256, DKG_ENCODE_WAVES) void k_encode(const uint32_t* __restrict__ ext, size_t stride,
-                                                size_t count, uint32_t* __restrict__ comp) {
+                                                size_t count, uint32_t* __restrict__ comp,
+                                                const uint32_t* __restrict__ skip) {
+  if (skip && *skip) return;
   size_t e = (size_t)blockIdx.x * blockDim.x + threadIdx.x;
   if (e >= count) return;
   fe u1, u2, t, inv, one;
@@ -164,11 +168,12 @@
                      L * npad, ok, N, npad, (uint32_t)nseg, (uint32_t)seg, L, pstride);
 }
 
-void encode_points(const uint32_t* ext, size_t stride, size_t count, uint32_t* comp, hipStream_t stream) {
+void encode_points(const uint32_t* ext, size_t stride, size_t count, uint32_t* comp, hipStream_t stream,
+                   const uint32_t* skip) {
   if (!count) return;
   const size_t lanes = DKG_ENCODE_PAIR ? (count + 1) / 2 : count;
   hipLaunchKernelGGL(k_encode, dim3((unsigned)((lanes + 255) / 256)), dim3(256), 0, stream, ext, stride,
-                     count, comp);
+                     count, comp, skip);
 }
 
 __global__ __launch_bounds__(64) void k_build_comb(const uint32_t* __restrict__ ext, size_t stride, size_t e0,
@@ -2172,14 +2177,33 @@
 }
 
 __global__ __launch_bounds__(256) void k_mask_not_and(size_t V, const uint8_t* __restrict__ a,
-                                                      const uint8_t* __restrict__ b, uint8_t* __restrict__ out) {
+                                                      const uint8_t* __restrict__ b, uint8_t* __restrict__ out,
+                                                      const uint32_t* __restrict__ skip) {
+  if (skip && *skip) return;
   const size_t i = (size_t)blockIdx.x * 256 + threadIdx.x;
   if (i < V) out[i] = !a[i] && (!b || b[i]);
 }
 
-void mask_not_and(size_t V, const uint8_t* a, const uint8_t* b, uint8_t* out, hipStream_t stream) {
+void mask_not_and(size_t V, const uint8_t* a, const uint8_t* b, uint8_t* out, hipStream_t stream,
+                  const uint32_t* skip) {
   if (!V) return;
-  hipLaunchKernelGGL(k_mask_not_and, dim3((unsigned)((V + 255) / 256)), dim3(256), 0, stream, V, a, b, out);
+  hipLaunchKernelGGL(k_mask_not_and, dim3((unsigned)((V + 255) / 256)), dim3(256), 0, stream, V, a, b, out, skip);
+}
+
+__global__ __launch_bounds__(256) void k_all_equal(size_t V, const uint8_t* __restrict__ a, uint32_t want,
+                                                   const uint32_t* __restrict__ prev, uint32_t* __restrict__ out) {
+  __shared__ uint32_t bad;
+  if (threadIdx.x == 0) bad = prev && !*prev;
+  __syncthreads();
+  uint32_t mine = 0;
+  for (size_t i = threadIdx.x; i < V; i += 256) mine |= a[i] != want;
+  if (mine) bad = 1;
+  __syncthreads();
+  if (threadIdx.x == 0) *out = !bad;
+}
+
+void all_equal(size_t V, const uint8_t* a, uint32_t want, const uint32_t* prev, uint32_t* out, hipStream_t stream) {
+  hipLaunchKernelGGL(k_all_equal, dim3(1), dim3(256), 0, stream, V, a, want, prev, out);
 }
 
 void dealer_ok(size_t ndealers, size_t N, const uint8_t* point_ok, uint8_t* ok, hipStream_t stream) {
@@ -2215,7 +2239,8 @@
 
 __global__ __launch_bounds__(256) void k_sum_points(size_t count, const uint32_t* __restrict__ pts, size_t stride,
                                                     const uint8_t* __restrict__ mask, uint32_t* __restrict__ out,
-                                                    size_t ostride, size_t col) {
+                                                    size_t ostride, size_t col, const uint32_t* __restrict__ skip) {
+  if (skip && *skip) return;
   __shared__ uint32_t red[256][PT_WORDS];
   ge_p3 acc;
   ge_identity(acc);
@@ -2252,10 +2277,10 @@
 }
 
 void sum_points(size_t count, const uint32_t* pts, size_t stride, const uint8_t* mask, uint32_t* out,
-                size_t ostride, size_t col, hipStream_t stream, size_t groups) {
+                size_t ostride, size_t col, hipStream_t stream, size_t groups, const uint32_t* skip) {
   if (!groups) return;
   hipLaunchKernelGGL(k_sum_points, dim3((unsigned)groups), dim3(256), 0, stream, count, pts, stride, mask, out,
-                     ostride, col);
+                     ostride, col, skip);
 }
 
 __global__ __launch_bounds__(256) void k_add_points(size_t count, const uint32_t* __restrict__ a,
@@ -2389,7 +2414,9 @@
 }
 
 __global__ __launch_bounds__(256, 4) void k_fixed_base(size_t count, const uint32_t* __restrict__ scalars,
-                                                    const uint32_t* __restrict__ tab, uint32_t* __restrict__ out) {
+                                                    const uint32_t* __restrict__ tab, uint32_t* __restrict__ out,
+                                                    const uint32_t* __restrict__ skip) {
+  if (skip && *skip) return;
   const size_t e = (size_t)blockIdx.x * blockDim.x + threadIdx.x;
   if (e >= count) return;
   sc x;
@@ -2400,10 +2427,11 @@
   pt_store(out, count, e, acc);
 }
 
-void fixed_base(size_t count, const uint32_t* scalars, const uint32_t* tab, uint32_t* out_ext, hipStream_t stream) {
+void fixed_base(size_t count, const uint32_t* scalars, const uint32_t* tab, uint32_t* out_ext, hipStream_t stream,
+                const uint32_t* skip) {
   if (!count) return;
   hipLaunchKernelGGL(k_fixed_base, dim3((unsigned)((count + 255) / 256)), dim3(256), 0, stream, count, scalars, tab,
-                     out_ext);
+                     out_ext, skip);
 }
 
 __global__ void k_to_pos_major(size_t D, size_t N, size_t npad, const uint32_t* __restrict__ in,
@@ -2445,19 +2473,21 @@
 template <int SLICES>
 __global__ __launch_bounds__(64 * SLICES) void k_sum_shares(size_t D, size_t n, const uint32_t* __restrict__ s,
                                                           const uint8_t* __restrict__ mask,
-                                                          uint32_t* __restrict__ out) {
+                                                          uint32_t* __restrict__ out,
+                                                          const uint32_t* __restrict__ skip) {
+  if (skip && *skip) return;
   __shared__ uint32_t part[SLICES > 1 ? SLICES * 8 * 64 : 1];
   const int lane = threadIdx.x & 63, slice = threadIdx.x >> 6;
   const size_t j = (size_t)blockIdx.x * 64 + lane;
   const size_t g = blockIdx.y;
   s += g * D * n * 8;
-  mask += g * D;
+  if (mask) mask += g * D;
   out += g * n * 8;
   sc acc, x;
   sc_zero(acc);
   if (j < n)
     for (size_t i = slice; i < D; i += SLICES) {
-      if (!mask[i]) continue;
+      if (mask && !mask[i]) continue;
       sc_load(x, s + 8 * (i * n + j));
       sc_add(acc, acc, x);
     }
@@ -2476,17 +2506,17 @@
 }
 
 void sum_shares(size_t D, size_t n, const uint32_t* s, const uint8_t* mask, uint32_t* out, hipStream_t stream,
-                size_t groups) {
+                size_t groups, const uint32_t* skip) {
   if (!n) return;
   for (size_t g0 = 0; g0 < groups; g0 += 65535) {
     const size_t gc = groups - g0 < 65535 ? groups - g0 : 65535;
     const dim3 grid((unsigned)((n + 63) / 64), (unsigned)gc);
     if (gc * ((n + 63) / 64) >= 1024)
-      hipLaunchKernelGGL(k_sum_shares<1>, grid, dim3(64), 0, stream, D, n, s + g0 * D * n * 8, mask + g0 * D,
-                         out + g0 * n * 8);
+      hipLaunchKernelGGL(k_sum_shares<1>, grid, dim3(64), 0, stream, D, n, s + g0 * D * n * 8,
+                         mask ? mask + g0 * D : nullptr, out + g0 * n * 8, skip);
     else
-      hipLaunchKernelGGL(k_sum_shares<16>, grid, dim3(1024), 0, stream, D, n, s + g0 * D * n * 8, mask + g0 * D,
-                         out + g0 * n * 8);
+      hipLaunchKernelGGL(k_sum_shares<16>, grid, dim3(1024), 0, stream, D, n, s + g0 * D * n * 8,
+                         mask ? mask + g0 * D : nullptr, out + g0 * n * 8, skip);
   }
 }
 
diff --git a/dkg_amd/csrc/kernels_decl.inc b/dkg_amd/csrc/kernels_decl.inc
--- a/dkg_amd/csrc/kernels_decl.inc
+++ b/dkg_amd/csrc/kernels_decl.inc
@@ -13,7 +13,8 @@
                 const uint32_t* sp, const uint32_t* R, const uint32_t* tab_g, const uint32_t* tab_h,
                 const uint8_t* dok, uint8_t* dec2, uint8_t* dec4, hipStream_t stream, const uint32_t* scale = nullptr,
                 size_t j0 = 0, size_t jn = 0, uint32_t* acc = nullptr);
-void encode_points(const uint32_t* ext, size_t stride, size_t count, uint32_t* comp, hipStream_t stream);
+void encode_points(const uint32_t* ext, size_t stride, size_t count, uint32_t* comp, hipStream_t stream,
+                   const uint32_t* skip = nullptr);
 void build_comb(const uint32_t* ext, size_t stride, size_t e0, uint32_t* tab, hipStream_t stream, size_t count = 1);
 void build_combw(const uint32_t* ext, size_t stride, size_t e0, uint32_t* tab, hipStream_t stream, size_t count = 1);
 
@@ -104,7 +105,7 @@
 void horner(size_t ndealers, size_t npad, size_t N, const uint32_t* C, uint32_t x0, size_t nrecv, uint32_t* R,
             hipStream_t stream);
 void sum_points(size_t count, const uint32_t* pts, size_t stride, const uint8_t* mask, uint32_t* out, size_t ostride,
-                size_t col, hipStream_t stream, size_t groups = 1);
+                size_t col, hipStream_t stream, size_t groups = 1, const uint32_t* skip = nullptr);
 void add_points(size_t count, const uint32_t* a, const uint32_t* b, size_t stride, uint32_t* out, hipStream_t stream);
 void r4_error(size_t groups, size_t n, size_t t, const uint8_t* dec, const uint8_t* qmask, uint8_t* out,
               hipStream_t stream);
@@ -112,7 +113,9 @@
                       hipStream_t stream);
 void apply_skipped(size_t groups, size_t n, uint8_t* dec, const uint8_t* qmask, hipStream_t stream);
 void compact_ranks(size_t n, size_t ws, size_t R, size_t width, const void* in, void* out, hipStream_t stream);
-void mask_not_and(size_t V, const uint8_t* a, const uint8_t* b, uint8_t* out, hipStream_t stream);
+void mask_not_and(size_t V, const uint8_t* a, const uint8_t* b, uint8_t* out, hipStream_t stream,
+                  const uint32_t* skip = nullptr);
+void all_equal(size_t V, const uint8_t* a, uint32_t want, const uint32_t* prev, uint32_t* out, hipStream_t stream);
 void row_reject(size_t rows, size_t n, const uint8_t* dec, uint8_t* out, hipStream_t stream);
 size_t key_comb_words();
 int key_comb_windows();
@@ -127,12 +130,12 @@
 void msm_batch(size_t B, size_t N, const uint32_t* scalars, const uint32_t* pts, size_t stride, uint32_t* tab,
                uint32_t* out_ext, hipStream_t stream);
 void fixed_base(size_t count, const uint32_t* scalars, const uint32_t* tab, uint32_t* out_ext,
-                hipStream_t stream);
+                hipStream_t stream, const uint32_t* skip = nullptr);
 void to_position_major(size_t D, size_t N, size_t npad, const uint32_t* in, uint32_t* out,
                        hipStream_t stream);
 void reduce_scalars(size_t count, const uint32_t* in, uint32_t* out, hipStream_t stream);
 void sum_shares(size_t D, size_t n, const uint32_t* s, const uint8_t* mask, uint32_t* out, hipStream_t stream,
-                size_t groups = 1);
+                size_t groups = 1, const uint32_t* skip = nullptr);
 void dealer_coeffs(size_t rows, size_t D, size_t d0, uint32_t c0, const uint32_t* master, size_t N, uint32_t* seeds,
                    uint32_t* a, uint32_t* b, hipStream_t stream);
 
diff --git a/dkg_amd/csrc/runtime.hip b/dkg_amd/csrc/runtime.hip
--- a/dkg_amd/csrc/runtime.hip
+++ b/dkg_amd/csrc/runtime.hip
@@ -54,6 +54,9 @@
   hipEvent_t fork = nullptr, join[MAX_SUB] = {};
   hipStream_t side = nullptr;
   hipEvent_t side_fork = nullptr, shares_done = nullptr, pub_done = nullptr;
+  hipEvent_t spec_done = nullptr;
+  uint32_t* last_honest = nullptr;
+  bool tail_spec = true;
   hipEvent_t terms_done = nullptr;
   bool shares_pending = false;
   bool overlap = true;
@@ -1041,6 +1044,7 @@
   ctx->last_step_flag_words = 0;
   ctx->last_bflags = nullptr;
   ctx->last_bflag_words = 0;
+  ctx->last_honest = nullptr;
   ctx->binom_any = nullptr;
   ctx->binom_any_host = nullptr;
   if (ctx->binom_step_ded && DKG_BINOM_STEP_DED == 1) {
@@ -1172,6 +1176,14 @@
   for (size_t i = 0; i < V; i++) recon[i] = qualified[i] && recon[i];
 }
 
+struct SpecScope {
+  dkg_ctx* ctx;
+  bool pending = false;
+  explicit SpecScope(dkg_ctx* c) : ctx(c) {}
+  ~SpecScope() {
+    if (pending) (void)hipStreamWaitEvent(ctx->stream, ctx->spec_done, 0);
+  }
+};
 struct RoundMasks {
   const uint8_t *e_ok = nullptr, *a_ok = nullptr, *cmask = nullptr, *proven4 = nullptr;
 };
@@ -1191,41 +1203,68 @@
   uint8_t* qmask = buf<uint8_t>(ctx, "qmask", n);
   uint8_t* rej2 = buf<uint8_t>(ctx, "o.rej2", n);
   int32_t* cnt = buf<int32_t>(ctx, "o.cnt", 4 * n);
+  uint32_t* pub = buf<uint32_t>(ctx, "pub_ext", PTB * n);
+  uint32_t* A0 = buf<uint32_t>(ctx, "A0ext", PTB * n);
+  uint32_t* mpk_ext = buf<uint32_t>(ctx, "mpk_ext", PTB);
+  uint32_t* mpk_c = buf<uint32_t>(ctx, "mpk_comp", 32);
+  uint32_t* honest = buf<uint32_t>(ctx, "o.honest", 8);
+  uint32_t* A0c = ctx->ext_A ? nullptr : buf<uint32_t>(ctx, "A0c", 32 * n);
+  uint8_t* a0ok = ctx->ext_A ? nullptr : buf<uint8_t>(ctx, "A0ok", n);
+  auto gather_A0 = [&](hipStream_t st) {
+    if (ctx->ext_A) {
+      dkgk::gather_points(ctx->ext_A, ctx->ext_stride, N, 0, n, A0, n, st);
+    } else {
+      HCK(hipMemcpy2DAsync(A0c, 32, Acomp, 32 * N, 32, n, hipMemcpyDeviceToDevice, st));
+      dkgk::decode_points(A0c, n, A0, n, a0ok, st);
+    }
+  };
+  HCK(hipMemsetAsync(honest, 0, 8, ctx->stream));
+  const bool spec = ctx->tail_spec;
+  SpecScope spec_scope(ctx);
+  if (spec) {
+    HCK(hipEventRecord(ctx->side_fork, ctx->stream));
+    HCK(hipStreamWaitEvent(ctx->side, ctx->side_fork, 0));
+    dkgk::sum_shares(n, n, s, nullptr, fs, ctx->side);
+    dkgk::fixed_base(n, fs, ctx->tab_gw, pub, ctx->side);
+    dkgk::encode_points(pub, n, n, pubc, ctx->side);
+    gather_A0(ctx->side);
+    dkgk::sum_points(n, A0, n, nullptr, mpk_ext, 1, 0, ctx->side);
+    dkgk::encode_points(mpk_ext, 1, 1, mpk_c, ctx->side);
+    HCK(hipEventRecord(ctx->spec_done, ctx->side));
+    spec_scope.pending = true;
+  }
   auto round3 = [&] {
     wait_shares(ctx, ctx->stream);
     round2_device(ctx, 1, n, dec2, qmask, rej2, cnt, m.cmask);
-    dkgk::sum_shares(n, n, s, qmask, fs, ctx->stream);
-    uint32_t* pub = buf<uint32_t>(ctx, "pub_ext", PTB * n);
+    if (spec) {
+      if (!m.cmask) dkgk::all_equal(n, qmask, 1, nullptr, honest, ctx->stream);
+      HCK(hipStreamWaitEvent(ctx->stream, ctx->spec_done, 0));
+      spec_scope.pending = false;
+    }
+    dkgk::sum_shares(n, n, s, qmask, fs, ctx->stream, 1, honest);
     HCK(hipEventRecord(ctx->side_fork, ctx->stream));
     HCK(hipStreamWaitEvent(ctx->side, ctx->side_fork, 0));
-    dkgk::fixed_base(n, fs, ctx->tab_gw, pub, ctx->side);
-    dkgk::encode_points(pub, n, n, pubc, ctx->side);
+    dkgk::fixed_base(n, fs, ctx->tab_gw, pub, ctx->side, honest);
+    dkgk::encode_points(pub, n, n, pubc, ctx->side, honest);
     HCK(hipEventRecord(ctx->pub_done, ctx->side));
     HCK(hipEventRecord(ctx->ev[3], ctx->stream));
   };
   verify_rounds(ctx, n, t, n, 0, Ecomp, Acomp, s, sp, dec2, dec4, ctx->ev[2], round3, m.e_ok, m.a_ok, false);
+  ctx->last_honest = honest;
   wait_shares(ctx, ctx->stream);
   ctx->shares_pending = false;
   uint8_t* rej4 = buf<uint8_t>(ctx, "o.rej4", n);
   uint8_t* r4d = buf<uint8_t>(ctx, "o.r4err", n);
   round4_device(ctx, 1, n, t, dec4, qmask, rej4, r4d);
   const uint8_t* acc4 = m.proven4 ? m.proven4 : rej4;
+  const uint32_t* honest4 = honest + 1;
+  if (spec && !m.proven4) dkgk::all_equal(n, rej4, 0, honest, honest + 1, ctx->stream);
   HCK(hipEventRecord(ctx->ev[4], ctx->stream));
-  uint32_t* A0 = buf<uint32_t>(ctx, "A0ext", PTB * n);
-  if (ctx->ext_A) {
-    dkgk::gather_points(ctx->ext_A, ctx->ext_stride, N, 0, n, A0, n, ctx->stream);
-  } else {
-    uint32_t* A0c = buf<uint32_t>(ctx, "A0c", 32 * n);
-    HCK(hipMemcpy2DAsync(A0c, 32, Acomp, 32 * N, 32, n, hipMemcpyDeviceToDevice, ctx->stream));
-    uint8_t* a0ok = buf<uint8_t>(ctx, "A0ok", n);
-    dkgk::decode_points(A0c, n, A0, n, a0ok, ctx->stream);
-  }
+  if (!spec) gather_A0(ctx->stream);
   uint8_t* hmask = buf<uint8_t>(ctx, "hmask", n);
-  dkgk::mask_not_and(n, acc4, qmask, hmask, ctx->stream);
-  uint32_t* mpk_ext = buf<uint32_t>(ctx, "mpk_ext", PTB);
-  dkgk::sum_points(n, A0, n, hmask, mpk_ext, 1, 0, ctx->stream);
-  uint32_t* mpk_c = buf<uint32_t>(ctx, "mpk_comp", 32);
-  dkgk::encode_points(mpk_ext, 1, 1, mpk_c, ctx->stream);
+  dkgk::mask_not_and(n, acc4, qmask, hmask, ctx->stream, honest4);
+  dkgk::sum_points(n, A0, n, hmask, mpk_ext, 1, 0, ctx->stream, 1, honest4);
+  dkgk::encode_points(mpk_ext, 1, 1, mpk_c, ctx->stream, honest4);
   check_launch(ctx);
   uint8_t* h = hbuf<uint8_t>(ctx, "rr.out", 8 * n + 32);
   d2h(ctx, h, rej2, n);
@@ -2545,6 +2584,7 @@
   *out = nullptr;
   dkg_ctx* ctx = new dkg_ctx();
   ctx->device = device;
+  if (const char* e = getenv("DKG_TAIL_SPEC")) ctx->tail_spec = atoi(e) != 0;
   int rc = guarded(ctx, [&] {
     int least = 0, greatest = 0;
     HCK(hipDeviceGetStreamPriorityRange(&least, &greatest));
@@ -2558,6 +2598,7 @@
     HCK(hipEventCreateWithFlags(&ctx->side_fork, hipEventDisableTiming));
     HCK(hipEventCreateWithFlags(&ctx->shares_done, hipEventDisableTiming));
     HCK(hipEventCreateWithFlags(&ctx->pub_done, hipEventDisableTiming));
+    HCK(hipEventCreateWithFlags(&ctx->spec_done, hipEventDisableTiming));
     HCK(hipEventCreateWithFlags(&ctx->terms_done, hipEventDisableTiming));
     HCK(hipEventCreateWithFlags(&ctx->fork, hipEventDisableTiming));
     for (auto& e : ctx->join) HCK(hipEventCreateWithFlags(&e, hipEventDisableTiming));
@@ -2608,6 +2649,7 @@
   if (ctx->side_fork) (void)hipEventDestroy(ctx->side_fork);
   if (ctx->shares_done) (void)hipEventDestroy(ctx->shares_done);
   if (ctx->pub_done) (void)hipEventDestroy(ctx->pub_done);
+  if (ctx->spec_done) (void)hipEventDestroy(ctx->spec_done);
   if (ctx->terms_done) (void)hipEventDestroy(ctx->terms_done);
   delete ctx;
 }
@@ -2688,6 +2730,23 @@
     long long c = 0;
     for (uint32_t x : h) c += x != 0;
     return c;
+  } catch (const Fail& f) {
+    return -1;
+  }
+}
+int dkg_ctx_set_tail_spec(dkg_ctx* ctx, int on) {
+  if (!ctx || on < 0 || on > 1) return DKG_E_ARG;
+  ctx->tail_spec = on != 0;
+  return DKG_OK;
+}
+int dkg_ctx_last_tail_speculated(dkg_ctx* ctx) {
+  if (!ctx) return -1;
+  if (!ctx->last_honest) return 0;
+  try {
+    uint32_t h[2] = {0, 0};
+    sync(ctx);
+    HCK(hipMemcpy(h, ctx->last_honest, 8, hipMemcpyDeviceToHost));
+    return h[0] && h[1];
   } catch (const Fail& f) {
     return -1;
   }
diff --git a/include/dkg_amd.h b/include/dkg_amd.h
--- a/include/dkg_amd.h
+++ b/include/dkg_amd.h
@@ -44,6 +44,8 @@
 int dkg_ctx_set_addends(dkg_ctx *ctx, int mode);
 int dkg_ctx_set_stepping_formula(dkg_ctx *ctx, int mode);
 long long dkg_ctx_stepping_redos(dkg_ctx *ctx);
+int dkg_ctx_last_tail_speculated(dkg_ctx *ctx);
+int dkg_ctx_set_tail_spec(dkg_ctx *ctx, int on);
 int dkg_zero_tests(dkg_ctx *ctx, size_t count, const uint32_t *limbs, uint8_t *out);
 int dkg_fe_ops(dkg_ctx *ctx, int flavour, int op, size_t count, const uint32_t *in, uint32_t *out);
 int dkg_sc_ops(dkg_ctx *ctx, int op, size_t count, const uint32_t *in, uint32_t *out);
```

New measurement: 13.64 million verified shares/s (median of 4 runs). Within noise of the previous version (+0.5%).
